# jinhojsk515/spmm

Measured on AMD Instinct MI355X. Metric: pretrain molecules/sec, higher is better.
Workload: dtype bf16; 1 GPU; SPMM pretrain step, text 12 layers (fusion at 6) + PV 6 layers, H=768, 12 heads, queue 36864, train mode (dropout 0.1), fwd+bwd+clip+AdamW+EMA; global_batch=128, seq_len=128, parallelism=dp1, schedule=eager launches on three HIP streams, packed text rows

## Files before the change

include/spmm_hip.h:

```cpp
#ifndef SPMM_HIP_H
#define SPMM_HIP_H

#include <stdint.h>

#ifdef __HIPCC__
#include <hip/hip_runtime.h>
typedef hipStream_t spmm_stream_t;
#else
typedef void* spmm_stream_t;
#endif

#ifdef __cplusplus
extern "C" {
#endif

int spmm_version(void);
const char* spmm_last_error(void);

#define SPMM_EPI_BF16 0
#define SPMM_EPI_GELU 1
#define SPMM_EPI_F32 2
#define SPMM_EPI_F32_ATOMIC 3
#define SPMM_EPI_GELU_GRAD 4
#define SPMM_EPI_F32_ACC 5
#define SPMM_EPI_GELU_DERIV 6
#define SPMM_EPI_MUL 7

#define SPMM_GEMM_AUTO 0
#define SPMM_GEMM_K128 1
#define SPMM_GEMM_K256x128 2
#define SPMM_GEMM_K256 3
#define SPMM_GEMM_K128PC 5
#define SPMM_GEMM_K256P8 8
#define SPMM_GEMM_K256P8_TILES 9
#define SPMM_GEMM_AUTO_TILES 16
int spmm_gemm_nt(const void* A, long lda, const void* W, long ldw, int M, int N, int K, int splits, const float* bias,
                 const float* div_ptr, float alpha, const void* R, long ldr, const void* G, long ldg, void* C, long ldc,
                 void* C2, long ldc2, int epi, float* colsum, int kernel, const int* M_dev, spmm_stream_t stream);
long spmm_gemm_tn_workspace_bytes(int M, int N, int K, int splits);
int spmm_gemm_tn_splits(int M, int N, int K, int kernel);
int spmm_gemm_tn(const void* A, long lda, const void* B, long ldb, int M, int N, int K, int splits, float alpha, float* C,
                 long ldc, float* workspace, int kernel, const int* M_dev, spmm_stream_t stream);
int spmm_gemm_tn_reduce(const float* ws, int ns, int N, int K, float* C, long ldc, spmm_stream_t stream);
int spmm_colsum_bf16(const void* x, long ld, int R, int C, float* out, const int* R_dev, spmm_stream_t stream);

int spmm_attn_fwd(const void* Q, long ldq, const void* K, long ldk, const void* V, long ldv, const int* kmask,
                  const int* kv_seq, const int* q_row0, const int* q_len, const int* kv_row0, const int* kv_len, void* O,
                  long ldo, float* LSE, int nseq, int nH, int Lq, int Lkv, int causal_from, int is_cross, float dropout_p,
                  const uint64_t* seed_ptr, uint64_t seed_salt, int q_off, int kv_off, spmm_stream_t stream);
int spmm_attn_bwd(const void* Q, long ldq, const void* K, long ldk, const void* V, long ldv, const int* kmask,
                  const int* kv_seq, const int* q_row0, const int* q_len, const int* kv_row0, const int* kv_len,
                  const void* O, long ldo, const float* LSE, const void* dO, long lddo, void* dQ,
                  long lddq, void* dK, long lddk, void* dV, long lddv, int nseq, int nH, int Lq, int Lkv, int causal_from,
                  int is_cross, float dropout_p, const uint64_t* seed_ptr, uint64_t seed_salt, int q_off, int kv_off, int d_mode,
                  float* Dbuf, spmm_stream_t stream);

int spmm_xattn_supported(int H, int nH, int Lq, int Lkv);
int spmm_xattn_pack_wo(const void* W, long ldw, void* out, int H, spmm_stream_t stream);
int spmm_xattn_fwd(const void* Q, long ldq, const void* K, long ldk, const void* V, long ldv, const int* kmask,
                   const int* kv_seq, const int* q_row0, const int* q_len, const int* kv_row0, const int* kv_len,
                   const void* WoF, const float* bo, const void* R, long ldr, const float* gamma, const float* beta, float eps,
                   void* Y, long ldy, void* Z, long ldz, float* mean, float* rstd, void* CTX, long ldc, float* LSE,
                   int nseq, int nH, int Lq, int Lkv, float attn_dropout_p, uint64_t salt_a, float hidden_dropout_p,
                   uint64_t salt_h, const uint64_t* seed_ptr, long row_base, spmm_stream_t stream);
int spmm_attn_probs(const void* Q, long ldq, const void* K, long ldk, const int* kmask, const int* kv_seq,
                    const int* q_row0, const int* q_len, const int* kv_row0, const int* kv_len,
                    float* P_mean, float* P_heads, long ldp, long head_stride,
                    int nseq, int nH, int Lq, int Lkv, spmm_stream_t stream);
int spmm_segment_sum_bf16(const void* src, const int* start, const int* list, void* out, int U, long W, spmm_stream_t stream);

int spmm_ln_fwd(const void* x, const void* res, const float* gamma, const float* beta, void* y, void* zout, float* mean,
                float* rstd, long rows, int H, float eps, float dropout_p, const uint64_t* seed_ptr, uint64_t salt,
                const int* rows_dev, spmm_stream_t stream);
int spmm_ln_fwd_r32(const void* x, const float* res32, const float* gamma, const float* beta, void* y, float* y32, void* zout,
                    float* mean, float* rstd, long rows, int H, float eps, float dropout_p, const uint64_t* seed_ptr,
                    uint64_t salt, spmm_stream_t stream);
int spmm_ln_bwd(const void* dy, const void* dy2, const void* z, const float* mean, const float* rstd, const float* gamma,
                void* dz, void* dx, float* dgamma, float* dbeta, long rows, int H, float dropout_p,
                const uint64_t* seed_ptr, uint64_t salt, int drop_on_dy, float* dxsum, const int* rows_dev,
                const float* beta_from_y, spmm_stream_t stream);

int spmm_embed_step_ln_fwd(const int* ids, int pos_index, const int* pos_ptr, const float* word, const float* pos, const float* type0,
                           const float* gamma, const float* beta, void* y, long rows, int H, float eps, spmm_stream_t stream);

int spmm_decode_attn(const void* q, long ldq, const void* K, const void* V, long seq_stride, long tok_stride, long head_stride, const int* anc,
                     int anc_ld, int kv_div, int group, void* out, long ldo, int R, int nH, int Lkv, float scale,
                     const int* t_ptr, const void* knew, const void* vnew, long ldn, const int* rowmap, spmm_stream_t stream);

int spmm_decode_xattn(const void* q, long ldq, const void* K, const void* V, long ldkv, const int* kv_seq, const int* kv_row0,
                      const int* kv_len, int group, void* out, long ldo, int R, int nH, int Lkv_max, float scale, spmm_stream_t stream);

int spmm_beam_step(const float* logits, long ldl, int N, int k, int V, int Lmax, int F, int t, const int* t_ptr, int t_off,
                   int* tokens, float* cur_p, float* fin_p, int* fin_len, int* fin_tok, int* fin_n, unsigned char* done,
                   int* anc, int anc_ld, int* ids_out, int* parent_out, int* n_done, const int* mol, const int* rowmap,
                   spmm_stream_t stream);

int spmm_beam_step_until(const float* logits, long ldl, int N, int k, int V, int Lmax, int F, int t, const int* t_ptr, int t_off,
                         int* tokens, float* cur_p, float* fin_p, int* fin_len, int* fin_tok, int* fin_n, unsigned char* done,
                         int* anc, int anc_ld, int* ids_out, int* parent_out, int* n_done, const int* mol, const int* rowmap,
                         int need, spmm_stream_t stream);

int spmm_beam_step_sampled(const float* logits, long ldl, int N, int k, int V, int Lmax, int F, int t, const int* t_ptr, int t_off,
                           int* tokens, float* cur_p, float* fin_p, int* fin_len, int* fin_tok, int* fin_n, unsigned char* done,
                           int* anc, int anc_ld, int* ids_out, int* parent_out, int* n_done, const int* mol, const int* rowmap,
                           const float* noise, long ldn, spmm_stream_t stream);

int spmm_gumbel_noise(const uint64_t* seed_ptr, uint64_t salt, int N, int k, int V, int Lmax, int t, const int* t_ptr, int t_off,
                      const int* mol, long mol_base, float* out, long ldo, spmm_stream_t stream);

int spmm_logit_warp(const float* lc, const float* lu, long ld, int R, int V, float w, float temperature, int top_k, float top_p,
                    int min_keep, float* out, long ldo, spmm_stream_t stream);

#define SPMM_SYNTAX_MASKED (-1e30f)
int spmm_smiles_mask(float* logits, float* logits2, long ld, int R, int V, const int* tokens, long tok_ld, int hist_rows, int k,
                     const int* mol, int Lmax, int t, const int* t_ptr, int t_off, int t_last, const int* table, int* state_out,
                     spmm_stream_t stream);

int spmm_wordpiece(const unsigned char* blob, const long* offsets, int N, int gap, const unsigned char* head, int head_len,
                   const int* table, int table_words, int max_chars, int max_pieces, int unk_id, int sep_id, int pad_id,
                   int* ids, long ld, int* lens, int* status, spmm_stream_t stream);

int spmm_sbs_step(const float* logits, long ldl, const float* noise, long ldn, int G, int W, int V, int Lmax, int t, const int* t_ptr,
                  int t_off, const float* phi_in, const float* gum_in, const unsigned char* fin_in, const int* len_in,
                  const int* tokens_in, const int* anc_in, float* phi_out, float* gum_out, unsigned char* fin_out, int* len_out,
                  int* tokens_out, int* anc_out, int anc_ld, int* ids_out, int* parent_out, int* open_out, unsigned int* ws,
                  spmm_stream_t stream);

int spmm_kv_prefill(const void* K, const void* V, long ld, long src_rows, const int* row0, const int* len, const int* dst_row, int E,
                    void* Kc, void* Vc, int R, int nH, int Lmax, spmm_stream_t stream);

int spmm_embed_ln_fwd(int mode, const int* ids, const float* word, const float* pos, const float* type0, const float* pv_x,
                      const float* pv_mask, const float* pv_w, const float* pv_b, const float* pv_cls,
                      const float* pv_masktok, int src_mod, const float* gamma, const float* beta, void* y, void* zout,
                      float* mean, float* rstd, long nseq, int L, int H, float eps, float dropout_p,
                      const uint64_t* seed_ptr, uint64_t salt, spmm_stream_t stream);
int spmm_embed_bwd(int mode, const void* dz, const int* ids, const float* pv_x, const float* pv_mask, int src_mod,
                   float* dword, float* dpos, float* dtype0, float* d_w, float* d_b, float* d_cls, float* d_masktok,
                   long nseq, int L, int H, spmm_stream_t stream);

int spmm_transpose_bf16(const void* in, long ldi, void* out, long ldo, int R, int C, int Rpad, float* colsum,
                        spmm_stream_t stream);
int spmm_cast_transpose(const float* in, void* out, void* outT, int R, int C, spmm_stream_t stream);
long spmm_cast_transpose_desc_bytes(void);
int spmm_cast_transpose_multi(const void* descs_dev, int ndesc, int total_tiles, spmm_stream_t stream);
int spmm_cast_f32_bf16(const float* in, void* out, long n, spmm_stream_t stream);
int spmm_cast_bf16_f32(const void* in, float* out, long n, spmm_stream_t stream);
int spmm_acc_rows(float* dst, long ldd, const void* src, long lds, const long* idx, long rows, int H, int atomic,
                  spmm_stream_t stream);
int spmm_gather_rows(void* dst, const void* src, const long* idx, long rows, int H, spmm_stream_t stream);

int spmm_gather_rows2(void* dst, const void* srcA, const void* srcB, const long* idx, long rows, int H, spmm_stream_t stream);
int spmm_add_rows_bf16(void* dst, const long* idx, const void* src, long rows, int H, spmm_stream_t stream);
int spmm_zero_bytes(void* p, long nbytes, spmm_stream_t stream);
int spmm_zero_rows(void* p, long rows, long row_bytes, long stride_bytes, spmm_stream_t stream);
int spmm_gelu_bwd(const void* dz, const void* pre, void* out, long n, spmm_stream_t stream);
int spmm_pack_plan(const int* mask, int B, int Lt, int M, int* lens32, int* row0_32, long* row0_64, long* rows, long* gidx2,
                   long* gidx4, long* inv, long* idx_m, int* bad, spmm_stream_t stream);
int spmm_fusion_plan(const long* neg, const int* lens32, const int* row0_32, int B, int Lt, int Lp, int M,
                     long* idx6, long* neg_rows, long* idx_top, int* small32, spmm_stream_t stream);

int spmm_l2norm_fwd(const float* x, long ldx, float* y, float* nrm, void* a3, void* w3, void* yT, long ldt, int rows, int E,
                    spmm_stream_t stream);
int spmm_l2norm_bwd(const float* dy, const float* y, const float* nrm, const float* gscale, void* dx, int rows, int E,
                    spmm_stream_t stream);
int spmm_ita_rows(const float* S, const float* SM, long ldj, int nrows, int B, int J, const float* alpha_ptr,
                  const float* temp_ptr, void* dS, long ldd, int Jpad, float* losses, int loss_slot, float* dtemp,
                  int* nan_flag, spmm_stream_t stream);
int spmm_sample_neg(const float* S, long ldj, int B, const long* forced, const uint64_t* seed_ptr, uint64_t salt, long* out,
                    long out_offset, spmm_stream_t stream);
int spmm_lm_loss(const float* logits, const float* logits_m, long ldl, const int* ids, long nseq, int L, int V,
                 const float* alpha_ptr, int* n_nonpad_ws, const float* gscale, void* dlogits, long ldd, int Vpad,
                 float* losses, int loss_slot, spmm_stream_t stream);
int spmm_s2s_loss(const float* logits, long ldl, const int* ids, const long* row_of, long rows, long nseq, int L, int V,
                  int* n_label_ws, const float* gscale, void* dlogits, long ldd, int Vpad, float* losses, int loss_slot,
                  spmm_stream_t stream);
int spmm_lm_score(const void* y, long ldy, const void* Wd, long ldw, const float* bias, const int* ids, const long* row_of, long rows,
                  long nseq, int L, int V, int H, const int* seq_row0, const int* seq_len, float* tok_lp, float* seq_lp, int* seq_n,
                  spmm_stream_t stream);
int spmm_itm_head(const void* xa, long stride_a, const void* xb, long stride_b, int H, const float* W, const float* bias,
                  int n, int B, const float* gscale, float* losses, int loss_slot, float* logits_out, void* dxa, void* dxb,
                  float* dW, float* db, int do_bwd, int x_is_f32, spmm_stream_t stream);
int spmm_task_head(const void* A, long lda, int B, int W, const float* W2, const float* b2, int C, int kind, const void* target,
                   const float* gscale, float* logits, float* loss, void* dA, long ldda, float* dW2, float* db2, int do_bwd,
                   spmm_stream_t stream);
int spmm_s2p_append(const void* y, long ldy, const float* w3, const float* b3, const float* pe_w, const float* pe_b, const float* pos,
                    const float* type0, const float* gamma, const float* beta, float eps, float* pred, long ldp, void* xcache,
                    long rows, int H, int n_props, int i, spmm_stream_t stream);
int spmm_mpm_head(const void* h, int Lp, int H, const float* w, const float* bias, const float* target, const float* mask,
                  int B, int* n_keep_ws, const float* gscale, float* losses, int loss_slot, float* pred_out, void* dh,
                  float* dw, float* db, int do_bwd, int x_is_f32, spmm_stream_t stream);
int spmm_rows_linear(const void* x, int x_is_bf16, long ldx, const float* W, const float* bias, float* out, long ldo, long rows,
                     int N, int K, int act, spmm_stream_t stream);
long spmm_sim_topk_workspace_bytes(int Q, long n, int k);
int spmm_sim_topk(const float* q, long ldq, const float* f, long ldf, long base, int Q, long n, int E, int k, float* scores, long* index,
                  int merge, const float* cut_scores, const long* cut_index, void* workspace, long workspace_bytes, spmm_stream_t stream);
int spmm_centroid_assign(const float* f, long ldf, const float* c, long ldc, long c0, long n, int Kc, int E, float* best, int* assign,
                         int merge, const int* prev, int* changed, spmm_stream_t stream);
long spmm_cluster_group_workspace_bytes(long n, int K);
int spmm_cluster_group(const int* assign, long n, int K, int* counts, long* offsets, int* members, int* outside, void* workspace,
                       long workspace_bytes, spmm_stream_t stream);
long spmm_cluster_centroids_workspace_bytes(long n, int K, int E);
int spmm_cluster_centroids(const float* f, long ldf, long n, int E, const float* best, const int* counts, const long* offsets,
                           const int* members, int K, float* centres, long ldc, float* norm, int* medoid, void* workspace,
                           long workspace_bytes, spmm_stream_t stream);
int spmm_enqueue(const float* feats, int n, int E, float* queue, int Q, void* w3, void* qT, long ldt, int Bloc, long* ptr,
                 int advance, const int* skip_flag, spmm_stream_t stream);
int spmm_queue_shadow(const float* queue, int E, int Q, void* w3, void* qT, long ldt, int Bloc, spmm_stream_t stream);
int spmm_clamp_scalar(float* p, float lo, float hi, spmm_stream_t stream);

long spmm_adam_scalars_bytes(void);
long spmm_grad_sqnorm_workspace_bytes(void);
int spmm_grad_sqnorm(const float* g, long n, float* out_zeroed, float* workspace, spmm_stream_t stream);
int spmm_adamw_step(float* p, const float* g, float* m, float* v, void* bf16_shadow, long n, const float* lr_ptr,
                    float beta1, float beta2, float eps, float weight_decay, const float* normsq, float max_norm, int* step,
                    const int* nan_flag, void* scalars_ws, spmm_stream_t stream);
int spmm_ema_update(float* pm, const float* p, void* bf16_shadow, long n, float momentum, spmm_stream_t stream);
int spmm_axpy_scalar(float* dst, const float* src, const float* scale_ptr, float scale, int n, spmm_stream_t stream);

#ifdef __cplusplus
}
#endif
#endif
```

spmm_amd/csrc/rowops.hip:

```cpp
#include "common.h"
#include <stdlib.h>
#include "../../include/spmm_hip.h"

namespace {

constexpr int MAXC = 4;

struct RowVec {
  float v[MAXC][4];
};

__device__ __forceinline__ void load_row_bf16(const bf16* __restrict__ p, int H, int lane, RowVec& r) {
#pragma unroll
  for (int i = 0; i < MAXC; ++i) {
    const int c = (lane + 64 * i) * 4;
    if (c < H) {
      const bf16x4 t = *(const bf16x4*)(p + c);
      r.v[i][0] = (float)t[0]; r.v[i][1] = (float)t[1]; r.v[i][2] = (float)t[2]; r.v[i][3] = (float)t[3];
    } else {
      r.v[i][0] = r.v[i][1] = r.v[i][2] = r.v[i][3] = 0.f;
    }
  }
}
__device__ __forceinline__ void store_row_bf16(bf16* __restrict__ p, int H, int lane, const RowVec& r) {
// ... 240 lines not shown
                                                     bf16* __restrict__ dz_o, bf16* __restrict__ dx_o,
                                                     float* __restrict__ dgamma, float* __restrict__ dbeta, long rows, int H,
                                                     uint32_t thresh16, float dscale, const uint64_t* seed_ptr, uint64_t salt,
                                                     int drop_on_dy, float* __restrict__ dxsum, const int* __restrict__ rows_ptr) {
  __shared__ float red[4][NC * 256];
  if (rows_ptr) { const long r_ = *rows_ptr; rows = r_ < rows ? r_ : rows; }
  const int lane = threadIdx.x & 63, wave = threadIdx.x >> 6;
  float gsum[NC][4], bsum[NC][4], xsum[NC][4];
#pragma unroll
  for (int i = 0; i < NC; ++i)
#pragma unroll
    for (int j = 0; j < 4; ++j) gsum[i][j] = bsum[i][j] = xsum[i][j] = 0.f;
  if (HOT) { dy2 = nullptr; drop_on_dy = 0; }
  const bool has2 = !HOT && dy2 != nullptr, has_dx = HOT || dx_o != nullptr, has_xs = HOT || dxsum != nullptr, drop = HOT || thresh16 != 0;
  const uint64_t seed = drop ? seed_mix(seed_ptr, salt) : 0;
  const long stride = (long)gridDim.x * 4;
  long row = (long)blockIdx.x * 4 + wave;
  RawRow<NC> ng, ng2, nz;
  float nmean = 0.f, nrstd = 0.f;
  if (row < rows) {
    load_raw<NC, EXACT>(dy + row * H, H, lane, ng);
    if (has2) load_raw<NC, EXACT>(dy2 + row * H, H, lane, ng2);
    load_raw<NC, EXACT>(z + row * H, H, lane, nz);
    nmean = FROMY ? 0.f : mean_i[row]; nrstd = rstd_i[row];
  }
  for (; row < rows; row += stride) {
    RawRow<NC> cg = ng, cg2 = ng2, cz = nz;
    const float mean = nmean, rstd = nrstd;
    const long nrow = row + stride;
    if (nrow < rows) {
      load_raw<NC, EXACT>(dy + nrow * H, H, lane, ng);
      if (has2) load_raw<NC, EXACT>(dy2 + nrow * H, H, lane, ng2);
      load_raw<NC, EXACT>(z + nrow * H, H, lane, nz);
      nmean = FROMY ? 0.f : mean_i[nrow]; nrstd = rstd_i[nrow];
    }
    float g[NC][4], xh[NC][4];
    const uint32_t rowkey = drop ? drop_rowkey(seed, (uint64_t)row) : 0u;
#pragma unroll
    for (int i = 0; i < NC; ++i)
#pragma unroll
      for (int j = 0; j < 4; ++j) g[i][j] = (float)cg.v[i][j] + (has2 ? (float)cg2.v[i][j] : 0.f);
    if (drop && drop_on_dy) {
#pragma unroll
      for (int i = 0; i < NC; ++i) {
        const int c = (lane + 64 * i) * 4;
        if (EXACT || c < H) {
          bool k[4];
          drop_keep4(rowkey, c, thresh16, k);
#pragma unroll
          for (int j = 0; j < 4; ++j) g[i][j] = k[j] ? g[i][j] * dscale : 0.f;
        }
      }
    }
    float s1 = 0.f, s2 = 0.f;
#pragma unroll
    for (int i = 0; i < NC; ++i) {
      const int c = (lane + 64 * i) * 4;
      if (EXACT || c < H) {
        const f32x4 gm = *(const f32x4*)(gamma + c);
        f32x4 bt = {0.f, 0.f, 0.f, 0.f}, ig = {0.f, 0.f, 0.f, 0.f};
        if constexpr (FROMY) {
          bt = *(const f32x4*)(beta + c);
#pragma unroll
          for (int j = 0; j < 4; ++j) ig[j] = gm[j] != 0.f ? __builtin_amdgcn_rcpf(gm[j]) : 0.f;
        }
#pragma unroll
        for (int j = 0; j < 4; ++j) {
          const float x = FROMY ? ((float)cz.v[i][j] - bt[j]) * ig[j] : ((float)cz.v[i][j] - mean) * rstd;
          const float dg = g[i][j] * gm[j];
          gsum[i][j] += g[i][j] * x;
          bsum[i][j] += g[i][j];
          if constexpr (!FROMY) xh[i][j] = x;
          g[i][j] = dg;
          s1 += dg;
          s2 += dg * x;
        }
      } else {
#pragma unroll
        for (int j = 0; j < 4; ++j) { if constexpr (!FROMY) xh[i][j] = 0.f; g[i][j] = 0.f; }
      }
    }
    s1 = wave_sum_dpp(s1) / H;
    s2 = wave_sum_dpp(s2) / H;
    const bool mask_dx = has_dx && drop && !drop_on_dy;
#pragma unroll
    for (int i = 0; i < NC; ++i) {
      const int c = (lane + 64 * i) * 4;
      if (EXACT || c < H) {
        float o[4];
        if constexpr (FROMY) {
          const f32x4 gm = *(const f32x4*)(gamma + c), bt = *(const f32x4*)(beta + c);
#pragma unroll
          for (int j = 0; j < 4; ++j) {
            const float x = ((float)cz.v[i][j] - bt[j]) * (gm[j] != 0.f ? __builtin_amdgcn_rcpf(gm[j]) : 0.f);
            o[j] = rstd * (g[i][j] - s1 - x * s2);
          }
        } else {
#pragma unroll
          for (int j = 0; j < 4; ++j) o[j] = rstd * (g[i][j] - s1 - xh[i][j] * s2);
        }
        const bf16x4 ob = to_bf16x4(o[0], o[1], o[2], o[3]);
        *(bf16x4*)(dz_o + row * H + c) = ob;
        if (has_dx) {
          bf16x4 xb = ob;
          if (mask_dx) {
            bool k[4];
            drop_keep4(rowkey, c, thresh16, k);
            xb = to_bf16x4(k[0] ? o[0] * dscale : 0.f, k[1] ? o[1] * dscale : 0.f, k[2] ? o[2] * dscale : 0.f, k[3] ? o[3] * dscale : 0.f);
          }
          *(bf16x4*)(dx_o + row * H + c) = xb;
          if (has_xs) {
#pragma unroll
            for (int j = 0; j < 4; ++j) xsum[i][j] += (float)xb[j];
          }
        } else if (has_xs) {
#pragma unroll
          for (int j = 0; j < 4; ++j) xsum[i][j] += (float)ob[j];
        }
      }
    }
  }
  if (!HOT && dgamma == nullptr && dxsum == nullptr) return;
#pragma unroll
  for (int which = 0; which < 3; ++which) {
    float* dst = which == 0 ? dgamma : which == 1 ? dbeta : dxsum;
    if (!HOT && dst == nullptr) continue;
    __syncthreads();
#pragma unroll
    for (int i = 0; i < NC; ++i)
#pragma unroll
      for (int j = 0; j < 4; ++j)
        red[wave][(lane + 64 * i) * 4 + j] = which == 0 ? gsum[i][j] : which == 1 ? bsum[i][j] : xsum[i][j];
    __syncthreads();
    for (int c = threadIdx.x; c < H; c += 256) atomicAdd(dst + c, red[0][c] + red[1][c] + red[2][c] + red[3][c]);
  }
}

struct EmbedP {
  const int* ids;
  const float* word;
  const float* pos;
  const float* type0;
  const float* pv_x;
  const float* pv_mask;
  const float* pv_w; const float* pv_b; const float* pv_cls; const float* pv_masktok;
  int src_mod;
  const float* gamma; const float* beta;
  bf16* y; bf16* zout; float* mean_o; float* rstd_o;
  long nseq; int L, H, mode; float eps;
  int pos0;
  const int* pos_ptr;
  uint32_t thresh16; float dscale; const uint64_t* seed_ptr; uint64_t salt;
};

__global__ __launch_bounds__(256) void embed_ln_fwd_kernel(EmbedP p) {
  const int lane = threadIdx.x & 63;
  const long row = (long)blockIdx.x * 4 + (threadIdx.x >> 6);
  if (row >= p.nseq * p.L) return;
  const long seq = row / p.L;
  const int l = (int)(row - seq * p.L);
  RowVec z, t, o;
  load_row_f32(p.pos + (long)(l + (p.pos_ptr ? *p.pos_ptr : p.pos0)) * p.H, p.H, lane, z);
  load_row_f32(p.type0, p.H, lane, t);
#pragma unroll
  for (int i = 0; i < MAXC; ++i)
#pragma unroll
    for (int j = 0; j < 4; ++j) z.v[i][j] += t.v[i][j];
  if (p.mode == 0) {
    const int id = p.ids[row];
    load_row_f32(p.word + (long)id * p.H, p.H, lane, t);
  } else if (p.mode == 2) {
    load_row_f32(p.pv_x + row * p.H, p.H, lane, t);
  } else if (l == 0) {
    load_row_f32(p.pv_cls, p.H, lane, t);
  } else {
    const long src = (seq % p.src_mod) * (p.L - 1) + (l - 1);
    const float m = p.pv_mask[src], xv = p.pv_x[src];
    RowVec w, b;
    load_row_f32(p.pv_w, p.H, lane, w);
    load_row_f32(p.pv_b, p.H, lane, b);
    load_row_f32(p.pv_masktok, p.H, lane, t);
#pragma unroll
    for (int i = 0; i < MAXC; ++i)
#pragma unroll
      for (int j = 0; j < 4; ++j) t.v[i][j] = (xv * w.v[i][j] + b.v[i][j]) * (1.f - m) + t.v[i][j] * m;
  }
#pragma unroll
  for (int i = 0; i < MAXC; ++i)
#pragma unroll
    for (int j = 0; j < 4; ++j) z.v[i][j] += t.v[i][j];
  float mean, rstd;
  ln_apply(z, p.H, lane, p.gamma, p.beta, p.eps, mean, rstd, o);
  if (p.thresh16) {
    const uint32_t rowkey = drop_rowkey(seed_mix(p.seed_ptr, p.salt), (uint64_t)row);
#pragma unroll
    for (int i = 0; i < MAXC; ++i) {
      const int c = (lane + 64 * i) * 4;
      if (c < p.H) {
        bool k[4];
        drop_keep4(rowkey, c, p.thresh16, k);
#pragma unroll
        for (int j = 0; j < 4; ++j) o.v[i][j] = k[j] ? o.v[i][j] * p.dscale : 0.f;
      }
    }
  }
  store_row_bf16(p.y + row * p.H, p.H, lane, o);
  if (p.zout) store_row_bf16(p.zout + row * p.H, p.H, lane, z);
  if (p.mean_o && lane == 0) { p.mean_o[row] = mean; p.rstd_o[row] = rstd; }
}

struct EmbedBwdP {
  const bf16* dz; const int* ids; const float* pv_x; const float* pv_mask; int src_mod;
  float* dword; float* dpos; float* dtype0; float* d_w; float* d_b; float* d_cls; float* d_masktok;
  long nseq; int L, H, mode;
};
__global__ __launch_bounds__(256) void embed_bwd_kernel(EmbedBwdP p) {
  const int l = blockIdx.x;
  const long s_per = (p.nseq + gridDim.y - 1) / gridDim.y;
  const long s_beg = blockIdx.y * s_per, s_end = min(p.nseq, s_beg + s_per);
  for (int c = threadIdx.x; c < p.H; c += 256) {
    float acc = 0.f, accw = 0.f, accb = 0.f, accm = 0.f;
    for (long s = s_beg; s < s_end; ++s) {
      const long row = s * p.L + l;
      const float g = (float)p.dz[row * p.H + c];
      acc += g;
      if (p.mode == 0) {
        const int id = p.ids[row];
        if (id != 0) atomicAdd(p.dword + (long)id * p.H + c, g);
      } else if (l > 0) {
        const long src = (s % p.src_mod) * (p.L - 1) + (l - 1);
        const float m = p.pv_mask[src];
        accw += g * (1.f - m) * p.pv_x[src];
        accb += g * (1.f - m);
        accm += g * m;
      }
    }
    atomicAdd(p.dpos + (long)l * p.H + c, acc);
    atomicAdd(p.dtype0 + c, acc);
    if (p.mode == 1) {
      if (l == 0) {
        atomicAdd(p.d_cls + c, acc);
      } else {
        atomicAdd(p.d_w + c, accw);
        atomicAdd(p.d_b + c, accb);
        atomicAdd(p.d_masktok + c, accm);
      }
    }
  }
}

__global__ __launch_bounds__(256) void transpose_bf16_kernel(const bf16* __restrict__ in, long ldi, bf16* __restrict__ out,
                                                             long ldo, int R, int C, int Rpad, float* __restrict__ colsum) {
  __shared__ bf16 tile[64][66];
  const int r0 = blockIdx.y * 64, c0 = blockIdx.x * 64;
  const int tx = threadIdx.x & 63, ty = threadIdx.x >> 6;
  float cs = 0.f;
#pragma unroll
  for (int i = 0; i < 16; ++i) {
    const int r = r0 + ty * 16 + i, c = c0 + tx;
    const bf16 v = (r < R && c < C) ? in[(long)r * ldi + c] : (bf16)0.f;
    tile[ty * 16 + i][tx] = v;
    cs += (float)v;
  }
  if (colsum) {
    __shared__ float part[4][64];
    part[ty][tx] = cs;
    __syncthreads();
    if (ty == 0 && c0 + tx < C) atomicAdd(colsum + c0 + tx, part[0][tx] + part[1][tx] + part[2][tx] + part[3][tx]);
  } else {
    __syncthreads();
  }
#pragma unroll
  for (int i = 0; i < 16; ++i) {
    const int c = c0 + ty * 16 + i, r = r0 + tx;
    if (c < C && r < Rpad) out[(long)c * ldo + r] = tile[tx][ty * 16 + i];
  }
}

__global__ __launch_bounds__(256) void cast_transpose_kernel(const float* __restrict__ in, bf16* __restrict__ out,
                                                             bf16* __restrict__ outT, int R, int C) {
  __shared__ bf16 tile[64][66];
  const int r0 = blockIdx.y * 64, c0 = blockIdx.x * 64;
  const int tx = threadIdx.x & 63, ty = threadIdx.x >> 6;
#pragma unroll
  for (int i = 0; i < 16; ++i) {
    const int r = r0 + ty * 16 + i, c = c0 + tx;
    bf16 v = (bf16)0.f;
    if (r < R && c < C) {
      v = (bf16)in[(long)r * C + c];
      if (out) out[(long)r * C + c] = v;
    }
    tile[ty * 16 + i][tx] = v;
  }
  __syncthreads();
  if (outT) {
#pragma unroll
    for (int i = 0; i < 16; ++i) {
      const int c = c0 + ty * 16 + i, r = r0 + tx;
      if (c < C && r < R) outT[(long)c * R + r] = tile[tx][ty * 16 + i];
    }
  }
}

struct CtDesc { const float* src; bf16* dstT; int R, C; int tile0, ntc; };
__global__ __launch_bounds__(256) void cast_transpose_multi_kernel(const CtDesc* __restrict__ descs, int ndesc) {
  __shared__ bf16 tile[64][66];
  int lo = 0, hi = ndesc - 1;
  while (lo < hi) {
    const int mid = (lo + hi + 1) >> 1;
    if (descs[mid].tile0 <= (int)blockIdx.x) lo = mid; else hi = mid - 1;
  }
  const CtDesc d = descs[lo];
  const int tt = blockIdx.x - d.tile0;
  const int r0 = (tt / d.ntc) * 64, c0 = (tt % d.ntc) * 64;
  const int tx = threadIdx.x & 63, ty = threadIdx.x >> 6;
#pragma unroll
  for (int i = 0; i < 16; ++i) {
    const int r = r0 + ty * 16 + i, c = c0 + tx;
    tile[ty * 16 + i][tx] = (r < d.R && c < d.C) ? (bf16)d.src[(long)r * d.C + c] : (bf16)0.f;
  }
  __syncthreads();
#pragma unroll
  for (int i = 0; i < 16; ++i) {
    const int c = c0 + ty * 16 + i, r = r0 + tx;
    if (c < d.C && r < d.R) d.dstT[(long)c * d.R + r] = tile[tx][ty * 16 + i];
  }
}

__global__ void cast_f32_bf16_kernel(const float* __restrict__ in, bf16* __restrict__ out, long n4) {
  for (long i = (long)blockIdx.x * blockDim.x + threadIdx.x; i < n4; i += (long)gridDim.x * blockDim.x) {
    const f32x4 v = *(const f32x4*)(in + i * 4);
    *(bf16x4*)(out + i * 4) = to_bf16x4(v[0], v[1], v[2], v[3]);
  }
}
__global__ void cast_bf16_f32_kernel(const bf16* __restrict__ in, float* __restrict__ out, long n4) {
  for (long i = (long)blockIdx.x * blockDim.x + threadIdx.x; i < n4; i += (long)gridDim.x * blockDim.x) {
    const bf16x4 v = *(const bf16x4*)(in + i * 4);
    f32x4 o = {(float)v[0], (float)v[1], (float)v[2], (float)v[3]};
    *(f32x4*)(out + i * 4) = o;
  }
}

__global__ void acc_rows_kernel(float* __restrict__ dst, long ldd, const bf16* __restrict__ src, long lds,
                                const long* __restrict__ idx, long rows, int H, int atomic) {
  const int h4 = H / 4;
  for (long i = (long)blockIdx.x * blockDim.x + threadIdx.x; i < rows * h4; i += (long)gridDim.x * blockDim.x) {
    const long r = i / h4;
    const int c = (int)(i - r * h4) * 4;
    const long dr = idx ? idx[r] : r;
    if (dr < 0) continue;
    const bf16x4 v = *(const bf16x4*)(src + r * lds + c);
    float* d = dst + dr * ldd + c;
    if (atomic) {
#pragma unroll
      for (int j = 0; j < 4; ++j) atomicAdd(d + j, (float)v[j]);
    } else {
      f32x4 o = *(f32x4*)d;
      o[0] += (float)v[0]; o[1] += (float)v[1]; o[2] += (float)v[2]; o[3] += (float)v[3];
      *(f32x4*)d = o;
    }
  }
}
__global__ void gather_rows_kernel(bf16* __restrict__ dst, const bf16* __restrict__ src, const long* __restrict__ idx,
                                   long rows, int H) {
  const int h8 = H / 8;
  for (long i = (long)blockIdx.x * blockDim.x + threadIdx.x; i < rows * h8; i += (long)gridDim.x * blockDim.x) {
    const long r = i / h8;
    const int c = (int)(i - r * h8) * 8;
    *(bf16x8*)(dst + r * H + c) = *(const bf16x8*)(src + idx[r] * H + c);
  }
}

int grid_for(long work, int block) {
  long g = (work + block - 1) / block;
  return (int)(g < 1 ? 1 : (g > 2048 ? 2048 : g));
}


}

extern "C" int spmm_ln_fwd(const void* x, const void* res, const float* gamma, const float* beta, void* y, void* zout,
                           float* mean, float* rstd, long rows, int H, float eps, float dropout_p,
                           const uint64_t* seed_ptr, uint64_t salt, const int* rows_dev, hipStream_t stream) {
  SPMM_CHECK_SHAPE(rows > 0 && H > 0 && H % 4 == 0 && H <= 1024, "spmm_ln_fwd: rows=%ld H=%d (need H%%4==0, H<=1024)", rows, H);
  SPMM_CHECK_SHAPE(dropout_p == 0.f || seed_ptr, "spmm_ln_fwd: dropout needs a device seed");
  SPMM_CHECK_SHAPE(x && gamma && beta && y, "spmm_ln_fwd: null x / gamma / beta / y");
  SPMM_CHECK_SHAPE((mean == nullptr) == (rstd == nullptr), "spmm_ln_fwd: mean and rstd come together");
  const uint32_t th = (uint32_t)(dropout_p * 65536.f + 0.5f);
  const float ds = 1.f / (1.f - dropout_p);
#define LN_FWD16(NC)                                                                                                          \
  hipLaunchKernelGGL(ln_fwd16_kernel<NC>, dim3((rows + 7) / 8), dim3(256), 0, stream, (const bf16*)x, (const bf16*)res, gamma, \
                     beta, (bf16*)y, (bf16*)zout, mean, rstd, rows, eps, th, ds, seed_ptr, salt, rows_dev)
  if (H == 768) LN_FWD16(3);
  else if (H == 1024) LN_FWD16(4);
  else if (H == 512) LN_FWD16(2);
  else if (H == 256) LN_FWD16(1);
  else
    hipLaunchKernelGGL(ln_fwd_kernel, dim3((rows + 3) / 4), dim3(256), 0, stream, (const bf16*)x, (const bf16*)res, gamma, beta,
                       (bf16*)y, (bf16*)zout, mean, rstd, rows, H, eps, th, ds, seed_ptr, salt, rows_dev);
#undef LN_FWD16
  SPMM_LAUNCH_CHECK("spmm_ln_fwd");
  return SPMM_OK;
}

extern "C" int spmm_ln_fwd_r32(const void* x, const float* res32, const float* gamma, const float* beta, void* y, float* y32, void* zout,
                               float* mean, float* rstd, long rows, int H, float eps, float dropout_p, const uint64_t* seed_ptr,
                               uint64_t salt, hipStream_t stream) {
  SPMM_CHECK_SHAPE(rows > 0 && H > 0 && H % 4 == 0 && H <= 1024, "spmm_ln_fwd_r32: rows=%ld H=%d (need H%%4==0, H<=1024)", rows, H);
  SPMM_CHECK_SHAPE(dropout_p == 0.f || seed_ptr, "spmm_ln_fwd_r32: dropout needs a device seed");
  SPMM_CHECK_SHAPE((mean == nullptr) == (rstd == nullptr), "spmm_ln_fwd_r32: mean and rstd come together");
  hipLaunchKernelGGL(ln_fwd_r32_kernel, dim3((rows + 3) / 4), dim3(256), 0, stream, (const bf16*)x, res32, gamma, beta, (bf16*)y, y32,
                     (bf16*)zout, mean, rstd, rows, H, eps, (uint32_t)(dropout_p * 65536.f + 0.5f), 1.f / (1.f - dropout_p), seed_ptr, salt);
  SPMM_LAUNCH_CHECK("spmm_ln_fwd_r32");
  return SPMM_OK;
}

extern "C" int spmm_ln_bwd(const void* dy, const void* dy2, const void* z, const float* mean, const float* rstd,
                           const float* gamma, void* dz, void* dx, float* dgamma, float* dbeta, long rows, int H,
                           float dropout_p, const uint64_t* seed_ptr, uint64_t salt, int drop_on_dy, float* dxsum, const int* rows_dev,
                           const float* beta_from_y, hipStream_t stream) {
  SPMM_CHECK_SHAPE(rows > 0 && H > 0 && H % 4 == 0 && H <= 1024, "spmm_ln_bwd: rows=%ld H=%d", rows, H);
  SPMM_CHECK_SHAPE(beta_from_y != nullptr || mean != nullptr, "spmm_ln_bwd: the row means are required unless `z` holds the LayerNorm output (beta_from_y)");
  SPMM_CHECK_SHAPE(beta_from_y == nullptr || !drop_on_dy, "spmm_ln_bwd: the output of a LayerNorm followed by dropout does not determine the normalised values");
  SPMM_CHECK_SHAPE(dropout_p == 0.f || seed_ptr, "spmm_ln_bwd: dropout needs a device seed");
  SPMM_CHECK_SHAPE(dy && z && rstd && gamma && dz, "spmm_ln_bwd: null dy / z / rstd / gamma / dz");
  long g = (rows + 3) / 4;
  static const long genv = getenv("SPMM_LN_BWD_GRID") ? atol(getenv("SPMM_LN_BWD_GRID")) : 0;
  long gmax = genv > 0 ? genv : rows / 64;
  if (genv <= 0) gmax = gmax < 256 ? 256 : (gmax > 512 ? 512 : gmax);
  if (g > gmax) g = gmax;
  const uint32_t th = (uint32_t)(dropout_p * 65536.f + 0.5f);
  const float ds = 1.f / (1.f - dropout_p);
  const bool hot = !dy2 && dx && dgamma && dbeta && dxsum && th && !drop_on_dy;
#define LN_BWD_LAUNCH(NC, EX, HOT, FY)                                                                                                \
  hipLaunchKernelGGL((ln_bwd_kernel<NC, EX, HOT, FY>), dim3(g), dim3(256), 0, stream, (const bf16*)dy, (const bf16*)dy2, (const bf16*)z, \
                     mean, rstd, gamma, beta_from_y, (bf16*)dz, (bf16*)dx, dgamma, dbeta, rows, H, th, ds, seed_ptr, salt, drop_on_dy, dxsum, rows_dev)
  if (beta_from_y != nullptr) {
    if (H == 768 && hot) LN_BWD_LAUNCH(3, true, true, true);
    else if (H <= 768) LN_BWD_LAUNCH(3, false, false, true);
    else LN_BWD_LAUNCH(4, false, false, true);
  } else {
    if (H == 768 && hot) LN_BWD_LAUNCH(3, true, true, false);
    else if (H <= 768) LN_BWD_LAUNCH(3, false, false, false);
    else LN_BWD_LAUNCH(4, false, false, false);
  }
#undef LN_BWD_LAUNCH
  SPMM_LAUNCH_CHECK("spmm_ln_bwd");
  return SPMM_OK;
}

extern "C" int spmm_embed_ln_fwd(int mode, const int* ids, const float* word, const float* pos, const float* type0,
                                 const float* pv_x, const float* pv_mask, const float* pv_w, const float* pv_b,
                                 const float* pv_cls, const float* pv_masktok, int src_mod, const float* gamma,
                                 const float* beta, void* y, void* zout, float* mean, float* rstd, long nseq, int L, int H,
                                 float eps, float dropout_p, const uint64_t* seed_ptr, uint64_t salt, hipStream_t stream) {
  SPMM_CHECK_SHAPE(nseq > 0 && L > 0 && H > 0 && H % 4 == 0 && H <= 1024, "spmm_embed_ln_fwd: nseq=%ld L=%d H=%d (need 0 < H <= 1024, H%%4==0)", nseq, L, H);
  SPMM_CHECK_SHAPE(mode >= 0 && mode <= 2, "spmm_embed_ln_fwd: unknown mode %d", mode);
  SPMM_CHECK_SHAPE(pos && type0 && gamma && beta && y, "spmm_embed_ln_fwd: null pos / type0 / gamma / beta / y");
  SPMM_CHECK_SHAPE((mean == nullptr) == (rstd == nullptr), "spmm_embed_ln_fwd: mean and rstd come together");
  SPMM_CHECK_SHAPE(mode == 0 ? (ids && word) : mode == 2 ? (pv_x != nullptr) : (pv_x && pv_mask && pv_w && pv_b && pv_cls && pv_masktok && src_mod > 0),
                   "spmm_embed_ln_fwd: missing inputs for mode %d", mode);
  SPMM_CHECK_SHAPE(dropout_p == 0.f || seed_ptr, "spmm_embed_ln_fwd: dropout needs a device seed");
  EmbedP p = {};
  p.ids = ids; p.word = word; p.pos = pos; p.type0 = type0; p.pv_x = pv_x; p.pv_mask = pv_mask; p.pv_w = pv_w; p.pv_b = pv_b;
  p.pv_cls = pv_cls; p.pv_masktok = pv_masktok; p.src_mod = src_mod; p.gamma = gamma; p.beta = beta; p.y = (bf16*)y;
  p.zout = (bf16*)zout; p.mean_o = mean; p.rstd_o = rstd; p.nseq = nseq; p.L = L; p.H = H; p.mode = mode; p.eps = eps;
  p.thresh16 = (uint32_t)(dropout_p * 65536.f + 0.5f); p.dscale = 1.f / (1.f - dropout_p); p.seed_ptr = seed_ptr; p.salt = salt;
  hipLaunchKernelGGL(embed_ln_fwd_kernel, dim3((nseq * L + 3) / 4), dim3(256), 0, stream, p);
  SPMM_LAUNCH_CHECK("spmm_embed_ln_fwd");
  return SPMM_OK;
}

extern "C" int spmm_embed_step_ln_fwd(const int* ids, int pos_index, const int* pos_ptr, const float* word, const float* pos, const float* type0,
                                      const float* gamma, const float* beta, void* y, long rows, int H, float eps,
                                      hipStream_t stream) {
  SPMM_CHECK_SHAPE(rows > 0 && pos_index >= 0 && H % 4 == 0 && H <= 1024, "spmm_embed_step_ln_fwd: rows=%ld pos=%d H=%d", rows, pos_index, H);
  SPMM_CHECK_SHAPE(ids && word && pos && type0 && gamma && beta && y, "spmm_embed_step_ln_fwd: null argument");
  EmbedP p = {};
  p.ids = ids; p.word = word; p.pos = pos; p.type0 = type0; p.gamma = gamma; p.beta = beta; p.y = (bf16*)y;
  p.nseq = rows; p.L = 1; p.H = H; p.mode = 0; p.eps = eps; p.pos0 = pos_index; p.pos_ptr = pos_ptr; p.dscale = 1.f;
  hipLaunchKernelGGL(embed_ln_fwd_kernel, dim3((rows + 3) / 4), dim3(256), 0, stream, p);
  SPMM_LAUNCH_CHECK("spmm_embed_step_ln_fwd");
  return SPMM_OK;
}

extern "C" int spmm_embed_bwd(int mode, const void* dz, const int* ids, const float* pv_x, const float* pv_mask, int src_mod,
                              float* dword, float* dpos, float* dtype0, float* d_w, float* d_b, float* d_cls,
                              float* d_masktok, long nseq, int L, int H, hipStream_t stream) {
  SPMM_CHECK_SHAPE(nseq > 0 && L > 0 && H > 0, "spmm_embed_bwd: nseq=%ld L=%d H=%d", nseq, L, H);
  SPMM_CHECK_SHAPE(mode == 0 || mode == 1, "spmm_embed_bwd: mode %d (0 = text, 1 = PV; inputs_embeds has no backward)", mode);
  SPMM_CHECK_SHAPE(dz && dpos && dtype0, "spmm_embed_bwd: null dz / dpos / dtype0");
  SPMM_CHECK_SHAPE(mode != 0 || (ids && dword), "spmm_embed_bwd: mode 0 needs ids and dword");
  SPMM_CHECK_SHAPE(mode != 1 || (pv_x && pv_mask && d_w && d_b && d_cls && d_masktok), "spmm_embed_bwd: mode 1 needs pv_x, pv_mask, d_w, d_b, d_cls and d_masktok");
  SPMM_CHECK_SHAPE(mode != 1 || src_mod > 0, "spmm_embed_bwd: mode 1 needs src_mod > 0, got src_mod=%d", src_mod);
  EmbedBwdP p = {(const bf16*)dz, ids, pv_x, pv_mask, src_mod, dword, dpos, dtype0, d_w, d_b, d_cls, d_masktok, nseq, L, H, mode};
  hipLaunchKernelGGL(embed_bwd_kernel, dim3(L, nseq >= 32 ? 16 : 1), dim3(256), 0, stream, p);
  SPMM_LAUNCH_CHECK("spmm_embed_bwd");
  return SPMM_OK;
}

namespace {
__global__ __launch_bounds__(256) void segment_sum_kernel(const bf16* __restrict__ src, const int* __restrict__ start,
                                                          const int* __restrict__ list, bf16* __restrict__ out, long W) {
  const int u = blockIdx.y;
  const long c = ((long)blockIdx.x * 256 + threadIdx.x) * 8;
  if (c >= W) return;
  const int k0 = start[u], k1 = start[u + 1];
  float acc[8] = {0.f, 0.f, 0.f, 0.f, 0.f, 0.f, 0.f, 0.f};
  for (int k = k0; k < k1; ++k) {
    const bf16x8 v = *(const bf16x8*)(src + (long)list[k] * W + c);
#pragma unroll
    for (int e = 0; e < 8; ++e) acc[e] += (float)v[e];
  }
  bf16x8 o;
#pragma unroll
  for (int e = 0; e < 8; ++e) o[e] = (bf16)acc[e];
  *(bf16x8*)(out + (long)u * W + c) = o;
}
}

extern "C" int spmm_segment_sum_bf16(const void* src, const int* start, const int* list, void* out, int U, long W, hipStream_t stream) {
  SPMM_CHECK_SHAPE(U > 0 && U <= 65535 && W > 0 && W % 8 == 0, "spmm_segment_sum_bf16: U=%d W=%ld (W %% 8 == 0)", U, W);
  SPMM_CHECK_SHAPE(src && start && list && out, "spmm_segment_sum_bf16: null src / start / list / out");
  hipLaunchKernelGGL(segment_sum_kernel, dim3((unsigned)((W / 8 + 255) / 256), U), dim3(256), 0, stream, (const bf16*)src, start, list,
                     (bf16*)out, W);
  SPMM_LAUNCH_CHECK("spmm_segment_sum_bf16");
  return SPMM_OK;
}

extern "C" int spmm_transpose_bf16(const void* in, long ldi, void* out, long ldo, int R, int C, int Rpad, float* colsum,
                                   hipStream_t stream) {
  SPMM_CHECK_SHAPE(R > 0 && C > 0 && Rpad >= R && ldo >= Rpad, "spmm_transpose_bf16: R=%d C=%d Rpad=%d ldo=%ld", R, C, Rpad, ldo);
  SPMM_CHECK_SHAPE(ldi >= C, "spmm_transpose_bf16: ldi=%ld is shorter than a row of C=%d", ldi, C);
  SPMM_CHECK_SHAPE(in && out, "spmm_transpose_bf16: null in / out");
  hipLaunchKernelGGL(transpose_bf16_kernel, dim3((C + 63) / 64, (Rpad + 63) / 64), dim3(256), 0, stream, (const bf16*)in, ldi,
                     (bf16*)out, ldo, R, C, Rpad, colsum);
  SPMM_LAUNCH_CHECK("spmm_transpose_bf16");
  return SPMM_OK;
}

extern "C" int spmm_cast_transpose(const float* in, void* out, void* outT, int R, int C, hipStream_t stream) {
  SPMM_CHECK_SHAPE(R > 0 && C > 0, "spmm_cast_transpose: R=%d C=%d", R, C);
  SPMM_CHECK_SHAPE(in && (out || outT), "spmm_cast_transpose: null in, or neither out nor outT");
  hipLaunchKernelGGL(cast_transpose_kernel, dim3((C + 63) / 64, (R + 63) / 64), dim3(256), 0, stream, in, (bf16*)out, (bf16*)outT, R, C);
  SPMM_LAUNCH_CHECK("spmm_cast_transpose");
  return SPMM_OK;
}

extern "C" long spmm_cast_transpose_desc_bytes(void) { return sizeof(CtDesc); }
extern "C" int spmm_cast_transpose_multi(const void* descs_dev, int ndesc, int total_tiles, hipStream_t stream) {
  SPMM_CHECK_SHAPE(ndesc > 0 && total_tiles > 0, "spmm_cast_transpose_multi: ndesc=%d tiles=%d", ndesc, total_tiles);
  hipLaunchKernelGGL(cast_transpose_multi_kernel, dim3(total_tiles), dim3(256), 0, stream, (const CtDesc*)descs_dev, ndesc);
  SPMM_LAUNCH_CHECK("spmm_cast_transpose_multi");
  return SPMM_OK;
}

extern "C" int spmm_cast_f32_bf16(const float* in, void* out, long n, hipStream_t stream) {
  SPMM_CHECK_SHAPE(n > 0 && n % 4 == 0, "spmm_cast_f32_bf16: n=%ld must be a positive multiple of 4", n);
  SPMM_CHECK_SHAPE(in && out, "spmm_cast_f32_bf16: null in / out");
  hipLaunchKernelGGL(cast_f32_bf16_kernel, dim3(grid_for(n / 4, 256)), dim3(256), 0, stream, in, (bf16*)out, n / 4);
  SPMM_LAUNCH_CHECK("spmm_cast_f32_bf16");
  return SPMM_OK;
}
extern "C" int spmm_cast_bf16_f32(const void* in, float* out, long n, hipStream_t stream) {
  SPMM_CHECK_SHAPE(n > 0 && n % 4 == 0, "spmm_cast_bf16_f32: n=%ld must be a positive multiple of 4", n);
  SPMM_CHECK_SHAPE(in && out, "spmm_cast_bf16_f32: null in / out");
  hipLaunchKernelGGL(cast_bf16_f32_kernel, dim3(grid_for(n / 4, 256)), dim3(256), 0, stream, (const bf16*)in, out, n / 4);
  SPMM_LAUNCH_CHECK("spmm_cast_bf16_f32");
  return SPMM_OK;
}

extern "C" int spmm_acc_rows(float* dst, long ldd, const void* src, long lds, const long* idx, long rows, int H, int atomic,
                             hipStream_t stream) {
  SPMM_CHECK_SHAPE(rows > 0 && H > 0 && H % 4 == 0, "spmm_acc_rows: rows=%ld H=%d", rows, H);
  SPMM_CHECK_SHAPE(dst && src, "spmm_acc_rows: null dst / src");
  SPMM_CHECK_SHAPE(rows == 1 || (ldd >= H && lds >= H), "spmm_acc_rows: ldd=%ld lds=%ld are shorter than a row of H=%d", ldd, lds, H);
  hipLaunchKernelGGL(acc_rows_kernel, dim3(grid_for(rows * (H / 4), 256)), dim3(256), 0, stream, dst, ldd, (const bf16*)src, lds,
                     idx, rows, H, atomic);
  SPMM_LAUNCH_CHECK("spmm_acc_rows");
  return SPMM_OK;
}
extern "C" int spmm_gather_rows(void* dst, const void* src, const long* idx, long rows, int H, hipStream_t stream) {
  SPMM_CHECK_SHAPE(rows > 0 && H > 0 && H % 8 == 0 && idx, "spmm_gather_rows: rows=%ld H=%d", rows, H);
  SPMM_CHECK_SHAPE(dst && src, "spmm_gather_rows: null dst / src");
  hipLaunchKernelGGL(gather_rows_kernel, dim3(grid_for(rows * (H / 8), 256)), dim3(256), 0, stream, (bf16*)dst, (const bf16*)src,
                     idx, rows, H);
  SPMM_LAUNCH_CHECK("spmm_gather_rows");
  return SPMM_OK;
}
```

spmm_amd/engine.py:

```python
from __future__ import annotations

import contextlib
import functools
from dataclasses import dataclass
from typing import List, NamedTuple, Optional

import numpy as np
import torch

from . import ops, streams
from .config import BertConfig, SPMMConfig
from .options import EngineOptions
from .params import ParamStore

BF = torch.bfloat16
LOSS_MLM, LOSS_MPM, LOSS_ITA, LOSS_ITM = 0, 1, 2, 3


def _ceil(x, m):
    return (x + m - 1) // m * m


class KVSource:

    def __init__(self, kv: torch.Tensor, U: int, Lkv: int, row0=None, length=None, pack_idx=None, proj=None):
        self.kv, self.U, self.Lkv, self.row0, self.len, self.pack_idx = kv, U, Lkv, row0, length, pack_idx
        self.proj = proj
        self._idx: List[torch.Tensor] = []
        self.nseq = 0
        self.start = self.list = None

    def add(self, idx: torch.Tensor) -> int:
        off = self.nseq
        self._idx.append(idx)
        self.nseq += idx.numel()
        return off

    def preset(self, nseq: int, start: torch.Tensor, lst: torch.Tensor):
        self.nseq, self.start, self.list = nseq, start, lst
        return self

    def finalize(self):
        idx = torch.cat(self._idx)
        order = torch.sort(idx, stable=True).indices
        start = torch.zeros(self.U + 1, dtype=torch.int32, device=idx.device)
        counts = torch.zeros(self.U, dtype=torch.int64, device=idx.device).index_add_(0, idx, torch.ones_like(idx))
        start[1:] = torch.cumsum(counts, 0)
        self.start, self.list = start, order.to(torch.int32)
        return self


@dataclass
class SelfKV:
    x: torch.Tensor
    dx: Optional[torch.Tensor] = None
    rows_dev: Optional[torch.Tensor] = None


@dataclass
class Group:
    row0: int
    nseq: int
    L: int
    kmask: Optional[torch.Tensor]
    causal_from: int
    kv: Optional[torch.Tensor] = None
    Lkv: int = 0
    kv_mask: Optional[torch.Tensor] = None
    q_row0: Optional[torch.Tensor] = None
    q_len: Optional[torch.Tensor] = None
    nrows: int = -1
    src: Optional[KVSource] = None
    kv_idx: Optional[torch.Tensor] = None
    kv_off: int = 0
    self_src: Optional[SelfKV] = None
    skv_row0: Optional[torch.Tensor] = None
    skv_len: Optional[torch.Tensor] = None
    skv_L: int = 0

    @property
    def rows(self):
        n = self.nrows if self.nrows >= 0 else self.nseq * self.L
        return slice(self.row0, self.row0 + n)

    def bind(self, src: KVSource, kv_idx: torch.Tensor, kv_off: int) -> "Group":
        self.src, self.Lkv, self.kv_idx, self.kv_off = src, src.Lkv, kv_idx, kv_off
        return self

    def attend(self, src: KVSource, idx: torch.Tensor) -> "Group":
        self.src, self.Lkv = src, src.Lkv
        self.kv_off = src.add(idx)
        self.kv_idx = idx.to(torch.int32)
        return self

    def cross_layout(self) -> dict:
        src = self.src
        return dict(kmask=self.kv_mask, kv_seq=self.kv_idx, q_row0=self.q_row0, q_len=self.q_len,
                    kv_row0=None if src is None else src.row0, kv_len=None if src is None else src.len)


@dataclass
class Batch:
    groups: List[Group]
    rows_dev: Optional[torch.Tensor] = None

    def __iter__(self):
        return iter(self.groups)

    def __len__(self):
        return len(self.groups)


@dataclass
class LnTape:
    z: Optional[torch.Tensor]
    y: Optional[torch.Tensor]
    mean: Optional[torch.Tensor]
    rstd: Optional[torch.Tensor]
    salt: int = 0


@dataclass
class HeadTape:
    dense: str
    norm: str
    X: torch.Tensor
    pre: Optional[torch.Tensor]
    ln: LnTape


def _prefix_lens(mask_h: torch.Tensor) -> Optional[torch.Tensor]:
    lens = mask_h.sum(1)
    prefix = bool((lens > 0).all()) and bool(((torch.arange(mask_h.shape[1])[None, :] < lens[:, None]) == (mask_h != 0)).all())
    return lens if prefix else None


def host_lens(mask_h: torch.Tensor, what: str) -> np.ndarray:
    if mask_h.dim() != 2 or mask_h.shape[0] == 0:
        raise ValueError(f"{what}: the attention mask must be [n, L] with n >= 1")
    lens = _prefix_lens(mask_h)
    if lens is None:
        raise ValueError(f"{what}: every attention mask must be a non-empty prefix (what padding a batch to its longest gives)")
    return lens.numpy().astype(np.int64)


def host_token_count(mask) -> Optional[int]:
    if not (torch.is_tensor(mask) and mask.device.type == "cpu" and mask.dim() == 2):
        return None
    lens = _prefix_lens(mask)
    return None if lens is None else int(lens.sum())


class PairLayout(NamedTuple):
    len_p: np.ndarray
    qrow0: np.ndarray
    Mt: int
    pos: np.ndarray
    seq: np.ndarray
    gather: np.ndarray


@dataclass
class TextRows:
    x: torch.Tensor
    groups: Batch
    pk: Optional[dict]
    cls_rows: torch.Tensor
    ids32: torch.Tensor
    mask32: torch.Tensor
    B: int
    L: int
    esv: LnTape
    y: Optional[torch.Tensor] = None
    tape: Optional[list] = None

    @property
    def kv_mask(self):
        return None if self.pk else self.mask32

    def tables(self):
        if self.pk:
            return self.pk["row0"], self.pk["len"]
        return torch.arange(self.B, dtype=torch.int32, device=self.mask32.device) * self.L, self.mask32.sum(1).to(torch.int32)

    def source(self, proj=None, tables: bool = False) -> KVSource:
        row0, length = self.tables() if (self.pk or tables) else (None, None)
        return KVSource(self.y, self.B, self.L, row0=row0, length=length, pack_idx=self.pk["rows"] if self.pk else None, proj=proj)

    def pair_layout(self, lens_u: np.ndarray, inv: np.ndarray) -> PairLayout:
        row0_u = np.concatenate([[0], np.cumsum(lens_u)[:-1]]) if self.pk else np.arange(self.B, dtype=np.int64) * self.L
        len_p = lens_u[inv]
        qrow0 = np.concatenate([[0], np.cumsum(len_p)[:-1]])
        pos = np.concatenate([np.arange(l) for l in len_p])
        seq = np.repeat(np.arange(len(inv)), len_p)
        return PairLayout(len_p, qrow0, int(len_p.sum()), pos, seq, row0_u[inv][seq] + pos)


STREAM_TOKENS_MAX = 49152


class Engine:
    def __init__(self, cfg: SPMMConfig, params: ParamStore, device, options: Optional[EngineOptions] = None):
        self.cfg, self.P, self.dev = cfg, params, device
        self.opt = options if options is not None else EngineOptions.from_env()
        if torch.device(device).type == "cuda":
            from ._lib import bind_device
            bind_device(torch.device(device).index if torch.device(device).index is not None else torch.cuda.current_device())
        f32 = dict(dtype=torch.float32, device=device)
        self.alpha = torch.zeros(1, **f32)
        self.lr = torch.zeros(1, **f32)
        self.gscale = torch.ones(4, **f32)
        self.step_zero = torch.zeros(16, dtype=torch.int32, device=device)
        self.losses = self.step_zero[0:8].view(torch.float32)
        self.loss_scratch = torch.zeros(8, **f32)
        rank = torch.distributed.get_rank() if (torch.distributed.is_available() and torch.distributed.is_initialized()) else 0
        self.seed_rank_offset = rank * 0x9E3779B97F4A7C15 % (1 << 62)
        self.seed = torch.full((1,), (0x5DEECE66D + self.seed_rank_offset) % (1 << 62), dtype=torch.int64, device=device)
        self.nan_flag = self.step_zero[9:10]
        self.icount = torch.zeros(8, dtype=torch.int32, device=device)
        self.dtemp_ita = self.step_zero[8:9].view(torch.float32)
        self.train_mode = True
        self.hint_bad = self.step_zero[10:11]
        self.pack_text = self.opt.pack_text
        self.layer_done_cb = None
        self.multi_stream = self.opt.multi_stream
        self.wgrad_async = self.opt.wgrad_stream and self.multi_stream
        self._one_stream = False
        dist_ = torch.distributed
        will_exchange = dist_.is_available() and dist_.is_initialized() and (dist_.get_world_size() > 1 or self.opt.force_dist)
        self._one_side = bool(will_exchange and self.opt.dp_four_streams)
        if self.multi_stream and torch.device(device).type == "cuda" and not ops._DRY_RUN and not will_exchange:
            streams.bind_in_order(device, ("side0", "side1", "wgrad"))
        self.force_one_stream = False
        self._wg_stream, self._wg_pending, self._wg_keep = None, False, []
        self._salt = 0
        self._off_path_ok, self._pre_bwd = False, None
        self._xattn_checked = self._xattn_off = False
        self.tape = None
        E, Q = cfg.embed_dim, cfg.queue_size
        self._bank = None

    def _fork(self, which: int = 0):
        if not self.multi_stream or self._one_stream or self.dev.type != "cuda" or ops._DRY_RUN:
            return None
        side = streams.get(self.dev, "side0" if self._one_side else f"side{which}")
        streams.after(side, torch.cuda.current_stream())
        return side

    def _join(self, side):
        if side is not None:
            streams.after(torch.cuda.current_stream(), side)

    @staticmethod
    def _on(side):
        return torch.cuda.stream(side) if side is not None else contextlib.nullcontext()

    def _new(self, *shape, dtype=BF):
        return torch.empty(*shape, dtype=dtype, device=self.dev)

    def _stats(self, M, save):
        return (self._new(M, dtype=torch.float32), self._new(M, dtype=torch.float32)) if save else (None, None)

    def _zeros(self, *shape, dtype=BF):
        return ops.zero_(torch.empty(*shape, dtype=dtype, device=self.dev))

    def _next_salt(self):
        self._salt += 1
        return self._salt * 0x9E3779B97F4A7C15 % (1 << 63)

    def _p_hidden(self, c: BertConfig):
        return c.hidden_dropout_prob if self.train_mode else 0.0

    def _p_attn(self, c: BertConfig):
        return c.attention_probs_dropout_prob if self.train_mode else 0.0

    def _wT(self, key, src_fp32):
        return self.P.wT(key, src_fp32)

    def _wgrad(self, dY, X, gW, gb=None, inline=False, md=None):
        ws = None if inline else self._wgrad_side()
        C = gW.view(dY.shape[1], X.shape[1])
        if ws is None:
            if gb is not None:
                ops.colsum_bf16(dY, gb, R_dev=md)
            ops.gemm_tn(dY, X, C, M_dev=md)
            return
        streams.after(ws, torch.cuda.current_stream())
        with torch.cuda.stream(ws):
            if gb is not None:
                ops.colsum_bf16(dY, gb, R_dev=md)
            ops.gemm_tn(dY, X, C, M_dev=md)
        self._wg_keep.append((dY, X))
        self._wg_pending = True

    def _wgrad_side(self):
        if not self.wgrad_async or self._one_stream or self.dev.type != "cuda" or ops._DRY_RUN:
            return None
        self._wg_stream = streams.get(self.dev, "wgrad")
        return self._wg_stream

    def off_path(self, fn):
        ws = self._wgrad_side() if self._off_path_ok else None
        if ws is None or torch.cuda.is_current_stream_capturing():
            fn()
            return
        streams.after(ws, torch.cuda.current_stream())
        with torch.cuda.stream(ws):
            fn()
            self._pre_bwd = streams.mark(ws)

    def pre_backward_wait(self):
        ev, self._pre_bwd = self._pre_bwd, None
        if ev is not None:
            torch.cuda.current_stream().wait_event(ev)

    def wgrad_join(self, release: bool = False):
        if self._wg_stream is not None and self._wg_pending:
            streams.after(torch.cuda.current_stream(), self._wg_stream)
            if release:
                self._wg_keep.clear()
                self._wg_pending = False

    def end_backward(self):
        self.wgrad_join(release=True)
        self.tape = None

    def _pack_plan(self, mask32: torch.Tensor, B: int, Lt: int, n_tokens: Optional[int] = None):
        if n_tokens is not None:
            M = int(n_tokens)
            if M >= B * Lt:
                return None
        else:
            lens = mask32.sum(1)
            prefix = (torch.arange(Lt, device=mask32.device)[None, :] < lens[:, None]) == (mask32 != 0)
            stats = torch.stack([lens.sum(), (lens > 0).sum(), prefix.all().to(lens.dtype)]).cpu()
            M, nonempty, is_prefix = int(stats[0]), int(stats[1]), int(stats[2])
            if nonempty != B or not is_prefix or M >= B * Lt:
                return None
        if M < 1:
            return None
        return ops.pack_plan(mask32, M, self.hint_bad)

    def text_rows(self, x: torch.Tensor, mask32: torch.Tensor, pk: Optional[dict]):
        B, L = mask32.shape
        if not pk:
            return x, Batch([Group(0, B, L, mask32, B)]), torch.arange(B, dtype=torch.int64, device=self.dev) * L
        x = ops.gather_rows2(self._new(pk["M"], x.shape[1]), x, pk["rows"])
        return x, Batch([Group(0, B, L, None, B, q_row0=pk["row0"], q_len=pk["len"], nrows=pk["M"])]), pk["row0_64"]

    def text_rows_of(self, pfx, c, ids32, mask32, *, n_tokens: Optional[int] = None, save=False, causal=False, what: str = "") -> TextRows:
        B, L = ids32.shape
        if L > c.max_position_embeddings:
            raise ValueError(f"{what}sequence length {L} exceeds the {c.max_position_embeddings} position embeddings")
        x, esv = self.embed_text(pfx, c, ids32, B, L, save)
        pk = self._pack_plan(mask32, B, L, n_tokens) if (self.pack_text and L <= ops.ATTN_MAXL) else None
        x, groups, cls_rows = self.text_rows(x, mask32, pk)
        if causal:
            groups.groups[0].causal_from = 0
        return TextRows(x, groups, pk, cls_rows, ids32, mask32, B, L, esv)

    def encode_text(self, pfx, c, ids32, mask32, *, n_tokens: Optional[int] = None, save=False, causal=False, what: str = "") -> TextRows:
        t = self.text_rows_of(pfx, c, ids32, mask32, n_tokens=n_tokens, save=save, causal=causal, what=what)
        t.y, t.tape, _ = self.stack_fwd(pfx, c, range(0, c.fusion_layer), False, t.x, t.groups, save)
        return t

    def _ln_res(self, x, X, X32, gamma, beta, y, md, **kw):
        if X32 is None:
            ops.ln_fwd(x, X, gamma, beta, y, rows_dev=md, **kw)
            return None
        assert md is None
        y32 = self._new(*y.shape, dtype=torch.float32)
        ops.ln_fwd_r32(x, X32, gamma, beta, y, y32=y32, **kw)
        return y32

    def _proj_ln(self, op, A, resid, X32, *, save, eps, ph, salt, md=None):
        P = self.P
        Wb = P.wb(op + "dense.weight")
        M, H = A.shape[0], Wb.shape[0]
        x, y = self._new(M, H), self._new(M, H)
        mean, rstd = self._stats(M, save)
        ops.gemm_nt(A, Wb, x, bias=P.w(op + "dense.bias"), M_dev=md)
        from_y = self.opt.ln_from_y and X32 is None
        y32 = self._ln_res(x, resid, X32, P.w(op + "LayerNorm.weight"), P.w(op + "LayerNorm.bias"), y, md,
                           zout=x if (save and not from_y) else None, mean=mean, rstd=rstd, eps=eps, dropout_p=ph, seed=self.seed, salt=salt)
        return y, LnTape(None if from_y else x, y, mean, rstd, salt), y32

    def _proj_ln_bwd(self, op, tape, dY, A, ph, md=None):
        P, (M, H) = self.P, dY.shape
        dz = self._new(M, H)
        dx = self._new(M, H) if ph > 0 else dz
        from_y = tape.z is None
        ops.ln_bwd(dY, tape.y if from_y else tape.z, tape.mean, tape.rstd, P.w(op + "LayerNorm.weight"), dz, dx=dx if ph > 0 else None,
                   dgamma=P.g(op + "LayerNorm.weight"), dbeta=P.g(op + "LayerNorm.bias"), dropout_p=ph, seed=self.seed, salt=tape.salt,
                   dxsum=P.g(op + "dense.bias"), rows_dev=md, beta_from_y=P.w(op + "LayerNorm.bias") if from_y else None)
        self._wgrad(dx, A, P.g(op + "dense.weight"), md=md)
        return dz, dx

    def _attn_block_fwd(self, pfx, c, X, groups, save, cross, X32=None, kv_tap=None, xattn_tap=None):
        P, H, nH = self.P, c.hidden_size, c.num_attention_heads
        salts_a = [self._next_salt() for _ in groups]
        salt_h = self._next_salt()
        sv = {"X": X, "salt_a": salts_a, "cross": cross}
        if not cross:
            ctx, core = self._self_attn_fwd(pfx, c, X, groups, save, salts_a, kv_tap)
        else:
            sv["Qc"] = Qc = ops.gemm_nt(X, P.wb(pfx + ".self.query.weight"), self._new(X.shape[0], H), bias=P.w(pfx + ".self.query.bias"),
                                        M_dev=groups.rows_dev)
            done = {id(g.src): g.src.proj[pfx] for g in groups if g.src is not None and g.src.proj and pfx in g.src.proj}
            kv_of = functools.partial(self._xattn_kv, P.fused(pfx + ".self.", ("key", "value"), "weight"),
                                      P.fused(pfx + ".self.", ("key", "value"), "bias", what="w"), done)
            if xattn_tap is not None:
                for gi, g in enumerate(groups):
                    xattn_tap(gi, g, Qc[g.rows], kv_of(g)[:, :H])
            fx = self.opt.fused_xattn
            fused = ((fx is True or fx == "all" or (fx == "nograd" and not save)) and not self._xattn_off and X32 is None
                     and groups.rows_dev is None and all(ops.xattn_supported(H, nH, g.L, g.Lkv) for g in groups))
            if fused:
                y, out = self._xattn_fused_fwd(pfx, c, X, Qc, kv_of, groups, save, salts_a, salt_h)
                g0 = groups.groups[0]
                if not self._xattn_checked and not ops._DRY_RUN and g0.row0 == 0:
                    self._xattn_checked = True
                    agrees, dmax, dmean = self._xattn_agrees(pfx, c, X, Qc, out["KV"][0], g0, y, salts_a[0], salt_h)
                    if not agrees:
                        import warnings
                        warnings.warn(f"spmm_amd: the fused cross-attention kernel disagrees with the composite launches (max |dy| {dmax:.3g}, "
                                      f"mean {dmean:.3g}); falling back to the composite for this process (SPMM_FUSED_XATTN=off)")
                        streams.note("fused cross-attention kernel failed its one-time self-check: composite launches used instead")
                        self._xattn_off = True
                        fused = False
                if fused:
                    sv.update(out)
                    return y, (sv if save else None), None
            ctx, core = self._xattn_core_fwd(c, Qc, kv_of, groups, save, salts_a)
        y, ln, y32 = self._proj_ln(pfx + ".output.", ctx, X, X32, save=save, eps=c.layer_norm_eps, ph=self._p_hidden(c), salt=salt_h,
                                   md=groups.rows_dev)
        sv.update(core, ctx=ctx, ln=ln)
        return y, (sv if save else None), y32

    def _self_attn_fwd(self, pfx, c, X, groups, save, salts, kv_tap=None):
        P, H, nH, M = self.P, c.hidden_size, c.num_attention_heads, X.shape[0]
        Wqkv = P.fused(pfx + ".self.", ("query", "key", "value"), "weight")
        bqkv = P.fused(pfx + ".self.", ("query", "key", "value"), "bias", what="w")
        QKV = ops.gemm_nt(X, Wqkv, self._new(M, 3 * H), bias=bqkv, M_dev=groups.rows_dev)
        if kv_tap is not None:
            kv_tap(QKV)
        ctx, lses = self._new(M, H), []
        skv = {}
        for g, salt in zip(groups, salts):
            lse = self._new(g.nseq, nH, g.L, dtype=torch.float32) if save else None
            r = g.rows
            kw = dict(nseq=g.nseq, nH=nH, Lq=g.L, dropout_p=self._p_attn(c), seed=self.seed, salt=salt, q_row0=g.q_row0, q_len=g.q_len)
            if g.self_src is not None:
                if id(g.self_src) not in skv:
                    skv[id(g.self_src)] = ops.gemm_nt(g.self_src.x, Wqkv[H:], self._new(g.self_src.x.shape[0], 2 * H), bias=bqkv[H:],
                                                      M_dev=g.self_src.rows_dev)
                KVs = skv[id(g.self_src)]
                ops.attn_fwd_long(QKV[r, :H], KVs[:, :H], KVs[:, H:], ctx[r], lse, Lkv=g.skv_L, kmask=None, causal_from=g.nseq,
                                  kv_row0=g.skv_row0, kv_len=g.skv_len, **kw)
            else:
                ops.attn_fwd_long(QKV[r, :H], QKV[r, H:2 * H], QKV[r, 2 * H:], ctx[r], lse, Lkv=g.L, kmask=g.kmask, causal_from=g.causal_from,
                                  kv_row0=g.q_row0, kv_len=g.q_len, **kw)
            lses.append(lse)
        return ctx, dict(QKV=QKV, SKV=skv, lse=lses)

    def _xattn_kv(self, Wkv, bkv, done, g):
        key, kv = (id(g), g.kv) if g.src is None else (id(g.src), g.src.kv)
        if key not in done:
            done[key] = ops.gemm_nt(kv, Wkv, self._new(kv.shape[0], Wkv.shape[0]), bias=bkv)
        return done[key]

    def _xattn_core_fwd(self, c, Qc, kv_of, groups, save, salts):
        H, nH = c.hidden_size, c.num_attention_heads
        ctx, KVs, lses = self._new(Qc.shape[0], H), [], []
        for g, salt in zip(groups, salts):
            KV = kv_of(g)
            lse = self._new(g.nseq, nH, g.L, dtype=torch.float32) if save else None
            ops.attn_fwd_long(Qc[g.rows], KV[:, :H], KV[:, H:], ctx[g.rows], lse, nseq=g.nseq, nH=nH, Lq=g.L, Lkv=g.Lkv, is_cross=True,
                              dropout_p=self._p_attn(c), seed=self.seed, salt=salt, **g.cross_layout())
            KVs.append(KV)
            lses.append(lse)
        return ctx, dict(KV=KVs, lse=lses)

    def _xattn_fused_fwd(self, pfx, c, X, Qc, kv_of, groups, save, salts, salt_h):
        P, H, nH, M = self.P, c.hidden_size, c.num_attention_heads, X.shape[0]
        y = self._new(M, H)
        z, ctx = (self._new(M, H), self._new(M, H)) if save else (None, None)
        mean, rstd = self._stats(M, save)
        WoF = P.wF(pfx + ".output.dense.weight")
        KVs, lses = [], []
        for g, salt in zip(groups, salts):
            KV = kv_of(g)
            lse = self._new(g.nseq, nH, g.L, dtype=torch.float32) if save else None
            r = g.rows
            ops.xattn_fwd(Qc[r], KV[:, :H], KV[:, H:], WoF, P.w(pfx + ".output.dense.bias"), X[r], P.w(pfx + ".output.LayerNorm.weight"),
                          P.w(pfx + ".output.LayerNorm.bias"), y[r], nseq=g.nseq, nH=nH, Lq=g.L, Lkv=g.Lkv, eps=c.layer_norm_eps,
                          Z=None if z is None else z[r], mean=None if mean is None else mean[r.start:r.stop],
                          rstd=None if rstd is None else rstd[r.start:r.stop], CTX=None if ctx is None else ctx[r], lse=lse,
                          attn_dropout_p=self._p_attn(c), salt_a=salt, hidden_dropout_p=self._p_hidden(c), salt_h=salt_h, seed=self.seed,
                          row_base=r.start, **g.cross_layout())
            KVs.append(KV)
            lses.append(lse)
        return y, dict(KV=KVs, lse=lses, ctx=ctx, ln=LnTape(z, y, mean, rstd, salt_h))

    def _xattn_agrees(self, pfx, c, X, Qc, KV, g, y, salt_a, salt_h):
        H, r = c.hidden_size, g.rows
        c2 = self._new(r.stop, H)
        ops.attn_fwd_long(Qc[r], KV[:, :H], KV[:, H:], c2, None, nseq=g.nseq, nH=c.num_attention_heads, Lq=g.L, Lkv=g.Lkv, is_cross=True,
                          dropout_p=self._p_attn(c), seed=self.seed, salt=salt_a, **g.cross_layout())
        y2, _, _ = self._proj_ln(pfx + ".output.", c2, X[r], None, save=False, eps=c.layer_norm_eps, ph=self._p_hidden(c), salt=salt_h)
        d = (y[r].float() - y2.float()).abs()
        dmax, dmean = float(d.max()), float(d.mean())
        scale = max(1.0, float(y2.float().abs().max()) / 8.0)
        return dmax < 0.25 * scale and dmean < 5e-3 * scale, dmax, dmean

    def _attn_block_bwd(self, pfx, c, sv, dY, groups, dkv_acc):
        P, H, nH = self.P, c.hidden_size, c.num_attention_heads
        X, M, md = sv["X"], sv["X"].shape[0], groups.rows_dev
        pa, ph = self._p_attn(c), self._p_hidden(c)
        dz, dx = self._proj_ln_bwd(pfx + ".output.", sv["ln"], dY, sv["ctx"], ph, md)
        dctx = self._new(M, H)
        ops.gemm_nt(dx, self._wT(pfx + ".output.dense", P.w(pfx + ".output.dense.weight")), dctx, M_dev=md)
        dX = self._new(M, H)
        if not sv["cross"]:
            QKV = sv["QKV"]
            dQKV = self._new(M, 3 * H)
            gWqkv = P.fused(pfx + ".self.", ("query", "key", "value"), "weight", what="g")
            gbqkv = P.fused(pfx + ".self.", ("query", "key", "value"), "bias", what="g")
            dskv = {}
            for i, g in enumerate(groups):
                r = g.rows
                kw = dict(nseq=g.nseq, nH=nH, Lq=g.L, dropout_p=pa, seed=self.seed, salt=sv["salt_a"][i], q_row0=g.q_row0, q_len=g.q_len)
                if g.self_src is not None:
                    if id(g.self_src) not in dskv:
                        dskv[id(g.self_src)] = (g.self_src, self._zeros(g.self_src.x.shape[0], 2 * H))
                    KVs, dKVs = sv["SKV"][id(g.self_src)], dskv[id(g.self_src)][1]
                    ops.attn_bwd_long(QKV[r, :H], KVs[:, :H], KVs[:, H:], sv["ctx"][r], sv["lse"][i], dctx[r], dQKV[r, :H], dKVs[:, :H], dKVs[:, H:],
                                      Lkv=g.skv_L, kmask=None, causal_from=g.nseq, kv_row0=g.skv_row0, kv_len=g.skv_len, **kw)
                    ops.zero_(dQKV[r, H:])
                    continue
                ops.attn_bwd_long(QKV[r, :H], QKV[r, H:2 * H], QKV[r, 2 * H:], sv["ctx"][r], sv["lse"][i], dctx[r], dQKV[r, :H],
                                  dQKV[r, H:2 * H], dQKV[r, 2 * H:], Lkv=g.L, kmask=g.kmask, causal_from=g.causal_from,
                                  kv_row0=g.q_row0, kv_len=g.q_len, **kw)
            self._wgrad(dQKV, X, gWqkv, gbqkv, md=md)
            WT = self._wT(pfx + ".self.qkv", P.fused(pfx + ".self.", ("query", "key", "value"), "weight", what="w"))
            for src, dKVs in dskv.values():
                self._wgrad(dKVs, src.x, gWqkv[H:], gbqkv[H:], md=src.rows_dev)
                ops.gemm_nt(dKVs, WT[:, H:], src.dx, M_dev=src.rows_dev)
            ops.gemm_nt(dQKV, WT, dX, R=dz, M_dev=md)
        else:
            Qc = sv["Qc"]
            dQc = self._new(M, H)
            gWkv = P.fused(pfx + ".self.", ("key", "value"), "weight", what="g")
            gbkv = P.fused(pfx + ".self.", ("key", "value"), "bias", what="g")
            WkvT = self._wT(pfx + ".self.kv", P.fused(pfx + ".self.", ("key", "value"), "weight", what="w"))
            pool = {}
            for i, g in enumerate(groups):
                r = g.rows
                KV = sv["KV"][i]
                src = g.src
                if src is not None:
                    if id(src) not in pool:
                        pool[id(src)] = (src, self._new(src.nseq * src.Lkv, 2 * H))
                    dKV = pool[id(src)][1][g.kv_off * g.Lkv:(g.kv_off + g.nseq) * g.Lkv]
                else:
                    dKV = self._new(g.nseq * g.Lkv, 2 * H)
                ops.attn_bwd_long(Qc[r], KV[:, :H], KV[:, H:], sv["ctx"][r], sv["lse"][i], dctx[r], dQc[r], dKV[:, :H], dKV[:, H:],
                                  nseq=g.nseq, nH=nH, Lq=g.L, Lkv=g.Lkv, is_cross=True, dropout_p=pa, seed=self.seed, salt=sv["salt_a"][i],
                                  **g.cross_layout())
                if src is None:
                    self._wgrad(dKV, g.kv, gWkv, gbkv)
                    ops.gemm_nt(dKV, WkvT, dkv_acc[i], epi=ops.EPI_F32_ACC)
            for src, dKV in pool.values():
                W = src.Lkv * 2 * H
                dKVu = ops.segment_sum_bf16(dKV.view(src.nseq, W), src.start, src.list, self._new(src.U, W)).view(-1, 2 * H)
                if src.pack_idx is not None:
                    dKVu = ops.gather_rows(self._new(src.pack_idx.numel(), 2 * H), dKVu, src.pack_idx)
                self._wgrad(dKVu, src.kv, gWkv, gbkv)
                ops.gemm_nt(dKVu, WkvT, dkv_acc[id(src)], epi=ops.EPI_F32_ACC)
            self._wgrad(dQc, X, P.g(pfx + ".self.query.weight"), P.g(pfx + ".self.query.bias"), md=md)
            ops.gemm_nt(dQc, self._wT(pfx + ".self.query", P.w(pfx + ".self.query.weight")), dX, R=dz, M_dev=md)
        return dX

    def _layer_fwd(self, lp, c, has_cross, X, groups, save, X32=None, kv_tap=None, xattn_tap=None):
        P, H, I, M = self.P, c.hidden_size, c.intermediate_size, X.shape[0]
        tap = {} if kv_tap is None else {"kv_tap": kv_tap}
        a, sv1, a32 = self._attn_block_fwd(lp + "attention", c, X, groups, save, cross=False, X32=X32, **tap)
        sv2 = None
        if has_cross:
            xtap = {} if xattn_tap is None else {"xattn_tap": xattn_tap}
            a, sv2, a32 = self._attn_block_fwd(lp + "crossattention", c, a, groups, save, cross=True, X32=a32, **xtap)
        h = self._new(M, I)
        dact = self._new(M, I) if save else None
        ops.gemm_nt(a, P.wb(lp + "intermediate.dense.weight"), h, bias=P.w(lp + "intermediate.dense.bias"),
                    epi=ops.EPI_GELU_DERIV if save else ops.EPI_GELU, C2=dact, M_dev=groups.rows_dev)
        salt = self._next_salt()
        y, ln, y32 = self._proj_ln(lp + "output.", h, a, a32, save=save, eps=c.layer_norm_eps, ph=self._p_hidden(c), salt=salt, md=groups.rows_dev)
        sv = dict(att=sv1, cross=sv2, a=a, h=h, dact=dact, ln=ln) if save else None
        return y, sv, y32

    def _layer_bwd(self, lp, c, sv, dY, groups, dkv_acc):
        P, H, I, M, md = self.P, c.hidden_size, c.intermediate_size, dY.shape[0], groups.rows_dev
        dz, dx = self._proj_ln_bwd(lp + "output.", sv["ln"], dY, sv["h"], self._p_hidden(c), md)
        dpre = self._new(M, I)
        ops.gemm_nt(dx, self._wT(lp + "output.dense", P.w(lp + "output.dense.weight")), dpre,
                    epi=ops.EPI_MUL, G=sv["dact"], colsum=P.g(lp + "intermediate.dense.bias"), M_dev=md)
        self._wgrad(dpre, sv["a"], P.g(lp + "intermediate.dense.weight"), md=md)
        da = self._new(M, H)
        ops.gemm_nt(dpre, self._wT(lp + "intermediate.dense", P.w(lp + "intermediate.dense.weight")), da, R=dz, M_dev=md)
        if sv["cross"] is not None:
            da = self._attn_block_bwd(lp + "crossattention", c, sv["cross"], da, groups, dkv_acc)
        return self._attn_block_bwd(lp + "attention", c, sv["att"], da, groups, None)

    def stack_fwd(self, pfx, c, layers, has_cross, X, groups, save, X32=None, kv_tap=None, xattn_tap=None):
        tape = []
        for i in layers:
            tap = None if kv_tap is None else functools.partial(kv_tap, i)
            xtap = {} if xattn_tap is None else {"xattn_tap": functools.partial(xattn_tap, i)}
            X, sv, X32 = self._layer_fwd(f"{pfx}encoder.layer.{i}.", c, has_cross and i >= c.fusion_layer, X, groups, save, X32=X32, kv_tap=tap,
                                         **xtap)
            tape.append(sv)
        return X, tape, X32

    def stack_bwd(self, pfx, c, layers, tape, dY, groups, dkv_acc=None):
        for i, sv in zip(reversed(list(layers)), reversed(tape)):
            dY = self._layer_bwd(f"{pfx}encoder.layer.{i}.", c, sv, dY, groups, dkv_acc)
            if self.layer_done_cb is not None:
                self._layer_done(f"{pfx}encoder.layer.{i}.")
        return dY

    def _layer_done(self, prefix):
        ws = self._wg_stream if (self._wg_pending and self.wgrad_async) else None
        if ws is None:
            self.wgrad_join()
            return self.layer_done_cb(prefix)
        streams.after(ws, torch.cuda.current_stream())
        with torch.cuda.stream(ws):
            return self.layer_done_cb(prefix)

    def _embed(self, mode, pfx, c, nseq, L, save, salt, **src):
        P, H = self.P, c.hidden_size
        y = self._new(nseq * L, H)
        z = self._new(nseq * L, H) if save else None
        mean, rstd = self._stats(nseq * L, save)
        ops.embed_ln_fwd(mode, y, nseq=nseq, L=L, H=H, pos=P.w(pfx + "embeddings.position_embeddings.weight"),
                         type0=P.w(pfx + "embeddings.token_type_embeddings.weight"), gamma=P.w(pfx + "embeddings.LayerNorm.weight"),
                         beta=P.w(pfx + "embeddings.LayerNorm.bias"), zout=z, mean=mean, rstd=rstd, eps=c.layer_norm_eps,
                         dropout_p=self._p_hidden(c), seed=self.seed, salt=salt, **src)
        return y, LnTape(z, None, mean, rstd, salt)

    def embed_text(self, pfx, c, ids32, nseq, L, save):
        return self._embed(0, pfx, c, nseq, L, save, self._next_salt(), ids=ids32, word=self.P.w(pfx + "embeddings.word_embeddings.weight"))

    def embed_pv(self, pfx, c, prop, mpm_mask, nseq, src_mod, save):
        P = self.P
        return self._embed(1, pfx, c, nseq, self.cfg.n_props + 1, save, self._next_salt(), pv_x=prop, pv_mask=mpm_mask,
                           pv_w=P.w("property_embed.weight"), pv_b=P.w("property_embed.bias"), pv_cls=P.w("property_cls"),
                           pv_masktok=P.w("property_mask"), src_mod=src_mod)

    def embed_generic(self, pfx, c, inputs_embeds_f32, nseq, L):
        return self._embed(2, pfx, c, nseq, L, False, self._next_salt(), pv_x=inputs_embeds_f32)[0]

    def _embed_ln_bwd(self, pfx, c, tape, dY):
        P = self.P
        dz = self._new(*dY.shape)
        ops.ln_bwd(dY, tape.z, tape.mean, tape.rstd, P.w(pfx + "embeddings.LayerNorm.weight"), dz,
                   dgamma=P.g(pfx + "embeddings.LayerNorm.weight"), dbeta=P.g(pfx + "embeddings.LayerNorm.bias"),
                   dropout_p=self._p_hidden(c), seed=self.seed, salt=tape.salt, drop_on_dy=True)
        return dz

    def _transform_fwd(self, dense, norm, X, save, *, eps, r32=False, pre=True):
        P, M, H = self.P, X.shape[0], X.shape[1]
        t = self._new(M, H)
        pre = self._new(M, H) if pre else None
        ops.gemm_nt(X, P.wb(dense + ".weight"), t, bias=P.w(dense + ".bias"), epi=ops.EPI_GELU, C2=pre)
        y = self._new(M, H)
        mean, rstd = self._stats(M, save)
        z = t if save else None
        kw = dict(zout=z, mean=mean, rstd=rstd, eps=eps)
        if r32:
            y32 = self._new(M, H, dtype=torch.float32)
            ops.ln_fwd_r32(t, None, P.w(norm + ".weight"), P.w(norm + ".bias"), y, y32=y32, **kw)
            y = y32
        else:
            ops.ln_fwd(t, None, P.w(norm + ".weight"), P.w(norm + ".bias"), y, **kw)
        return y, HeadTape(dense, norm, X, pre, LnTape(z, y, mean, rstd))

    def _transform_bwd(self, tape, dy):
        P, ln = self.P, tape.ln
        dz = self._new(*dy.shape)
        ops.ln_bwd(dy, ln.z, ln.mean, ln.rstd, P.w(tape.norm + ".weight"), dz, dgamma=P.g(tape.norm + ".weight"), dbeta=P.g(tape.norm + ".bias"))
        dpre = self._gelu_bwd(dz, tape.pre)
        self._wgrad(dpre, tape.X, P.g(tape.dense + ".weight"), P.g(tape.dense + ".bias"))
        return dpre

    def lm_head_fwd(self, pfx, c, X, save):
        P = self.P
        tf = pfx + "cls.predictions.transform."
        y, tape = self._transform_fwd(tf + "dense", tf + "LayerNorm", X, save, eps=c.layer_norm_eps)
        logits = self._new(X.shape[0], c.vocab_size, dtype=torch.float32)
        ops.gemm_nt(y, P.wb(pfx + "cls.predictions.decoder.weight"), logits, bias=P.w(pfx + "cls.predictions.bias"), epi=ops.EPI_F32)
        return logits, tape

    def lm_head_bwd(self, pfx, c, tape, dlogits, out=None):
        P, H, V, M = self.P, c.hidden_size, c.vocab_size, dlogits.shape[0]
        Vp = dlogits.shape[1]
        self._wgrad(dlogits[:, :V], tape.ln.y, P.g(pfx + "bert.embeddings.word_embeddings.weight"), P.g(pfx + "cls.predictions.bias"), inline=True)
        dy = self._new(M, H)
        ops.gemm_nt(dlogits, P.wT_padded(pfx + "cls.decoderT", pfx + "bert.embeddings.word_embeddings.weight", Vp), dy)
        dpre = self._transform_bwd(tape, dy)
        dX = self._new(M, H) if out is None else out
        ops.gemm_nt(dpre, self._wT(pfx + "cls.transform", P.w(pfx + "cls.predictions.transform.dense.weight")), dX)
        return dX

    def _gelu_bwd(self, dz, pre):
        return ops.gelu_bwd(dz, pre)

    def _feat_fwd(self, proj, X, L, B, save, cls_rows=None, X32=None):
        P, E, H = self.P, self.cfg.embed_dim, self.cfg.text.hidden_size
        if cls_rows is not None:
            cls = X.index_select(0, cls_rows)
        else:
            cls = X.view(-1, L * H)[:B, :H]
        raw = self._new(B, E, dtype=torch.float32)
        if X32 is not None:
            cls32 = X32.index_select(0, cls_rows) if cls_rows is not None else X32.view(-1, L * H)[:B, :H]
            ops.rows_linear(cls32, P.w(proj + ".weight"), P.w(proj + ".bias"), raw)
        else:
            ops.gemm_nt(cls, P.wb(proj + ".weight"), raw, bias=P.w(proj + ".bias"), epi=ops.EPI_F32)
        feat = self._new(B, E, dtype=torch.float32)
        nrm = self._new(B, dtype=torch.float32)
        return raw, feat, nrm, cls

    def _banks(self, B):
        if self._bank is not None and self._bank["B"] == B:
            return self._bank
        E, Q = self.cfg.embed_dim, self.cfg.queue_size
        J = B + Q
        Jp = _ceil(J, 64)
        bank = {"B": B, "J": J, "Jp": Jp}
        for nm in ("prop", "text"):
            w3 = torch.zeros(J, 3 * E, dtype=BF, device=self.dev)
            qT = torch.zeros(E, Jp, dtype=BF, device=self.dev)
            ops.queue_shadow(self.P.buffers[nm + "_queue"], w3, qT, Bloc=B)
            bank[nm] = (w3, qT)
        self._bank = bank
        return bank

    def invalidate_banks(self):
        self._bank = None
```

spmm_amd/ops.py:

```python
import ctypes
import os

import torch

from ._lib import lib

EPI_BF16, EPI_GELU, EPI_F32, EPI_F32_ATOMIC, EPI_GELU_GRAD, EPI_F32_ACC, EPI_GELU_DERIV, EPI_MUL = range(8)
BF16 = torch.bfloat16


_DRY_RUN = False
_dry_log = []


def _p(t):
    return None if t is None else ctypes.c_void_p(t.data_ptr())


def _st():
    if _DRY_RUN:
        return None
    return ctypes.c_void_p(torch.cuda.current_stream().cuda_stream)


_DEBUG_SYNC = os.environ.get("SPMM_DEBUG_SYNC") == "1"


def _call(name, *args):
    if not _DRY_RUN:
        if _DEBUG_SYNC:
            import sys
            r = lib().call(name, *args)
            print(f"[launch] {name} {[a for a in args if isinstance(a, int) and not isinstance(a, bool)][:8]}", file=sys.stderr, flush=True)
            torch.cuda.synchronize()
            return r
        return lib().call(name, *args)
    res, argtypes = lib().protos[name]
    if len(args) != len(argtypes):
        raise TypeError(f"{name}: {len(args)} arguments, header declares {len(argtypes)}")
    for i, (a, t) in enumerate(zip(args, argtypes)):
        try:
            t(a) if not isinstance(a, ctypes.c_void_p) else None
        except Exception as e:
            raise TypeError(f"{name}: argument {i} = {a!r} is not a {t.__name__}") from e
        if t is ctypes.c_void_p and not (a is None or isinstance(a, (ctypes.c_void_p, int))):
            raise TypeError(f"{name}: argument {i} must be a pointer, got {type(a)}")
    _dry_log.append(name)


def _row_stride(t):
    assert t.dim() == 2 and (t.stride(1) == 1 or t.shape[1] == 1), (t.shape, t.stride())
    return t.stride(0)


GEMM_AUTO, GEMM_AUTO_TILES = 0, 16
_nt_auto = GEMM_AUTO


class nt_tiles_per_workgroup:

    def __init__(self, on=True):
        self.on = on

    def __enter__(self):
        global _nt_auto
        self._prev = _nt_auto
        if self.on:
            _nt_auto = GEMM_AUTO_TILES
        return self

    def __exit__(self, *exc):
        global _nt_auto
        _nt_auto = self._prev
        return False


def gemm_nt(A, W, C, *, bias=None, epi=EPI_BF16, R=None, G=None, C2=None, alpha=1.0, div=None, splits=1, K=None, colsum=None, kernel=0,
            M_dev=None):
    if kernel == 0:
        kernel = _nt_auto
    M, Ka = A.shape
    N = W.shape[0]
    K = Ka if K is None else K
    assert A.dtype == BF16 and W.dtype == BF16 and W.shape[1] >= K and C.shape[0] >= M and C.shape[1] >= N
    if epi in (EPI_BF16, EPI_GELU, EPI_GELU_GRAD, EPI_GELU_DERIV, EPI_MUL):
        assert C.dtype == BF16
    else:
        assert C.dtype == torch.float32
    _call("spmm_gemm_nt", _p(A), _row_stride(A), _p(W), _row_stride(W), M, N, K, splits, _p(bias), _p(div),
               float(alpha), _p(R), 0 if R is None else _row_stride(R), _p(G), 0 if G is None else _row_stride(G),
               _p(C), _row_stride(C), _p(C2), 0 if C2 is None else _row_stride(C2), epi, _p(colsum), int(kernel), _p(M_dev), _st())
    return C


def gemm_tn(A, B, C, *, alpha=1.0, splits=None, kernel=0, M_dev=None):
    M, N = A.shape
    K = B.shape[1]
    assert A.dtype == BF16 and B.dtype == BF16 and C.dtype == torch.float32 and B.shape[0] == M and tuple(C.shape) == (N, K)
    if splits is None:
        splits = 1 if _DRY_RUN else lib().cdll.spmm_gemm_tn_splits(M, N, K, int(kernel))
    ws = torch.empty(splits * N * K, dtype=torch.float32, device=C.device) if splits > 1 else None
    _call("spmm_gemm_tn", _p(A), _row_stride(A), _p(B), _row_stride(B), M, N, K, splits, float(alpha), _p(C), _row_stride(C), _p(ws),
          int(kernel), _p(M_dev), _st())
    return C


def colsum_bf16(x, out, *, R_dev=None):
    R, C = x.shape
    _call("spmm_colsum_bf16", _p(x), _row_stride(x), R, C, _p(out), _p(R_dev), _st())
    return out


def attn_fwd(Q, K, V, O, lse, *, nseq, nH, Lq, Lkv, kmask=None, causal_from=None, is_cross=False, dropout_p=0.0,
             seed=None, salt=0, kv_seq=None, q_row0=None, q_len=None, kv_row0=None, kv_len=None, q_off=0, kv_off=0):
    cf = nseq if causal_from is None else causal_from
    _call("spmm_attn_fwd", _p(Q), _row_stride(Q), _p(K), _row_stride(K), _p(V), _row_stride(V), _p(kmask), _p(kv_seq), _p(q_row0),
               _p(q_len), _p(kv_row0), _p(kv_len), _p(O),
               _row_stride(O), _p(lse), nseq, nH, Lq, Lkv, cf, int(is_cross), float(dropout_p), _p(seed), salt, int(q_off), int(kv_off), _st())
    return O


def attn_bwd(Q, K, V, O, lse, dO, dQ, dK, dV, *, nseq, nH, Lq, Lkv, kmask=None, causal_from=None, is_cross=False,
             dropout_p=0.0, seed=None, salt=0, kv_seq=None, q_row0=None, q_len=None, kv_row0=None, kv_len=None, q_off=0, kv_off=0,
             d_mode=0, dbuf=None):
    cf = nseq if causal_from is None else causal_from
    _call("spmm_attn_bwd", _p(Q), _row_stride(Q), _p(K), _row_stride(K), _p(V), _row_stride(V), _p(kmask), _p(kv_seq), _p(q_row0),
               _p(q_len), _p(kv_row0), _p(kv_len), _p(O),
               _row_stride(O), _p(lse), _p(dO), _row_stride(dO), _p(dQ), _row_stride(dQ), _p(dK), _row_stride(dK), _p(dV),
               _row_stride(dV), nseq, nH, Lq, Lkv, cf, int(is_cross), float(dropout_p), _p(seed), salt, int(q_off), int(kv_off), int(d_mode),
               _p(dbuf), _st())


def attn_probs(Q, K, *, nseq, nH, Lq, Lkv, kmask=None, kv_seq=None, q_row0=None, q_len=None, kv_row0=None, kv_len=None, mean=True, heads=False,
               P_mean=None, P_heads=None):
    assert Q.dtype == BF16 and K.dtype == BF16 and Q.dim() == 2 and K.dim() == 2
    rows = Q.shape[0]
    if P_mean is None and mean:
        P_mean = torch.zeros(rows, Lkv, dtype=torch.float32, device=Q.device)
    if P_heads is None and heads:
        P_heads = torch.zeros(nH, rows, Lkv, dtype=torch.float32, device=Q.device)
    assert P_mean is not None or P_heads is not None, "attn_probs: nothing requested"
    ldp = None
    if P_mean is not None:
        assert P_mean.dtype == torch.float32 and P_mean.dim() == 2 and P_mean.shape[0] >= rows and P_mean.shape[1] >= Lkv
        ldp = _row_stride(P_mean)
    hs = 0
    if P_heads is not None:
        assert P_heads.dtype == torch.float32 and P_heads.dim() == 3 and tuple(P_heads.shape[:2]) == (nH, rows) and P_heads.shape[2] >= Lkv
        assert P_heads.stride(2) == 1 or P_heads.shape[2] == 1
        assert ldp is None or ldp == P_heads.stride(1), "attn_probs: P_mean and P_heads share one row stride"
        ldp, hs = P_heads.stride(1), P_heads.stride(0)
    _call("spmm_attn_probs", _p(Q), _row_stride(Q), _p(K), _row_stride(K), _p(kmask), _p(kv_seq), _p(q_row0), _p(q_len), _p(kv_row0),
          _p(kv_len), _p(P_mean), _p(P_heads), int(ldp), int(hs), int(nseq), int(nH), int(Lq), int(Lkv), _st())
    return P_mean, P_heads


def xattn_supported(H, nH, Lq, Lkv):
    return bool(_DRY_RUN or lib().cdll.spmm_xattn_supported(int(H), int(nH), int(Lq), int(Lkv)))


def xattn_pack_wo(W, out=None):
    H = W.shape[0]
    assert W.dtype == BF16 and W.shape[1] == H
    out = torch.empty(H * H, dtype=BF16, device=W.device) if out is None else out
    _call("spmm_xattn_pack_wo", _p(W), _row_stride(W), _p(out), H, _st())
    return out


def xattn_fwd(Q, K, V, WoF, bo, R, gamma, beta, Y, *, nseq, nH, Lq, Lkv, eps=1e-12, kmask=None, kv_seq=None, q_row0=None, q_len=None,
              kv_row0=None, kv_len=None, Z=None, mean=None, rstd=None, CTX=None, lse=None, attn_dropout_p=0.0, salt_a=0,
              hidden_dropout_p=0.0, salt_h=0, seed=None, row_base=0):
    _call("spmm_xattn_fwd", _p(Q), _row_stride(Q), _p(K), _row_stride(K), _p(V), _row_stride(V), _p(kmask), _p(kv_seq), _p(q_row0), _p(q_len),
          _p(kv_row0), _p(kv_len), _p(WoF), _p(bo), _p(R), _row_stride(R), _p(gamma), _p(beta), float(eps), _p(Y), _row_stride(Y), _p(Z),
          0 if Z is None else _row_stride(Z), _p(mean), _p(rstd), _p(CTX), 0 if CTX is None else _row_stride(CTX), _p(lse), nseq, nH, Lq, Lkv,
          float(attn_dropout_p), salt_a, float(hidden_dropout_p), salt_h, _p(seed), int(row_base), _st())
    return Y


def ln_fwd(x, res, gamma, beta, y, *, zout=None, mean=None, rstd=None, eps=1e-12, dropout_p=0.0, seed=None, salt=0, rows_dev=None):
    rows, H = x.shape
    _call("spmm_ln_fwd", _p(x), _p(res), _p(gamma), _p(beta), _p(y), _p(zout), _p(mean), _p(rstd), rows, H, float(eps),
               float(dropout_p), _p(seed), salt, _p(rows_dev), _st())
    return y


def ln_fwd_r32(x, res32, gamma, beta, y, *, y32=None, zout=None, mean=None, rstd=None, eps=1e-12, dropout_p=0.0, seed=None, salt=0):
    rows, H = x.shape
    assert res32 is None or res32.dtype == torch.float32
    assert y32 is None or y32.dtype == torch.float32
    _call("spmm_ln_fwd_r32", _p(x), _p(res32), _p(gamma), _p(beta), _p(y), _p(y32), _p(zout), _p(mean), _p(rstd), rows, H, float(eps),
          float(dropout_p), _p(seed), salt, _st())
    return y


def ln_bwd(dy, z, mean, rstd, gamma, dz, *, dy2=None, dx=None, dgamma=None, dbeta=None, dropout_p=0.0, seed=None, salt=0,
           drop_on_dy=False, dxsum=None, rows_dev=None, beta_from_y=None):
    rows, H = dy.shape
    _call("spmm_ln_bwd", _p(dy), _p(dy2), _p(z), _p(mean), _p(rstd), _p(gamma), _p(dz), _p(dx), _p(dgamma), _p(dbeta),
               rows, H, float(dropout_p), _p(seed), salt, int(drop_on_dy), _p(dxsum), _p(rows_dev), _p(beta_from_y), _st())
    return dz


def embed_ln_fwd(mode, y, *, nseq, L, H, pos, type0, gamma, beta, ids=None, word=None, pv_x=None, pv_mask=None, pv_w=None,
                 pv_b=None, pv_cls=None, pv_masktok=None, src_mod=1, zout=None, mean=None, rstd=None, eps=1e-12,
                 dropout_p=0.0, seed=None, salt=0):
    _call("spmm_embed_ln_fwd", mode, _p(ids), _p(word), _p(pos), _p(type0), _p(pv_x), _p(pv_mask), _p(pv_w), _p(pv_b),
               _p(pv_cls), _p(pv_masktok), src_mod, _p(gamma), _p(beta), _p(y), _p(zout), _p(mean), _p(rstd), nseq, L, H,
               float(eps), float(dropout_p), _p(seed), salt, _st())
    return y


def embed_bwd(mode, dz, *, nseq, L, H, dpos, dtype0, ids=None, dword=None, pv_x=None, pv_mask=None, src_mod=1, d_w=None,
              d_b=None, d_cls=None, d_masktok=None):
    _call("spmm_embed_bwd", mode, _p(dz), _p(ids), _p(pv_x), _p(pv_mask), src_mod, _p(dword), _p(dpos), _p(dtype0),
               _p(d_w), _p(d_b), _p(d_cls), _p(d_masktok), nseq, L, H, _st())


def transpose_bf16(x, out, *, Rpad=None, colsum=None):
    R, C = x.shape
    Rpad = out.shape[1] if Rpad is None else Rpad
    _call("spmm_transpose_bf16", _p(x), _row_stride(x), _p(out), _row_stride(out), R, C, Rpad, _p(colsum), _st())
    return out


def cast_transpose(w32, out, outT):
    R, C = w32.shape
    _call("spmm_cast_transpose", _p(w32), _p(out), _p(outT), R, C, _st())


def cast_transpose_multi(descs_dev, ndesc, total_tiles):
    _call("spmm_cast_transpose_multi", _p(descs_dev), ndesc, total_tiles, _st())


def cast_f32_bf16(x, out):
    _call("spmm_cast_f32_bf16", _p(x), _p(out), x.numel(), _st())
    return out


def cast_bf16_f32(x, out):
    _call("spmm_cast_bf16_f32", _p(x), _p(out), x.numel(), _st())
    return out


def acc_rows(dst, src, *, idx=None, atomic=False):
    rows, H = src.shape
    _call("spmm_acc_rows", _p(dst), _row_stride(dst), _p(src), _row_stride(src), _p(idx), rows, H, int(atomic), _st())


def gather_rows(dst, src, idx):
    rows, H = dst.shape
    _call("spmm_gather_rows", _p(dst), _p(src), _p(idx), rows, H, _st())
    return dst


SRC_B = 1 << 40


def gather_rows2(dst, srcA, idx, srcB=None):
    rows, H = dst.shape
    assert idx.dtype == torch.int64 and idx.numel() >= rows and dst.is_contiguous() and srcA.is_contiguous() and (srcB is None or srcB.is_contiguous())
    assert dst.dtype == BF16 and srcA.dtype == BF16 and srcA.shape[1] == H and (srcB is None or (srcB.dtype == BF16 and srcB.shape[1] == H))
    _call("spmm_gather_rows2", _p(dst), _p(srcA), _p(srcB), _p(idx), rows, H, _st())
    return dst


def add_rows_bf16(dst, idx, src):
    rows, H = src.shape
    assert dst.dtype == BF16 and src.dtype == BF16 and idx.dtype == torch.int64 and dst.is_contiguous() and src.is_contiguous() and dst.shape[1] == H
    _call("spmm_add_rows_bf16", _p(dst), _p(idx), _p(src), rows, H, _st())
    return dst


def zero_(t):
    n = t.numel() * t.element_size()
    if n == 0:
        return t
    if not t.is_contiguous():
        es = t.element_size()
        if t.dim() == 2 and t.stride(1) == 1 and (t.shape[1] * es) % 16 == 0 and (t.stride(0) * es) % 16 == 0 and t.data_ptr() % 16 == 0:
            _call("spmm_zero_rows", _p(t), t.shape[0], t.shape[1] * es, t.stride(0) * es, _st())
            return t
        return t.zero_()
    if n % 16 or t.data_ptr() % 16:
        return t.zero_()
    _call("spmm_zero_bytes", _p(t), n, _st())
    return t


def gelu_bwd(dz, pre, out=None):
    assert dz.dtype == BF16 and pre.dtype == BF16 and dz.is_contiguous() and pre.is_contiguous() and dz.shape == pre.shape
    out = torch.empty_like(dz) if out is None else out
    _call("spmm_gelu_bwd", _p(dz), _p(pre), _p(out), dz.numel(), _st())
    return out


def pack_plan(mask32, M, bad):
    B, Lt = mask32.shape
    dev = mask32.device
    alloc = torch.zeros if _DRY_RUN else torch.empty
    i32 = alloc(2 * B, dtype=torch.int32, device=dev)
    i64 = alloc(B + M + (M + B * Lt) + 2 * M + 2 * B * Lt + (B + M), dtype=torch.int64, device=dev)
    o = [0]

    def cut(n):
        o[0] += n
        return i64[o[0] - n:o[0]]
    row0_64, rows, gidx2, gidx4, inv, idx_m = cut(B), cut(M), cut(M + B * Lt), cut(2 * M), cut(2 * B * Lt), cut(B + M)
    _call("spmm_pack_plan", _p(mask32), B, Lt, M, _p(i32[:B]), _p(i32[B:]), _p(row0_64), _p(rows), _p(gidx2), _p(gidx4), _p(inv), _p(idx_m), _p(bad), _st())
    return dict(M=M, rows=rows, row0=i32[B:], row0_64=row0_64, len=i32[:B], gidx2=gidx2, gidx4=gidx4, inv=inv, idx_m=idx_m)


FUSION_SMALL = dict(ar=(0, 1), kvidx_pv=(1, 3), kvidx_tp=(4, 2), qrow0_tp=(6, 2), qlen_tp=(8, 2), row0_8=(10, 1), len_8=(11, 1),
                    skv_row0_pv=(12, 3), skv_len_pv=(15, 3), skv_row0_tx=(18, 2), skv_len_tx=(20, 2), start_t=(22, 2), list_t=(24, 4),
                    start_p=(28, 2), list_p=(30, 4))


def fusion_plan(neg, pk, Lp):
    B = pk["len"].numel()
    Lt = (pk["inv"].numel() // 2) // B
    M, dev = pk["M"], neg.device
    Rcap = 4 * B * Lp + 2 * M + 2 * B * Lt
    ntop = 6 * B + B * Lt + B * Lp
    alloc = torch.zeros if _DRY_RUN else torch.empty
    i64 = alloc(Rcap + B * Lt + ntop, dtype=torch.int64, device=dev)
    idx6, neg_rows, idx_top = i64[:Rcap], i64[Rcap:Rcap + B * Lt], i64[Rcap + B * Lt:]
    small = alloc(35 * B + 2, dtype=torch.int32, device=dev)
    _call("spmm_fusion_plan", _p(neg), _p(pk["len"]), _p(pk["row0"]), B, Lt, Lp, M, _p(idx6), _p(neg_rows), _p(idx_top), _p(small), _st())
    out = dict(idx6=idx6, neg_rows=neg_rows, idx_top=idx_top, Rcap=Rcap, rows_dev=small[34 * B:34 * B + 1], mn_dev=small[34 * B + 1:34 * B + 2])
    for k, (o, n) in FUSION_SMALL.items():
        out[k] = small[o * B:(o + n) * B]
    out["start_t"], out["start_p"] = out["start_t"][:B + 1], out["start_p"][:B + 1]
    return out


def l2norm_fwd(x, y, nrm, *, a3=None, w3=None, yT=None):
    rows, E = y.shape
    _call("spmm_l2norm_fwd", _p(x), _row_stride(x), _p(y), _p(nrm), _p(a3), _p(w3), _p(yT),
               0 if yT is None else _row_stride(yT), rows, E, _st())


def l2norm_bwd(dy, y, nrm, dx, *, gscale=None):
    rows, E = y.shape
    _call("spmm_l2norm_bwd", _p(dy), _p(y), _p(nrm), _p(gscale), _p(dx), rows, E, _st())


def ita_rows(S, SM, dS, *, B, J, alpha, temp, losses, slot, dtemp, nan_flag=None):
    nrows = S.shape[0]
    _call("spmm_ita_rows", _p(S), _p(SM), _row_stride(S), nrows, B, J, _p(alpha), _p(temp), _p(dS), _row_stride(dS),
               dS.shape[1], _p(losses), slot, _p(dtemp), _p(nan_flag), _st())


def sample_neg(S, B, out, *, forced=None, seed=None, salt=0, offset=0):
    _call("spmm_sample_neg", _p(S), _row_stride(S), B, _p(forced), _p(seed), salt, _p(out), offset, _st())


def lm_loss(logits, logits_m, ids, *, nseq, L, V, alpha, ws, losses, slot, dlogits=None, gscale=None):
    _call("spmm_lm_loss", _p(logits), _p(logits_m), _row_stride(logits), _p(ids), nseq, L, V, _p(alpha), _p(ws),
               _p(gscale), _p(dlogits), 0 if dlogits is None else _row_stride(dlogits),
               V if dlogits is None else dlogits.shape[1], _p(losses), slot, _st())


def s2s_loss(logits, ids, *, nseq, L, V, ws, losses, slot, row_of=None, dlogits=None, gscale=None):
    rows = logits.shape[0]
    assert logits.dtype == torch.float32 and logits.dim() == 2 and logits.shape[1] >= V and ids.dtype == torch.int32 and ids.numel() == nseq * L
    assert ids.is_contiguous() and ws.dtype == torch.int32 and ws.numel() >= 4 and losses.dtype == torch.float32
    assert row_of is None or (row_of.dtype == torch.int64 and row_of.numel() >= rows and row_of.is_contiguous())
    assert row_of is not None or rows == nseq * L
    assert dlogits is None or (dlogits.dtype == BF16 and dlogits.dim() == 2 and dlogits.shape[0] == rows)
    _call("spmm_s2s_loss", _p(logits), _row_stride(logits), _p(ids), _p(row_of), rows, nseq, L, V, _p(ws), _p(gscale), _p(dlogits),
          0 if dlogits is None else _row_stride(dlogits), V if dlogits is None else dlogits.shape[1], _p(losses), slot, _st())


LM_SCORE_MAXV = 512


def lm_score(y, Wd, bias, ids, *, nseq, L, row_of=None, seq_row0=None, seq_len=None, tok_lp=None, seq_lp=None, seq_n=None):
    rows, H = y.shape
    V = Wd.shape[0]
    dev = y.device
    assert y.dtype == BF16 and Wd.dtype == BF16 and Wd.shape[1] >= H and y.stride(1) == 1 and Wd.stride(1) == 1
    assert bias.dtype == torch.float32 and bias.numel() == V and bias.is_contiguous()
    assert ids.dtype == torch.int32 and ids.numel() == nseq * L and ids.is_contiguous()
    assert row_of is None or (row_of.dtype == torch.int64 and row_of.numel() >= rows and row_of.is_contiguous())
    assert (seq_row0 is None) == (seq_len is None)
    assert seq_row0 is None or all(t.dtype == torch.int32 and t.numel() == nseq and t.is_contiguous() for t in (seq_row0, seq_len))
    tok_lp = torch.empty(rows, dtype=torch.float32, device=dev) if tok_lp is None else tok_lp
    seq_lp = torch.empty(nseq, dtype=torch.float32, device=dev) if seq_lp is None else seq_lp
    seq_n = torch.empty(nseq, dtype=torch.int32, device=dev) if seq_n is None else seq_n
    assert tok_lp.dtype == torch.float32 and tok_lp.numel() == rows and tok_lp.is_contiguous()
    assert seq_lp.dtype == torch.float32 and seq_lp.numel() == nseq and seq_lp.is_contiguous()
    assert seq_n.dtype == torch.int32 and seq_n.numel() == nseq and seq_n.is_contiguous()
    _call("spmm_lm_score", _p(y), _row_stride(y), _p(Wd), _row_stride(Wd), _p(bias), _p(ids), _p(row_of), rows, nseq, L, V, H, _p(seq_row0),
          _p(seq_len), _p(tok_lp), _p(seq_lp), _p(seq_n), _st())
    return tok_lp, seq_lp, seq_n


def itm_head(xa, stride_a, xb, stride_b, H, W, bias, *, n, B, losses, slot, logits=None, dxa=None, dxb=None, dW=None,
             db=None, gscale=None):
    do_bwd = dxa is not None
    assert xa.dtype == xb.dtype and xa.dtype in (BF16, torch.float32)
    _call("spmm_itm_head", _p(xa), stride_a, _p(xb), stride_b, H, _p(W), _p(bias), n, B, _p(gscale), _p(losses), slot,
               _p(logits), _p(dxa), _p(dxb), _p(dW), _p(db), int(do_bwd), int(xa.dtype == torch.float32), _st())

# ... 36 lines not shown
    assert xcache is None or (xcache.dtype == BF16 and tuple(xcache.shape) == (rows, n_props + 1, H) and xcache.is_contiguous())
    assert pos is None or (pos.dtype == torch.float32 and pos.is_contiguous() and pos.shape[0] >= n_props + 1 and pos.shape[1] == H)
    _call("spmm_s2p_append", _p(y), _row_stride(y), _p(w3), _p(b3), _p(pe_w), _p(pe_b), _p(pos), _p(type0), _p(gamma), _p(beta), float(eps),
          _p(pred), _row_stride(pred), _p(xcache), rows, H, int(n_props), int(i), _st())
    return pred


def rows_linear(x, W, bias, out, *, act=0):
    rows, K = x.shape
    N = W.shape[0]
    assert W.dtype == torch.float32 and W.is_contiguous() and W.shape[1] == K and out.dtype == torch.float32 and tuple(out.shape) == (rows, N)
    assert x.dtype in (torch.float32, BF16) and x.stride(1) == 1
    _call("spmm_rows_linear", _p(x), int(x.dtype == BF16), _row_stride(x), _p(W), _p(bias), _p(out), _row_stride(out), rows, N, K, int(act), _st())
    return out


SIM_TOPK_MAXK = 64


def sim_topk_workspace(Q, n, k, device):
    nbytes = 16 if _DRY_RUN else lib().cdll.spmm_sim_topk_workspace_bytes(int(Q), int(n), int(k))
    return torch.empty(max(16, nbytes), dtype=torch.uint8, device=device)


def sim_topk(q, f, scores, index, *, base=0, merge=False, cut=None, ws=None):
    Q, E = q.shape
    n = f.shape[0]
    k = scores.shape[1]
    assert q.dtype == torch.float32 and f.dtype == torch.float32 and (n == 0 or f.shape[1] == E)
    assert scores.dtype == torch.float32 and index.dtype == torch.int64 and tuple(scores.shape) == tuple(index.shape) == (Q, k)
    assert scores.is_contiguous() and index.is_contiguous()
    cs, ci = (None, None) if cut is None else cut
    assert cut is None or (cs.dtype == torch.float32 and ci.dtype == torch.int64 and cs.numel() == ci.numel() == Q and cs.is_contiguous() and ci.is_contiguous())
    if ws is None and n > 0:
        ws = sim_topk_workspace(Q, n, k, q.device)
    _call("spmm_sim_topk", _p(q), _row_stride(q), _p(f) if n > 0 else None, _row_stride(f) if n > 0 else E, int(base), Q, n, E, k, _p(scores),
          _p(index), int(bool(merge)), _p(cs), _p(ci), _p(ws), 0 if ws is None else ws.numel(), _st())
    return scores, index


def centroid_assign(f, c, best, assign, *, c0=0, merge=False, prev=None, changed=None):
    n, E = f.shape
    Kc = c.shape[0]
    assert f.dtype == torch.float32 and c.dtype == torch.float32 and c.shape[1] == E
    assert best.dtype == torch.float32 and assign.dtype == torch.int32 and best.numel() == assign.numel() == n
    assert best.is_contiguous() and assign.is_contiguous()
    assert (prev is None) == (changed is None)
    assert prev is None or (prev.dtype == torch.int32 and prev.numel() == n and prev.is_contiguous() and changed.dtype == torch.int32
                            and prev.data_ptr() != assign.data_ptr())
    _call("spmm_centroid_assign", _p(f) if n > 0 else None, _row_stride(f) if n > 0 else E, _p(c), _row_stride(c), int(c0), n, Kc, E, _p(best),
          _p(assign), int(bool(merge)), _p(prev), _p(changed), _st())
    return best, assign


def cluster_group(assign, K, counts, offsets, members, outside, ws=None):
    n = assign.numel()
    assert assign.dtype == torch.int32 and assign.is_contiguous() and counts.dtype == torch.int32 and counts.numel() == K and counts.is_contiguous()
    assert offsets.dtype == torch.int64 and offsets.numel() == K + 1 and offsets.is_contiguous()
    assert members.dtype == torch.int32 and members.numel() == n and members.is_contiguous() and outside.dtype == torch.int32
    if ws is None:
        ws = cluster_group_workspace(n, K, counts.device)
    _call("spmm_cluster_group", _p(assign) if n > 0 else None, n, int(K), _p(counts), _p(offsets), _p(members) if n > 0 else None, _p(outside),
          _p(ws), ws.numel(), _st())
    return counts, offsets, members


def cluster_group_workspace(n, K, device):
    nbytes = 16 if _DRY_RUN else lib().cdll.spmm_cluster_group_workspace_bytes(int(n), int(K))
    return torch.empty(max(16, nbytes), dtype=torch.uint8, device=device)


def cluster_centroids_workspace(n, K, E, device):
    nbytes = 16 if _DRY_RUN else lib().cdll.spmm_cluster_centroids_workspace_bytes(int(n), int(K), int(E))
    return torch.empty(max(16, nbytes), dtype=torch.uint8, device=device)


def cluster_centroids(f, best, counts, offsets, members, centres, norm, medoid, ws=None):
    n, E = f.shape
    K = counts.numel()
    assert f.dtype == torch.float32 and best.dtype == torch.float32 and best.numel() == n and best.is_contiguous()
    assert counts.dtype == torch.int32 and offsets.dtype == torch.int64 and offsets.numel() == K + 1 and members.dtype == torch.int32
    assert members.numel() == n and counts.is_contiguous() and offsets.is_contiguous() and members.is_contiguous()
    assert centres.dtype == torch.float32 and tuple(centres.shape) == (K, E) and norm.dtype == torch.float32 and norm.numel() == K
    assert medoid.dtype == torch.int32 and medoid.numel() == K and norm.is_contiguous() and medoid.is_contiguous()
    if ws is None:
        ws = cluster_centroids_workspace(n, K, E, f.device)
    _call("spmm_cluster_centroids", _p(f) if n > 0 else None, _row_stride(f) if n > 0 else E, n, E, _p(best) if n > 0 else None, _p(counts),
          _p(offsets), _p(members) if n > 0 else None, K, _p(centres), _row_stride(centres), _p(norm), _p(medoid), _p(ws), ws.numel(), _st())
    return centres, norm, medoid


def enqueue(feats, queue, w3, qT, ptr, *, Bloc, advance=True, skip_flag=None):
    n, E = feats.shape
    _call("spmm_enqueue", _p(feats), n, E, _p(queue), queue.shape[1], _p(w3), _p(qT), _row_stride(qT), Bloc, _p(ptr),
               int(advance), _p(skip_flag), _st())


def queue_shadow(queue, w3, qT, *, Bloc):
    E, Q = queue.shape
    _call("spmm_queue_shadow", _p(queue), E, Q, _p(w3), _p(qT), _row_stride(qT), Bloc, _st())


def clamp_scalar(p, lo, hi):
    _call("spmm_clamp_scalar", _p(p), float(lo), float(hi), _st())


def adam_scalars_bytes():
    return lib().cdll.spmm_adam_scalars_bytes()


_sqn_ws = {}


def grad_sqnorm(g, out):
    ws = _sqn_ws.get(g.device)
    if ws is None:
        nbytes = 4096 if _DRY_RUN else lib().cdll.spmm_grad_sqnorm_workspace_bytes()
        ws = _sqn_ws[g.device] = torch.zeros(nbytes // 4, dtype=torch.float32, device=g.device)
    _call("spmm_grad_sqnorm", _p(g), g.numel(), _p(out), _p(ws), _st())


def adamw_step(p, g, m, v, shadow, *, lr, beta1=0.9, beta2=0.999, eps=1e-8, weight_decay=0.02, normsq, max_norm=5.0, step,
               nan_flag=None, scalars):
    _call("spmm_adamw_step", _p(p), _p(g), _p(m), _p(v), _p(shadow), p.numel(), _p(lr), beta1, beta2, eps, weight_decay,
               _p(normsq), max_norm, _p(step), _p(nan_flag), _p(scalars), _st())


def ema_update(pm, p, shadow, momentum):
    _call("spmm_ema_update", _p(pm), _p(p), _p(shadow), pm.numel(), float(momentum), _st())


def axpy_scalar(dst, src, *, scale_ptr=None, scale=1.0):
    _call("spmm_axpy_scalar", _p(dst), _p(src), _p(scale_ptr), float(scale), dst.numel(), _st())


def embed_step_ln_fwd(ids32, pos_index, y, *, word, pos, type0, gamma, beta, eps=1e-12, pos_ptr=None):
    rows, H = y.shape
    assert ids32.dtype == torch.int32 and ids32.numel() == rows and y.dtype == BF16
    _call("spmm_embed_step_ln_fwd", _p(ids32), int(pos_index), _p(pos_ptr), _p(word), _p(pos), _p(type0), _p(gamma), _p(beta), _p(y), rows, H,
          float(eps), _st())
    return y


def decode_attn(q, K, V, out, *, nH, Lkv, seq_stride, tok_stride, head_stride=64, anc=None, kv_div=1, group=1, scale=0.125, t_ptr=None, knew=None, vnew=None,
                rowmap=None):
    R = q.shape[0]
    assert q.dtype == BF16 and K.dtype == BF16 and V.dtype == BF16 and out.dtype == BF16
    assert anc is None or (anc.dtype == torch.int32 and anc.shape[0] == R)
    assert (knew is None) == (vnew is None) and (knew is None or (knew.dtype == BF16 and vnew.dtype == BF16 and _row_stride(knew) == _row_stride(vnew)))
    _call("spmm_decode_attn", _p(q), _row_stride(q), _p(K), _p(V), int(seq_stride), int(tok_stride), int(head_stride), _p(anc),
          0 if anc is None else _row_stride(anc), int(kv_div), int(group), _p(out), _row_stride(out), R, nH, Lkv, float(scale), _p(t_ptr),
          _p(knew), _p(vnew), 0 if knew is None else _row_stride(knew), _p(rowmap), _st())
    return out


def decode_xattn(q, K, V, out, *, nH, kv_row0, kv_len, Lkv_max, kv_seq=None, group=1, scale=0.125):
    R = q.shape[0]
    assert q.dtype == BF16 and K.dtype == BF16 and V.dtype == BF16 and out.dtype == BF16 and _row_stride(K) == _row_stride(V)
    assert kv_row0.dtype == torch.int32 and kv_len.dtype == torch.int32 and kv_row0.numel() == kv_len.numel()
    assert kv_row0.is_contiguous() and kv_len.is_contiguous()
    assert kv_seq is None or (kv_seq.dtype == torch.int32 and kv_seq.is_contiguous() and kv_seq.numel() * group == R)
    assert kv_seq is not None or kv_len.numel() * group >= R
    _call("spmm_decode_xattn", _p(q), _row_stride(q), _p(K), _p(V), _row_stride(K), _p(kv_seq), _p(kv_row0), _p(kv_len), int(group), _p(out),
          _row_stride(out), R, nH, int(Lkv_max), float(scale), _st())
    return out


def beam_step(logits, book, *, t=0, t_ptr=None, t_off=0, anc=None, ids_out=None, parent_out=None, rowmap=None, noise=None, need=None):
    _, k, L = book.tokens.shape
    mol = getattr(book, "mol", None)
    N = book.tokens.shape[0] if mol is None else mol.numel()
    assert logits.dtype == torch.float32 and logits.dim() == 2 and logits.shape[0] == N * k and logits.stride(1) == 1
    assert (mol is None or mol.dtype == torch.int32) and (rowmap is None or (rowmap.dtype == torch.int32 and rowmap.numel() == N * k))
    assert book.tokens.dtype == torch.int32 and book.fin_tok.dtype == torch.int32 and book.fin_len.dtype == torch.int32 and book.fin_n.dtype == torch.int32
    assert book.tokens.is_contiguous() and book.fin_tok.is_contiguous() and book.cur_p.is_contiguous() and book.fin_p.is_contiguous()
    assert anc is None or (anc.dtype == torch.int32 and anc.shape[0] == N * k and anc.stride(1) == 1)
    if ids_out is None:
        ids_out = torch.empty(N * k, dtype=torch.int32, device=logits.device)
    args = (_p(logits), logits.stride(0), N, k, logits.shape[1], L, book.F, int(t), _p(t_ptr), int(t_off), _p(book.tokens),
            _p(book.cur_p), _p(book.fin_p), _p(book.fin_len), _p(book.fin_tok), _p(book.fin_n), _p(book.done), _p(anc),
            0 if anc is None else anc.stride(0), _p(ids_out), _p(parent_out), _p(book.n_done), _p(mol), _p(rowmap))
    until = need is not None
    need = int(getattr(book, "need", k) if need is None else need)
    if until or need != k:
        assert noise is None, "the sampled search ends at k finals"
        _call("spmm_beam_step_until", *args, need, _st())
    elif noise is None:
        _call("spmm_beam_step", *args, _st())
    else:
        assert noise.dtype == torch.float32 and noise.dim() == 2 and noise.stride(1) == 1 and noise.device == logits.device
        assert noise.shape[0] == N * k and noise.shape[1] >= logits.shape[1], (noise.shape, logits.shape)
        _call("spmm_beam_step_sampled", *args, _p(noise), noise.stride(0), _st())
    return ids_out


def gumbel_noise(seed, N, k, V, Lmax, *, salt=0, t=0, t_ptr=None, t_off=0, mol=None, mol_base=0, out=None):
    assert seed.dtype == torch.int64 and seed.numel() == 1
    assert mol is None or (mol.dtype == torch.int32 and mol.numel() == N and mol.is_contiguous())
    if out is None:
        out = torch.empty(N * k, V, dtype=torch.float32, device=seed.device)
    assert out.dtype == torch.float32 and out.dim() == 2 and out.shape[0] == N * k and out.shape[1] >= V and out.stride(1) == 1
    _call("spmm_gumbel_noise", _p(seed), int(salt), N, k, V, Lmax, int(t), _p(t_ptr), int(t_off), _p(mol), int(mol_base), _p(out), out.stride(0), _st())
    return out


SBS_MAXW = 1024


def sbs_step(logits, noise, book, *, t=0, t_ptr=None, t_off=0, ids_out=None, parent_out=None):
    cur, nxt = book.cur, book.nxt
    G, W, L = cur["tokens"].shape
    assert logits.dtype == torch.float32 and logits.dim() == 2 and logits.shape[0] == G * W and logits.stride(1) == 1
    V = logits.shape[1]
    assert noise.dtype == torch.float32 and noise.dim() == 2 and noise.stride(1) == 1 and noise.device == logits.device
    assert noise.shape[0] == G * W and noise.shape[1] >= V, (noise.shape, logits.shape)
    for s in (cur, nxt):
        assert s["phi"].dtype == torch.float32 and s["gum"].dtype == torch.float32 and s["fin"].dtype == torch.uint8
        assert s["len"].dtype == torch.int32 and s["tokens"].dtype == torch.int32 and s["anc"].dtype == torch.int32
        assert all(s[f].is_contiguous() for f in ("phi", "gum", "fin", "len", "tokens")) and s["anc"].stride(1) == 1
        assert s["anc"].shape[0] == G * W and s["anc"].shape[1] >= L
    assert cur["anc"].stride(0) == nxt["anc"].stride(0)
    if ids_out is None:
        ids_out = torch.empty(G * W, dtype=torch.int32, device=logits.device)
    if book.ws is None or book.ws.numel() < 2 * G * W * V:
        book.ws = torch.empty(2 * G * W * V, dtype=torch.int32, device=logits.device)
    _call("spmm_sbs_step", _p(logits), logits.stride(0), _p(noise), noise.stride(0), G, W, V, L, int(t), _p(t_ptr), int(t_off),
          _p(cur["phi"]), _p(cur["gum"]), _p(cur["fin"]), _p(cur["len"]), _p(cur["tokens"]), _p(cur["anc"]),
          _p(nxt["phi"]), _p(nxt["gum"]), _p(nxt["fin"]), _p(nxt["len"]), _p(nxt["tokens"]), _p(nxt["anc"]), cur["anc"].stride(0),
          _p(ids_out), _p(parent_out), _p(book.open), _p(book.ws), _st())
    return ids_out


def logit_warp(lc, lu=None, *, w=1.0, temperature=1.0, top_k=0, top_p=1.0, min_keep=1, out=None):
    assert lc.dtype == torch.float32 and lc.dim() == 2 and (lc.stride(1) == 1 or lc.shape[1] == 1)
    R, V = lc.shape
    if lu is not None:
        assert lu.dtype == torch.float32 and lu.shape == lc.shape and lu.device == lc.device and (R <= 1 or lu.stride(0) == lc.stride(0))
        assert lu.stride(1) == 1 or V == 1
    if out is None:
        out = lc
    assert out.dtype == torch.float32 and out.shape == lc.shape and out.device == lc.device and (out.stride(1) == 1 or V == 1)
    _call("spmm_logit_warp", _p(lc), _p(lu), lc.stride(0), R, V, float(w), float(temperature), int(top_k), float(top_p), int(min_keep),
          _p(out), out.stride(0), _st())
    return out


SYNTAX_MASKED = -1e30


def smiles_mask(logits, tokens, table, *, t=0, t_last, k=1, mol=None, Lmax=None, logits2=None, t_ptr=None, t_off=0, state_out=None):
    assert logits.dtype == torch.float32 and logits.dim() == 2 and (logits.stride(1) == 1 or logits.shape[1] == 1)
    R, V = logits.shape
    if logits2 is not None:
        assert logits2.dtype == torch.float32 and logits2.shape == logits.shape and logits2.device == logits.device
        assert (R <= 1 or logits2.stride(0) == logits.stride(0)) and (logits2.stride(1) == 1 or V == 1)
    assert tokens.dtype == torch.int32 and tokens.dim() in (2, 3) and tokens.stride(-1) == 1
    if tokens.dim() == 3:
        assert tokens.is_contiguous() and tokens.shape[1] == k
        tokens = tokens.view(-1, tokens.shape[2])
    if Lmax is None:
        Lmax = tokens.shape[1]
    assert tokens.shape[1] >= (t if t_ptr is None else t_last), (tokens.shape, t, t_last)
    assert table.dtype == torch.int32 and tuple(table.shape) == (V, 4) and table.is_contiguous() and table.device == logits.device
    assert mol is None or (mol.dtype == torch.int32 and mol.is_contiguous() and mol.numel() * k == R)
    assert state_out is None or (state_out.dtype == torch.int32 and tuple(state_out.shape) == (R, 4) and state_out.is_contiguous())
    _call("spmm_smiles_mask", _p(logits), _p(logits2), logits.stride(0), R, V, _p(tokens), tokens.stride(0), tokens.shape[0], int(k), _p(mol),
          int(Lmax), int(t), _p(t_ptr), int(t_off), int(t_last), _p(table), _p(state_out), _st())
    return logits


WORDPIECE_TABLE_MAX, WORDPIECE_CHARS_MAX, WORDPIECE_HEAD_MAX = 8192, 256, 16


def wordpiece(blob, offsets, table, head, ids, lens, status, *, gap, max_chars, max_pieces, unk_id, sep_id, pad_id):
    assert blob.dtype == torch.uint8 and blob.dim() == 1 and blob.is_contiguous()
    assert offsets.dtype == torch.int64 and offsets.dim() == 1 and offsets.is_contiguous() and offsets.numel() >= 1
    N = offsets.numel() - 1
    assert head.dtype == torch.uint8 and head.dim() == 1 and head.is_contiguous() and head.numel() <= WORDPIECE_HEAD_MAX
    assert table.dtype == torch.int32 and table.dim() == 1 and table.is_contiguous() and table.numel() <= WORDPIECE_TABLE_MAX
    assert ids.dtype == torch.int32 and ids.dim() == 2 and ids.shape[0] == N and ids.shape[1] >= max_pieces + 1
    assert all(t.dtype == torch.int32 and tuple(t.shape) == (N,) and t.is_contiguous() for t in (lens, status))
    assert all(t.device == ids.device for t in (blob, offsets, table, head, lens, status))
    assert 1 <= max_chars <= WORDPIECE_CHARS_MAX and max_pieces >= 1 and gap in (0, 1)
    _call("spmm_wordpiece", _p(blob), _p(offsets), N, int(gap), _p(head), head.numel(), _p(table), table.numel(), int(max_chars),
          int(max_pieces), int(unk_id), int(sep_id), int(pad_id), _p(ids), _row_stride(ids), _p(lens), _p(status), _st())
    return ids


def kv_prefill(K, V, row0, length, dst_row, Kc, Vc):
    R, nH, Lmax, dh = Kc.shape
    assert K.dtype == BF16 and V.dtype == BF16 and Kc.dtype == BF16 and Vc.dtype == BF16 and dh == 64
    assert K.shape == V.shape and K.shape[1] == nH * 64 and _row_stride(K) == _row_stride(V)
    assert Kc.is_contiguous() and Vc.is_contiguous() and Vc.shape == Kc.shape
    E = row0.numel()
    assert all(t.dtype == torch.int32 and t.numel() == E and t.is_contiguous() and t.device == Kc.device for t in (row0, length, dst_row))
    _call("spmm_kv_prefill", _p(K), _p(V), _row_stride(K), K.shape[0], _p(row0), _p(length), _p(dst_row), E, _p(Kc), _p(Vc), R, nH, Lmax, _st())


def segment_sum_bf16(src, start, lst, out):
    U, W = out.shape
    assert src.dtype == BF16 and out.dtype == BF16 and src.shape[1] == W and src.is_contiguous() and out.is_contiguous()
    assert start.dtype == torch.int32 and lst.dtype == torch.int32 and start.numel() == U + 1
    _call("spmm_segment_sum_bf16", _p(src), _p(start), _p(lst), _p(out), U, W, _st())
    return out


ATTN_MAXL = 256


def _chunks(L, step=128):
    return [(o, min(step, L - o)) for o in range(0, L, step)]


def attn_fwd_long(Q, K, V, O, lse, *, nseq, nH, Lq, Lkv, kmask=None, causal_from=None, is_cross=False, dropout_p=0.0, seed=None,
                  salt=0, kv_seq=None, q_row0=None, q_len=None, kv_row0=None, kv_len=None):
    if Lq <= ATTN_MAXL and Lkv <= ATTN_MAXL:
        return attn_fwd(Q, K, V, O, lse, nseq=nseq, nH=nH, Lq=Lq, Lkv=Lkv, kmask=kmask, causal_from=causal_from, is_cross=is_cross,
                        dropout_p=dropout_p, seed=seed, salt=salt, kv_seq=kv_seq, q_row0=q_row0, q_len=q_len, kv_row0=kv_row0, kv_len=kv_len)
    if q_row0 is not None or kv_row0 is not None:
        raise ValueError("packed layouts are limited to %d-token sequences" % ATTN_MAXL)
    dev, H = Q.device, nH * 64
    nsrc = K.shape[0] // Lkv
    ar_q = torch.arange(nseq, dtype=torch.int32, device=dev)
    ar_k = torch.arange(nsrc, dtype=torch.int32, device=dev)
    Ov = O.view(nseq, Lq, nH, 64)
    for qi, (q0, ql) in enumerate(_chunks(Lq)):
        q_row0, q_len = ar_q * Lq + q0, torch.full((nseq,), ql, dtype=torch.int32, device=dev)
        outs, lses = [], []
        for ci, (k0, kl) in enumerate(_chunks(Lkv)):
            Oc = torch.empty(nseq * Lq, H, dtype=BF16, device=dev)
            lc = torch.empty(nseq, nH, ql, dtype=torch.float32, device=dev)
            attn_fwd(Q, K, V, Oc, lc, nseq=nseq, nH=nH, Lq=ql, Lkv=kl, kmask=None if kmask is None else kmask[:, k0:k0 + kl].contiguous(),
                     causal_from=causal_from, is_cross=is_cross, dropout_p=dropout_p, seed=seed, salt=salt + 7919 * (qi * 8 + ci + 1),
                     kv_seq=kv_seq, q_row0=q_row0, q_len=q_len, kv_row0=ar_k * Lkv + k0,
                     kv_len=torch.full((nsrc,), kl, dtype=torch.int32, device=dev), q_off=q0, kv_off=k0)
            outs.append(Oc.view(nseq, Lq, nH, 64)[:, q0:q0 + ql].float())
            lses.append(lc)
        L = torch.stack(lses)
        tot = torch.logsumexp(L, dim=0)
        acc = sum(o * torch.exp(l - tot).permute(0, 2, 1)[..., None] for o, l in zip(outs, lses))
        Ov[:, q0:q0 + ql] = acc.to(BF16)
        if lse is not None:
            lse[:, :, q0:q0 + ql] = tot
    return O


def attn_bwd_long(Q, K, V, O, lse, dO, dQ, dK, dV, *, nseq, nH, Lq, Lkv, kmask=None, causal_from=None, is_cross=False, dropout_p=0.0,
                  seed=None, salt=0, kv_seq=None, q_row0=None, q_len=None, kv_row0=None, kv_len=None):
    if Lq <= ATTN_MAXL and Lkv <= ATTN_MAXL:
        return attn_bwd(Q, K, V, O, lse, dO, dQ, dK, dV, nseq=nseq, nH=nH, Lq=Lq, Lkv=Lkv, kmask=kmask, causal_from=causal_from,
                        is_cross=is_cross, dropout_p=dropout_p, seed=seed, salt=salt, kv_seq=kv_seq, q_row0=q_row0, q_len=q_len,
                        kv_row0=kv_row0, kv_len=kv_len)
    if q_row0 is not None or kv_row0 is not None:
        raise ValueError("packed layouts are limited to %d-token sequences" % ATTN_MAXL)
    dev, H = Q.device, nH * 64
    nsrc = K.shape[0] // Lkv
    nkv_out = nseq if kv_seq is not None else nsrc
    ar_q = torch.arange(nseq, dtype=torch.int32, device=dev)
    ar_k = torch.arange(nsrc, dtype=torch.int32, device=dev)
    dQ32 = torch.zeros(nseq, Lq, H, dtype=torch.float32, device=dev)
    dK32 = torch.zeros(nkv_out, Lkv, H, dtype=torch.float32, device=dev)
    dV32 = torch.zeros(nkv_out, Lkv, H, dtype=torch.float32, device=dev)
    for qi, (q0, ql) in enumerate(_chunks(Lq)):
        q_row0, q_len = ar_q * Lq + q0, torch.full((nseq,), ql, dtype=torch.int32, device=dev)
        lse_i = lse[:, :, q0:q0 + ql].contiguous()
        calls = []
        for ci, (k0, kl) in enumerate(_chunks(Lkv)):
            calls.append(dict(nseq=nseq, nH=nH, Lq=ql, Lkv=kl, kmask=None if kmask is None else kmask[:, k0:k0 + kl].contiguous(),
                              causal_from=causal_from, is_cross=is_cross, dropout_p=dropout_p, seed=seed,
                              salt=salt + 7919 * (qi * 8 + ci + 1), kv_seq=kv_seq, q_row0=q_row0, q_len=q_len, kv_row0=ar_k * Lkv + k0,
                              kv_len=torch.full((nsrc,), kl, dtype=torch.int32, device=dev), q_off=q0, kv_off=k0))
        dQc = torch.empty(nseq * Lq, H, dtype=BF16, device=dev)
        D = torch.zeros(nseq, nH, ql, dtype=torch.float32, device=dev)
        for (k0, kl), kw in zip(_chunks(Lkv), calls):
            Dc = torch.empty_like(D)
            tmp = torch.empty((nseq if kv_seq is not None else nsrc) * (kl if kv_seq is not None else Lkv), H, dtype=BF16, device=dev)
            attn_bwd(Q, K, V, O, lse_i, dO, dQc, tmp, tmp, d_mode=1, dbuf=Dc, **kw)
            D += Dc
        for (k0, kl), kw in zip(_chunks(Lkv), calls):
            if kv_seq is not None:
                dKc = torch.zeros(nseq * kl, H, dtype=BF16, device=dev); dVc = torch.zeros_like(dKc)
            else:
                dKc = torch.zeros(nsrc * Lkv, H, dtype=BF16, device=dev); dVc = torch.zeros_like(dKc)
            attn_bwd(Q, K, V, O, lse_i, dO, dQc, dKc, dVc, d_mode=2, dbuf=D, **kw)
            dQ32[:, q0:q0 + ql] += dQc.view(nseq, Lq, H)[:, q0:q0 + ql].float()
            if kv_seq is not None:
                dK32[:, k0:k0 + kl] += dKc.view(nseq, kl, H).float(); dV32[:, k0:k0 + kl] += dVc.view(nseq, kl, H).float()
            else:
                dK32[:, k0:k0 + kl] += dKc.view(nsrc, Lkv, H)[:, k0:k0 + kl].float(); dV32[:, k0:k0 + kl] += dVc.view(nsrc, Lkv, H)[:, k0:k0 + kl].float()
    dQ.copy_(dQ32.view(nseq * Lq, H))
    dK.copy_(dK32.view(nkv_out * Lkv, H))
    dV.copy_(dV32.view(nkv_out * Lkv, H))
```

spmm_amd/options.py:

```python
from __future__ import annotations

import dataclasses
import os
from dataclasses import dataclass

_ENV = {
    "pack_text": ("SPMM_PACK_TEXT", lambda s: s != "0"),
    "cls_only_top": ("SPMM_CLS_ONLY_TOP", lambda s: s != "0"),
    "multi_stream": ("SPMM_STREAMS", lambda s: s != "1"),
    "wgrad_stream": ("SPMM_WGRAD_STREAM", lambda s: s != "0"),
    "pv_wgrad_inline": ("SPMM_PV_WGRAD_INLINE", int),
    "ln_from_y": ("SPMM_LN_FROM_Y", lambda s: s != "0"),
    "resid_fp32": ("SPMM_RESID_FP32", lambda s: s == "1"),
    "fused_xattn": ("SPMM_FUSED_XATTN", lambda s: {"0": "off", "1": "all"}.get(s, s)),
    "grad_overlap": ("SPMM_GRAD_OVERLAP", lambda s: s != "0"),
    "grad_wire": ("SPMM_GRAD_WIRE", str),
    "nt_under_comm": ("SPMM_NT_UNDER_COMM", str),
    "force_dist": ("SPMM_FORCE_DIST", lambda s: s == "1"),
    "dp_four_streams": ("SPMM_DP_FOUR_STREAMS", lambda s: s != "0"),
    "probe_streams": ("SPMM_PROBE_STREAMS", lambda s: s != "0"),
    "schedule_check": ("SPMM_SCHEDULE_CHECK", lambda s: s != "0"),
}


@dataclass
class EngineOptions:
    pack_text: bool = True
    cls_only_top: bool = True
    multi_stream: bool = True
    wgrad_stream: bool = True
    pv_wgrad_inline: int = 4
    ln_from_y: bool = True
    fused_xattn: str = "nograd"
    resid_fp32: bool = False
    grad_overlap: bool = True
    grad_wire: str = "fp32"
    nt_under_comm: str = "auto"
    force_dist: bool = False
    dp_four_streams: bool = True
    schedule_check: bool = True
    probe_streams: bool = False

    @classmethod
    def from_env(cls, **overrides) -> "EngineOptions":
        kw = {}
        for field, (var, parse) in _ENV.items():
            if var in os.environ:
                kw[field] = parse(os.environ[var])
        kw.update(overrides)
        o = cls(**kw)
        if isinstance(o.fused_xattn, bool):
            o.fused_xattn = "all" if o.fused_xattn else "off"
        if o.fused_xattn not in ("off", "nograd", "all"):
            raise ValueError(f"fused_xattn must be off, nograd or all, not {o.fused_xattn!r}")
        if o.grad_wire not in ("fp32", "bf16"):
            raise ValueError(f"grad_wire must be fp32 or bf16, not {o.grad_wire!r}")
        if o.nt_under_comm not in ("tiles", "persistent", "auto"):
            raise ValueError(f"nt_under_comm must be tiles, persistent or auto, not {o.nt_under_comm!r}")
        return o

    def replace(self, **kw) -> "EngineOptions":
        return dataclasses.replace(self, **kw)
```

spmm_amd/params.py:

```python
from __future__ import annotations

import math
import struct
from typing import Dict, List, Optional

import torch

from . import ops
from .config import SPMMConfig, is_buffer, momentum_twin, state_spec, student_of

ALIGN = 64


def ct_descriptor_table(pairs):
    blob, tile0 = b"", 0
    for src, dstT in pairs:
        R, C = src.shape
        ntr, ntc = (R + 63) // 64, (C + 63) // 64
        blob += struct.pack("<QQiiii", src.data_ptr(), dstT.data_ptr(), R, C, tile0, ntc)
        tile0 += ntr * ntc
    assert len(blob) == len(pairs) * 32
    return blob, tile0


def _layout_order(spec) -> List[str]:
    names = [n for n, _, k in spec if not is_buffer(n) and student_of(n) is None and k not in ("tied_w", "tied_b")]
    done, out = set(), []
    for n in names:
        if n in done:
            continue
        if n.endswith(".self.query.weight"):
            base = n[:-len("query.weight")]
            grp = [base + f"{x}.{y}" for y in ("weight", "bias") for x in ("query", "key", "value")]
            out += grp
            done.update(grp)
        else:
            out.append(n)
            done.add(n)
    assert sorted(out) == sorted(names)
    return out


class ParamStore:
    def __init__(self, cfg: SPMMConfig, device, train: bool = True, spec=None):
        self.cfg, self.device, self.train = cfg, device, train
        twins = spec is None
        self.spec = state_spec(cfg) if twins else list(spec)
        self.shape = {n: s for n, s, _ in self.spec}
        self.kind = {n: k for n, _, k in self.spec}
        self.order = _layout_order(self.spec)
        self.offset: Dict[str, int] = {}
        off = 0
        for n in self.order:
            self.offset[n] = off
            numel = int(math.prod(self.shape[n])) if self.shape[n] else 1
            off += (numel + ALIGN - 1) // ALIGN * ALIGN
        self.total = off
        f32 = dict(dtype=torch.float32, device=device)
        self.flat = torch.zeros(self.total, **f32)
        self.flat_m = torch.zeros(self.total if twins else 0, **f32)
        self.shadow = torch.zeros(self.total, dtype=torch.bfloat16, device=device)
        self.shadow_m = torch.zeros(self.total if twins else 0, dtype=torch.bfloat16, device=device)
        if train:
            self.grad = torch.zeros(self.total, **f32)
            self.adam_m = torch.zeros(self.total, **f32)
            self.adam_v = torch.zeros(self.total, **f32)
        H, E, Q = cfg.text.hidden_size, cfg.embed_dim, cfg.queue_size
        self.buffers: Dict[str, torch.Tensor] = {}
        for n, s, k in self.spec:
            if k == "posid":
                self.buffers[n] = torch.arange(s[1], device=device).expand(1, -1).clone()
            elif k == "queue":
                self.buffers[n] = torch.zeros(s, **f32)
            elif k == "ptr":
                self.buffers[n] = torch.zeros(1, dtype=torch.long, device=device)
        self._wT: Dict[str, torch.Tensor] = {}
        self._wT_pad: Dict[str, str] = {}
        self._wF: Dict[str, tuple] = {}

    def _resolve(self, name: str):
        st = student_of(name)
        mom = st is not None
        base = st if mom else name
        if self.kind.get(base) == "tied_w":
            base = base.replace("cls.predictions.decoder.weight", "bert.embeddings.word_embeddings.weight")
        elif self.kind.get(base) == "tied_b":
            base = base.replace("cls.predictions.decoder.bias", "cls.predictions.bias")
        return mom, base

    def _view(self, buf: torch.Tensor, base: str, shape=None):
        shape = self.shape[base] if shape is None else shape
        n = int(math.prod(shape)) if shape else 1
        return buf[self.offset[base]: self.offset[base] + n].view(shape)

    def w(self, name: str) -> torch.Tensor:
        mom, base = self._resolve(name)
        return self._view(self.flat_m if mom else self.flat, base)

    def wb(self, name: str) -> torch.Tensor:
        mom, base = self._resolve(name)
        return self._view(self.shadow_m if mom else self.shadow, base)

    def g(self, name: str) -> torch.Tensor:
        mom, base = self._resolve(name)
        assert not mom
        return self._view(self.grad, base)

    def fused(self, prefix: str, names, kind: str, what: str = "wb") -> torch.Tensor:
        first = f"{prefix}{names[0]}.{kind}"
        mom, base = self._resolve(first)
        shp = self.shape[base]
        rows = sum(self.shape[self._resolve(f"{prefix}{n}.{kind}")[1]][0] for n in names)
        o = self.offset[base]
        for n in names:
            b = self._resolve(f"{prefix}{n}.{kind}")[1]
            assert self.offset[b] == o, (b, self.offset[b], o)
            o += int(math.prod(self.shape[b]))
        buf = {"wb": self.shadow_m if mom else self.shadow, "w": self.flat_m if mom else self.flat,
               "g": None if mom else getattr(self, "grad", None)}[what]
        full = (rows,) + tuple(shp[1:])
        return buf[self.offset[base]: self.offset[base] + int(math.prod(full))].view(full)

    def wT(self, key: str, src: Optional[torch.Tensor] = None) -> torch.Tensor:
        if key not in self._wT:
            assert src is not None
            R, C = src.shape
            self._wT[key] = torch.empty(C, R, dtype=torch.bfloat16, device=self.device)
            self._wT_src = getattr(self, "_wT_src", {})
            self._wT_src[key] = src
            ops.cast_transpose(src, None, self._wT[key])
        return self._wT[key]

    def wT_padded(self, key: str, name: str, cols: int) -> torch.Tensor:
        if key not in self._wT:
            self._wT[key] = torch.zeros(self.w(name).shape[1], cols, dtype=torch.bfloat16, device=self.device)
            self._wT_pad[key] = name
            self.refresh_padded_shadows()
        return self._wT[key]

    def refresh_padded_shadows(self):
        for key, name in self._wT_pad.items():
            w = self.w(name)
            self._wT[key][:, :w.shape[0]].copy_(w.t())

    def wF(self, name: str) -> torch.Tensor:
        if name not in self._wF:
            src = self.wb(name)
            self._wF[name] = (src, torch.empty(src.numel(), dtype=torch.bfloat16, device=self.device), student_of(name) is not None)
            ops.xattn_pack_wo(src, self._wF[name][1])
        return self._wF[name][1]

    def refresh_frag(self, momentum: bool):
        for src, out, mom in self._wF.values():
            if mom == momentum:
                ops.xattn_pack_wo(src, out)

    def refresh_shadows(self, transposed_only: bool = False, part: str = "all"):
        if not transposed_only:
            ops.cast_f32_bf16(self.flat, self.shadow)
            if self.flat_m.numel():
                ops.cast_f32_bf16(self.flat_m, self.shadow_m)
        if part in ("all", "forward"):
            self.refresh_frag(False)
            if not transposed_only:
                self.refresh_frag(True)
        if part == "forward":
            return
        srcs = getattr(self, "_wT_src", {})
        if not srcs:
            return
        if getattr(self, "_ct_n", -1) != len(srcs):
            blob, tiles = ct_descriptor_table([(src, self._wT[key]) for key, src in srcs.items()])
            self._ct_desc = torch.frombuffer(bytearray(blob), dtype=torch.uint8).to(self.device)
            self._ct_n, self._ct_tiles = len(srcs), tiles
        ops.cast_transpose_multi(self._ct_desc, self._ct_n, self._ct_tiles)

    def copy_params(self):
        self.flat_m.copy_(self.flat)
        self.shadow_m.copy_(self.shadow)

    def named_tensors(self):
        for n, _, _ in self.spec:
            yield n, (self.buffers[n] if n in self.buffers else self.w(n))

    def load_state_dict(self, sd: Dict[str, torch.Tensor], strict: bool = True):
        missing = [n for n, _, _ in self.spec if n not in sd]
        unexpected = [k for k in sd if k not in self.shape]
        bad = [k for k in sd if k in self.shape and tuple(sd[k].shape) != tuple(self.shape[k]) and sd[k].numel() != int(math.prod(self.shape[k]) if self.shape[k] else 1)]
        if bad:
            raise RuntimeError(f"size mismatch for {bad[:5]}")
        if strict and (missing or unexpected):
            raise KeyError(f"state_dict mismatch: missing {missing[:5]} unexpected {unexpected[:5]}")
        with torch.no_grad():
            for n, t in self.named_tensors():
                if n in sd:
                    if self.kind[n] in ("tied_w", "tied_b"):
                        continue
                    t.copy_(sd[n].to(t.device).reshape(t.shape))
        self.refresh_shadows()
        return missing, unexpected
```

spmm_amd/step.py:

```python
from __future__ import annotations

from typing import Callable, Optional, Tuple

import torch

from . import ops, streams
from .engine import STREAM_TOKENS_MAX, BF, LOSS_ITA, LOSS_ITM, LOSS_MLM, LOSS_MPM, Batch, Engine, Group, KVSource, SelfKV, _ceil


class PretrainStep(Engine):
    def _s6_forward_cls(self, B, Lt, M, pk, mask32, neg, y1, y2, prop_embeds, text_embeds, save):
        cfg = self.cfg
        ct = cfg.text
        H, Lp, f, n = ct.hidden_size, cfg.n_props + 1, ct.fusion_layer, ct.num_hidden_layers
        fp = ops.fusion_plan(neg, pk, Lp)
        o_tp = 3 * B * Lp
        o_lm = o_tp + 2 * M
        o_12 = o_lm + B * Lt
        o_8 = o_12 + B * Lp
        Rcap = fp["Rcap"]
        X6 = ops.gather_rows2(self._new(Rcap, H), y1, fp["idx6"], y2)
        src_pv = KVSource(prop_embeds.view(B * Lp, H), B, Lp).preset(4 * B, fp["start_p"], fp["list_p"])
        src_text = KVSource(text_embeds, B, Lt, row0=pk["row0"], length=pk["len"], pack_idx=pk["rows"]).preset(4 * B, fp["start_t"], fp["list_t"])
        ar = fp["ar"]
        g_lo = Batch([Group(0, 3 * B, Lp, None, 3 * B).bind(src_text, fp["kvidx_pv"], 0),
                      Group(o_tp, 2 * B, Lt, None, 2 * B, q_row0=fp["qrow0_tp"], q_len=fp["qlen_tp"], nrows=2 * M).bind(src_pv, fp["kvidx_tp"], 0),
                      Group(o_lm, B, Lt, mask32, 0).bind(src_pv, ar, 2 * B),
                      Group(o_12, B, Lp, None, 0).bind(src_text, ar, 3 * B),
                      Group(o_8, B, Lt, None, B, q_row0=fp["row0_8"], q_len=fp["len_8"], nrows=B * Lt).bind(src_pv, ar, 3 * B)],
                     rows_dev=fp["rows_dev"])
        y, tape_lo, _ = self.stack_fwd("text_encoder.bert.", ct, range(f, n - 1), True, X6, g_lo, save)
        ntop = 6 * B + B * Lt + B * Lp
        Xtop = ops.gather_rows2(self._new(ntop, H), y, fp["idx_top"])
        skv_a = SelfKV(y[:o_lm])
        skv_b = SelfKV(y[o_8:], rows_dev=fp["mn_dev"])
        g_top = Batch([Group(0, 3 * B, 1, None, 3 * B, self_src=skv_a, skv_row0=fp["skv_row0_pv"], skv_len=fp["skv_len_pv"], skv_L=Lp).bind(src_text, fp["kvidx_pv"], 0),
                       Group(3 * B, 2 * B, 1, None, 2 * B, self_src=skv_a, skv_row0=fp["skv_row0_tx"], skv_len=fp["skv_len_tx"], skv_L=Lt).bind(src_pv, fp["kvidx_tp"], 0),
                       Group(5 * B, B, 1, None, B, self_src=skv_b, skv_row0=fp["row0_8"], skv_len=fp["len_8"], skv_L=Lt).bind(src_pv, ar, 3 * B),
                       Group(6 * B, B, Lt, mask32, 0).bind(src_pv, ar, 2 * B),
                       Group(6 * B + B * Lt, B, Lp, None, 0).bind(src_text, ar, 3 * B)])
        ytop, sv_top, _ = self._layer_fwd(f"text_encoder.bert.encoder.layer.{n - 1}.", ct, True, Xtop, g_top, save)
        return dict(fp=fp, ytop=ytop, sv_top=sv_top, g_top=g_top, skv=(skv_a, skv_b), g_lo=g_lo, tape_lo=tape_lo, src_text=src_text, src_pv=src_pv,
                    o_tp=o_tp, o_lm=o_lm, o_12=o_12, o_8=o_8, ntop=ntop, Rcap=Rcap)

    def _s6_backward_cls(self, T, dYtop, d_pe, d_te):
        S6, B, Lt, M = T["S6"], T["B"], T["Lt"], T["M"]
        cfg = self.cfg
        ct = cfg.text
        H, Lp, f, n = ct.hidden_size, cfg.n_props + 1, ct.fusion_layer, ct.num_hidden_layers
        fp, o_lm, o_8 = S6["fp"], S6["o_lm"], S6["o_8"]
        dkv_acc = {id(S6["src_text"]): d_te[:M], id(S6["src_pv"]): d_pe.view(B * Lp, H)}
        dX6 = self._new(S6["Rcap"], H)
        S6["skv"][0].dx = dX6[:o_lm]
        S6["skv"][1].dx = dX6[o_8:]
        dXtop = self._layer_bwd(f"text_encoder.bert.encoder.layer.{n - 1}.", ct, S6["sv_top"], dYtop, S6["g_top"], dkv_acc)
        if self.layer_done_cb is not None:
            self._layer_done(f"text_encoder.bert.encoder.layer.{n - 1}.")
        ops.add_rows_bf16(dX6, fp["idx_top"][:6 * B], dXtop[:6 * B])
        dX6[o_lm:o_8].copy_(dXtop[6 * B:])
        return self.stack_bwd("text_encoder.bert.", ct, range(f, n - 1), S6["tape_lo"], dX6, S6["g_lo"], dkv_acc=dkv_acc)

    def forward(self, prop: torch.Tensor, ids: torch.Tensor, mask: torch.Tensor, *, mpm_mask: Optional[torch.Tensor] = None,
                neg_idx: Optional[Tuple[torch.Tensor, torch.Tensor]] = None, gather: Optional[Callable] = None,
                save: bool = True, aux: Optional[dict] = None, n_tokens: Optional[int] = None) -> torch.Tensor:
        cfg, P = self.cfg, self.P
        ct, cp = cfg.text, cfg.prop
        H, E, Lp, f, n = ct.hidden_size, cfg.embed_dim, cfg.n_props + 1, ct.fusion_layer, ct.num_hidden_layers
        B, Lt = ids.shape
        if B % 4 or cfg.queue_size % 4:
            raise ValueError("batch size and queue size must be multiples of 4")
        self._salt = 0
        if self.train_mode:
            self.seed.add_(1)
        ops.zero_(self.step_zero)
        temp = P.w("temp").view(1)
        ops.clamp_scalar(temp, 0.01, 0.5)
        ids32 = ids.to(torch.int32).contiguous()
        mask32 = mask.to(torch.int32).contiguous()
        prop = prop.to(torch.float32).contiguous()
        if mpm_mask is None:
            mpm_mask = (torch.rand(B, cfg.n_props, device=self.dev) < 0.5).to(torch.float32)
        mpm_mask = mpm_mask.to(torch.float32).contiguous()

        self._one_stream = self.force_one_stream or B * Lt > STREAM_TOKENS_MAX
        pk = self._pack_plan(mask32, B, Lt, n_tokens) if (self.pack_text and aux is None and Lt <= ops.ATTN_MAXL) else None
        if n_tokens is not None:
            self.nan_flag.bitwise_or_(self.hint_bad)
        M = pk["M"] if pk else B * Lt
        ids2 = torch.cat([ids32, ids32])
        r32 = self.opt.resid_fp32 and aux is None
        f32 = (lambda t: t.float()) if r32 else (lambda t: None)
        side = self._fork()
        with self._on(side):
            x2, esv2 = self.embed_text("text_encoder.bert.", ct, ids2, 2 * B, Lt, save)
            x2_32 = f32(x2)
            if pk:
                x2d = x2
                x2 = ops.gather_rows2(self._new(M + B * Lt, H), x2d, pk["gidx2"])
                if r32:
                    x2_32 = torch.cat([x2_32[:B * Lt].index_select(0, pk["rows"]), x2_32[B * Lt:]])
                g2 = Batch([Group(0, B, Lt, None, B, q_row0=pk["row0"], q_len=pk["len"], nrows=M), Group(M, B, Lt, mask32, 0)])
            else:
                g2 = Batch([Group(0, 2 * B, Lt, torch.cat([mask32, mask32]), B)])
            y2, tape2, y2_32 = self.stack_fwd("text_encoder.bert.", ct, range(0, f), True, x2, g2, save, X32=x2_32)
            text_embeds, hidden10 = y2[:M], y2[M:]
            text_embeds_32, hidden10_32 = (y2_32[:M], y2_32[M:]) if r32 else (None, None)
        side_m = self._fork(1)
        ema_done = None
        with self._on(side_m):
            ops.ema_update(P.flat_m, P.flat, P.shadow_m, cfg.momentum)
            P.refresh_frag(True)
            if side_m is not None:
                ema_done = streams.mark(side_m)
            x4, _ = self.embed_text("text_encoder_m.bert.", ct, ids2, 2 * B, Lt, False)
            x4_32 = f32(x4)
            if pk:
                x4d = x4
                x4 = ops.gather_rows2(self._new(2 * M, H), x4d, pk["gidx4"])
                if r32:
                    x4_32 = torch.cat([x4_32[:B * Lt].index_select(0, pk["rows"]), x4_32[B * Lt:].index_select(0, pk["rows"])])
                g4 = Batch([g2.groups[0], Group(M, B, Lt, None, 0, q_row0=pk["row0"], q_len=pk["len"], nrows=M)])
            else:
                g4 = g2
            cls_m = bool(pk) and self.opt.cls_only_top and not r32 and f >= 1
            if cls_m:
                y4, _, _ = self.stack_fwd("text_encoder_m.bert.", ct, range(0, f - 1), True, x4, g4, False)
                x4t = ops.gather_rows2(self._new(B + M, H), y4, pk["idx_m"])
                g4t = Batch([Group(0, B, 1, None, B, self_src=SelfKV(y4[:M]), skv_row0=pk["row0"], skv_len=pk["len"], skv_L=Lt),
                             Group(B, B, Lt, None, 0, q_row0=pk["row0"], q_len=pk["len"], nrows=M)])
                y4t, _, _ = self._layer_fwd(f"text_encoder_m.bert.encoder.layer.{f - 1}.", ct, False, x4t, g4t, False)
                text_embeds_m, hidden9 = y4t[:B], y4t[B:]
            else:
                y4, _, y4_32 = self.stack_fwd("text_encoder_m.bert.", ct, range(0, f), True, x4, g4, False, X32=x4_32)
                text_embeds_m, hidden9 = y4[:M], y4[M:]
            text_embeds_m_32, hidden9_32 = (y4_32[:M], y4_32[M:]) if r32 else (None, None)
        x1, esv1 = self.embed_pv("property_encoder.", cp, prop, mpm_mask, 2 * B, B, save)
        g1 = Batch([Group(0, 2 * B, Lp, None, B)])
        y1, tape1, y1_32 = self.stack_fwd("property_encoder.", cp, range(cp.num_hidden_layers), False, x1, g1, save, X32=f32(x1))
        prop_embeds, prop_embeds_causal = y1[:B * Lp], y1[B * Lp:]
        prop_embeds_32, prop_embeds_causal_32 = (y1_32[:B * Lp], y1_32[B * Lp:]) if r32 else (None, None)
        if ema_done is not None:
            torch.cuda.current_stream().wait_event(ema_done)
        x3, _ = self.embed_pv("property_encoder_m.", cp, prop, mpm_mask, B, B, False)
        prop_embeds_m, _, prop_embeds_m_32 = self.stack_fwd("property_encoder_m.", cp, range(cp.num_hidden_layers), False, x3,
                                                            Batch([Group(0, B, Lp, None, B)]), False, X32=f32(x3))
        self._join(side)
        self._join(side_m)
        if pk:
            g5 = Batch([Group(0, B, Lt, None, 0, kv=prop_embeds_m, Lkv=Lp, kv_mask=None, q_row0=pk["row0"], q_len=pk["len"], nrows=M)])
        else:
            g5 = Batch([Group(0, B, Lt, mask32, 0, kv=prop_embeds_m, Lkv=Lp, kv_mask=None)])
        side5 = self._fork()
        with self._on(side5):
            y5, _, _ = self.stack_fwd("text_encoder_m.bert.", ct, range(f, n), True, hidden9, g5, False, X32=hidden9_32)
            logits_m, _ = self.lm_head_fwd("text_encoder_m.", ct, y5, False)
            if pk:
                V_ = logits_m.shape[1]
                if V_ % 4 == 0:
                    dense = torch.empty(B * Lt, V_, dtype=logits_m.dtype, device=self.dev)
                    ops.gather_rows2(dense.view(BF), logits_m.view(BF), pk["inv"])
                    logits_m = dense
                else:
                    logits_m = torch.zeros(B * Lt, V_, dtype=logits_m.dtype, device=self.dev).index_copy_(0, pk["rows"], logits_m)

        bank = self._banks(B)
        J, Jp = bank["J"], bank["Jp"]
        A3 = self._new(4 * B, 3 * E)
        feats = {}
        twins = {"property_proj": prop_embeds_32, "text_proj": text_embeds_32, "property_proj_m": prop_embeds_m_32, "text_proj_m": text_embeds_m_32}
        for k, (proj, X, L, w3, qT) in enumerate((("property_proj", prop_embeds, Lp, None, None),
                                                  ("text_proj", text_embeds, Lt, None, None),
                                                  ("property_proj_m", prop_embeds_m, Lp, *bank["prop"]),
                                                  ("text_proj_m", text_embeds_m, Lt, *bank["text"]))):
            if proj == "text_proj_m" and cls_m:
                raw, feat, nrm, cls = self._feat_fwd(proj, X, 1, B, save, X32=None)
            else:
                raw, feat, nrm, cls = self._feat_fwd(proj, X, L, B, save, cls_rows=pk["row0_64"] if (pk and proj.startswith("text_proj")) else None,
                                                     X32=twins[proj])
            ops.l2norm_fwd(raw, feat, nrm, a3=A3[k * B:(k + 1) * B], w3=None if w3 is None else w3[:B], yT=qT)
            feats[proj] = (feat, nrm, cls)
        S_text = self._new(4 * B, J, dtype=torch.float32)
        S_prop = self._new(4 * B, J, dtype=torch.float32)
        ops.gemm_nt(A3, bank["text"][0], S_text, epi=ops.EPI_F32, div=temp)
        ops.gemm_nt(A3, bank["prop"][0], S_prop, epi=ops.EPI_F32, div=temp)
        dS_text, dS_prop = self._new(2 * B, Jp), self._new(2 * B, Jp)
        for S, dS in ((S_text, dS_text), (S_prop, dS_prop)):
            ops.ita_rows(S[:2 * B], S[2 * B:], dS, B=B, J=J, alpha=self.alpha, temp=temp, losses=self.losses, slot=LOSS_ITA,
                         dtemp=self.dtemp_ita, nan_flag=self.nan_flag)
        dfeat = None
        if save:
            dfeat = self._zeros(2 * B, E, dtype=torch.float32)
            sp = max(1, min(Jp // 64, 16))
            ops.gemm_nt(dS_text, bank["text"][1], dfeat, epi=ops.EPI_F32_ATOMIC, splits=sp, div=temp)
            ops.gemm_nt(dS_prop, bank["prop"][1], dfeat, epi=ops.EPI_F32_ATOMIC, splits=sp, div=temp)

        neg = self._zeros(2 * B, dtype=torch.int64)
        fp, ft = (None, None) if neg_idx is None else (neg_idx[0].to(torch.int64).contiguous(), neg_idx[1].to(torch.int64).contiguous())
        ops.sample_neg(S_prop[B:2 * B], B, neg[:B], forced=fp, seed=self.seed, salt=self._next_salt())
        ops.sample_neg(S_text[:B], B, neg[B:], forced=ft, seed=self.seed, salt=self._next_salt())

        cls_top = bool(pk) and self.opt.cls_only_top and not r32 and aux is None
        if cls_top:
            S6 = self._s6_forward_cls(B, Lt, M, pk, mask32, neg, y1, y2, prop_embeds, text_embeds, save)
            ytop = S6["ytop"]
            ops.itm_head(ytop[:3 * B], H, ytop[3 * B:6 * B], H, H, P.w("itm_head.weight"), P.w("itm_head.bias"), n=3 * B, B=B, losses=self.losses,
                         slot=LOSS_ITM, logits=None)
            ytext = hid10_cls = ytop[6 * B:6 * B + B * Lt]
            ypv = ypv_h = ytop
            hp12_cls = ytop[6 * B + B * Lt:]
            src_text = src_pv = neg_rows = cls_text = itm_text = g6 = tape6 = None
            Mn = B * Lt
        else:
            pe = prop_embeds.view(B, Lp * H)
            pe_neg = ops.gather_rows(self._new(B, Lp * H), pe, neg[:B])
            ar = torch.arange(B, dtype=torch.int64, device=self.dev)
            mask_neg = mask32.index_select(0, neg[B:])
            qpv = torch.cat([pe, pe_neg, pe, prop_embeds_causal.view(B, Lp * H)]).view(4 * B * Lp, H)
            if r32:
                pe32 = prop_embeds_32.view(B, Lp * H)
                qpv_32 = torch.cat([pe32, pe32.index_select(0, neg[:B]), pe32, prop_embeds_causal_32.view(B, Lp * H)]).view(4 * B * Lp, H)
            src_pv = KVSource(prop_embeds.view(B * Lp, H), B, Lp)
            if pk:
                src_text = KVSource(text_embeds, B, Lt, row0=pk["row0"], length=pk["len"], pack_idx=pk["rows"])
                neg_rows = pk["row0_64"].index_select(0, neg[B:])[:, None] + torch.arange(Lt, device=self.dev)[None, :]
                neg_rows = torch.where(mask_neg.bool(), neg_rows, torch.full_like(neg_rows, M)).view(-1)
                r0 = 4 * B * Lp
                Mn = B * Lt
                te_neg = torch.cat([text_embeds, self._zeros(1, H)]).index_select(0, neg_rows)
                qtext = torch.cat([text_embeds, text_embeds, te_neg, hidden10])
                if r32:
                    te_neg_32 = torch.cat([text_embeds_32, self._zeros(1, H, dtype=torch.float32)]).index_select(0, neg_rows)
                    qtext_32 = torch.cat([text_embeds_32, text_embeds_32, te_neg_32, hidden10_32])
                gt = [Group(r0, 2 * B, Lt, None, 2 * B, q_row0=torch.cat([pk["row0"], pk["row0"] + M]), q_len=torch.cat([pk["len"], pk["len"]]),
                            nrows=2 * M).attend(src_pv, torch.cat([ar, neg[:B]])),
                      Group(r0 + 2 * M, 2 * B, Lt, torch.cat([mask_neg, mask32]), B).attend(src_pv, torch.cat([ar, ar]))]
                cls_text = torch.cat([pk["row0_64"], pk["row0_64"] + M, 2 * M + ar * Lt])
                kvmask_qpv = None
            else:
                src_text = KVSource(text_embeds, B, Lt)
                te = text_embeds.view(B, Lt * H)
                te_neg = ops.gather_rows(self._new(B, Lt * H), te, neg[B:])
                qtext = torch.cat([te, te, te_neg, hidden10.view(B, Lt * H)]).view(4 * B * Lt, H)
                if r32:
                    te32 = text_embeds_32.view(B, Lt * H)
                    qtext_32 = torch.cat([te32, te32, te32.index_select(0, neg[B:]), hidden10_32.view(B, Lt * H)]).view(4 * B * Lt, H)
                kvmask_qpv = torch.cat([mask32, mask32, mask_neg, mask32])
                gt = [Group(4 * B * Lp, 4 * B, Lt, kvmask_qpv, 3 * B).attend(src_pv, torch.cat([ar, neg[:B], ar, ar]))]
                neg_rows, cls_text, Mn = None, torch.arange(3 * B, dtype=torch.int64, device=self.dev) * Lt, B * Lt
            X6 = torch.cat([qpv, qtext])
            g6 = Batch([Group(0, 4 * B, Lp, None, 3 * B, kv_mask=kvmask_qpv).attend(src_text, torch.cat([ar, ar, neg[B:], ar]))] + gt)
            src_text.finalize()
            src_pv.finalize()
            y6, tape6, y6_32 = self.stack_fwd("text_encoder.bert.", ct, range(f, n), True, X6, g6, save, X32=torch.cat([qpv_32, qtext_32]) if r32 else None)
            ypv, ytext = y6[:4 * B * Lp], y6[4 * B * Lp:]
            ypv_h, ytext_h = (y6_32[:4 * B * Lp], y6_32[4 * B * Lp:]) if r32 else (ypv, ytext)

            vl_logits = self._new(3 * B, 2, dtype=torch.float32) if aux is not None else None
            itm_text = ytext_h.index_select(0, cls_text)
            ops.itm_head(ypv_h, Lp * H, itm_text, H, H, P.w("itm_head.weight"), P.w("itm_head.bias"), n=3 * B, B=B, losses=self.losses,
                         slot=LOSS_ITM, logits=vl_logits)

        feat_pm, feat_tm = feats["property_proj_m"][0], feats["text_proj_m"][0]
        if gather is not None:
            g = gather(torch.cat([feat_pm, feat_tm, self.nan_flag.to(torch.float32).expand(B, 1)], 1))
            feat_pm, feat_tm = g[:, :E].contiguous(), g[:, E:2 * E].contiguous()
            self.nan_flag.copy_((g[:, 2 * E].abs().sum() > 0).to(torch.int32).view(1))
        ptr = P.buffers["queue_ptr"]
        ops.enqueue(feat_pm, P.buffers["prop_queue"], *bank["prop"], ptr, Bloc=B, advance=False, skip_flag=self.nan_flag)
        ops.enqueue(feat_tm, P.buffers["text_queue"], *bank["text"], ptr, Bloc=B, advance=True, skip_flag=self.nan_flag)

        self._join(side5)
        hid10 = hid10_cls if cls_top else ytext[ytext.shape[0] - B * Lt:]
        logits, lmsv = self.lm_head_fwd("text_encoder.", ct, hid10, save)
        ops.lm_loss(logits, logits_m, ids32, nseq=B, L=Lt, V=ct.vocab_size, alpha=self.alpha, ws=self.icount[0:4], losses=self.losses,
                    slot=LOSS_MLM)

        hp12 = hp12_cls if cls_top else ypv[3 * B * Lp:]
        mln_h, mpmsv = self._transform_fwd("property_mtr_head.0", "property_mtr_head.2", hp12, True, eps=ct.layer_norm_eps, r32=r32)
        pred = self._new(B, cfg.n_props, dtype=torch.float32) if aux is not None else None
        ops.mpm_head(mln_h, Lp, H, P.w("property_mtr_head.3.weight"), P.w("property_mtr_head.3.bias"), prop, mpm_mask, B=B,
                     ws=self.icount[4:8], losses=self.losses, slot=LOSS_MPM, pred=pred)

        if aux is not None:
            aux.update(prop_embeds=prop_embeds, text_embeds=text_embeds, prop_embeds_m=prop_embeds_m, text_embeds_m=text_embeds_m,
                       prop_feat=feats["property_proj"][0], text_feat=feats["text_proj"][0], prop_feat_m=feats["property_proj_m"][0],
                       text_feat_m=feats["text_proj_m"][0], sim_i2t=S_text[:B], sim_t2i=S_prop[B:2 * B], sim_i2t_m=S_text[2 * B:3 * B],
                       vl_output=vl_logits, mlm_output=logits.view(B, Lt, -1)[:, :-1], logits_m=logits_m.view(B, Lt, -1)[:, :-1],
                       pred=pred, prop_neg_idx=neg[:B], text_neg_idx=neg[B:], mpm_mask=mpm_mask,
                       prop_embeds_causal=prop_embeds_causal)
        if save:
            self.tape = dict(B=B, Lt=Lt, pk=pk, M=M, Mn=Mn, src_text=src_text, src_pv=src_pv, neg_rows=neg_rows, cls_text=cls_text, itm_text=itm_text,
                             prop=prop, mpm_mask=mpm_mask, ids32=ids32, ids2=ids2, esv1=esv1, g1=g1, tape1=tape1,
                             esv2=esv2, g2=g2, tape2=tape2, feats=feats, dfeat=dfeat, neg=neg, g6=g6, tape6=tape6, ypv=ypv_h,
                             ytext=ytext, logits=logits, logits_m=logits_m, lmsv=lmsv, mpmsv=mpmsv, S6=S6 if cls_top else None)
        return self.losses[:4]

    def backward(self):
        T = self.tape
        if T is None:
            raise RuntimeError("backward() without a taped forward()")
        self.pre_backward_wait()
        cfg, P = self.cfg, self.P
        ct, cp = cfg.text, cfg.prop
        H, E, Lp, f, n = ct.hidden_size, cfg.embed_dim, cfg.n_props + 1, ct.fusion_layer, ct.num_hidden_layers
        B, Lt = T["B"], T["Lt"]
        gs = self.gscale
        scratch = self.loss_scratch
        pk, M = T["pk"], T["M"]
        S6 = T["S6"]
        if S6 is not None:
            dYtop = self._new(S6["ntop"], H)
            dY_mpm, dY_lm = dYtop[6 * B + B * Lt:], dYtop[6 * B:6 * B + B * Lt]
        else:
            nt6 = T["ytext"].shape[0]
            dY6 = self._zeros(4 * B * Lp + nt6, H)
            dYpv, dYtext = dY6[:4 * B * Lp], dY6[4 * B * Lp:]
            dY_mpm, dY_lm = dYpv[3 * B * Lp:], dYtext[nt6 - B * Lt:]

        dmln = self._new(B * Lp, H)
        ops.mpm_head(T["mpmsv"].ln.y, Lp, H, P.w("property_mtr_head.3.weight"), P.w("property_mtr_head.3.bias"), T["prop"], T["mpm_mask"], B=B,
                     ws=self.icount[4:8], losses=scratch, slot=LOSS_MPM, dh=dmln, dw=P.g("property_mtr_head.3.weight"),
                     db=P.g("property_mtr_head.3.bias"), gscale=gs[1:2])
        dmpre = self._transform_bwd(T["mpmsv"], dmln)
        ops.gemm_nt(dmpre, self._wT("property_mtr_head.0", P.w("property_mtr_head.0.weight")), dY_mpm)

        V = ct.vocab_size
        dlogits = self._new(B * Lt, _ceil(V, 64))
        ops.lm_loss(T["logits"], T["logits_m"], T["ids32"], nseq=B, L=Lt, V=V, alpha=self.alpha, ws=self.icount[0:4], losses=scratch,
                    slot=LOSS_MLM, dlogits=dlogits, gscale=gs[0:1])
        self.lm_head_bwd("text_encoder.", ct, T["lmsv"], dlogits, out=dY_lm)

        neg_p, neg_t = T["neg"][:B], T["neg"][B:]
        d_pe = self._zeros(B, Lp * H, dtype=torch.float32)
        d_te = self._zeros(M + 1, H, dtype=torch.float32)
        if S6 is not None:
            ytop = S6["ytop"]
            ops.itm_head(ytop[:3 * B], H, ytop[3 * B:6 * B], H, H, P.w("itm_head.weight"), P.w("itm_head.bias"), n=3 * B, B=B, losses=scratch,
                         slot=LOSS_ITM, dxa=dYtop[:3 * B], dxb=dYtop[3 * B:6 * B], dW=P.g("itm_head.weight"), db=P.g("itm_head.bias"), gscale=gs[3:4])
            dX6 = self._s6_backward_cls(T, dYtop, d_pe, d_te)
            dXpv = dX6[:3 * B * Lp].view(3 * B, Lp * H)
            dXt = dX6[S6["o_tp"]:S6["o_lm"]]
            ops.acc_rows(d_pe, dXpv[0:B])
            ops.acc_rows(d_pe, dXpv[B:2 * B], idx=neg_p, atomic=True)
            ops.acc_rows(d_pe, dXpv[2 * B:3 * B])
            ops.acc_rows(d_te[:M], dXt[:M])
            ops.acc_rows(d_te[:M], dXt[M:2 * M])
            ops.acc_rows(d_te, dX6[S6["o_8"]:], idx=S6["fp"]["neg_rows"], atomic=True)
            dXt_lm, dX12 = dX6[S6["o_lm"]:S6["o_12"]], dX6[S6["o_12"]:S6["o_8"]]
        else:
            ditm = self._new(3 * B, H)
            ops.itm_head(T["ypv"], Lp * H, T["itm_text"], H, H, P.w("itm_head.weight"), P.w("itm_head.bias"), n=3 * B, B=B, losses=scratch,
                         slot=LOSS_ITM, dxa=dYpv, dxb=ditm, dW=P.g("itm_head.weight"), db=P.g("itm_head.bias"), gscale=gs[3:4])
            dYtext.index_copy_(0, T["cls_text"], ditm)
            dX6 = self.stack_bwd("text_encoder.bert.", ct, range(f, n), T["tape6"], dY6, T["g6"],
                                 dkv_acc={id(T["src_text"]): d_te[:M], id(T["src_pv"]): d_pe.view(B * Lp, H)})
            dXpv, dXt = dX6[:4 * B * Lp].view(4 * B, Lp * H), dX6[4 * B * Lp:]
            ops.acc_rows(d_pe, dXpv[0:B])
            ops.acc_rows(d_pe, dXpv[B:2 * B], idx=neg_p, atomic=True)
            ops.acc_rows(d_pe, dXpv[2 * B:3 * B])
            if pk:
                ops.acc_rows(d_te[:M], dXt[:M])
                ops.acc_rows(d_te[:M], dXt[M:2 * M])
                nr = T["neg_rows"]
                ops.acc_rows(d_te, dXt[2 * M:2 * M + T["Mn"]], idx=torch.where(nr < M, nr, torch.full_like(nr, -1)), atomic=True)
            else:
                dte, dxt = d_te[:M].view(B, Lt * H), dXt.view(4 * B, Lt * H)
                ops.acc_rows(dte, dxt[0:B])
                ops.acc_rows(dte, dxt[B:2 * B])
                ops.acc_rows(dte, dxt[2 * B:3 * B], idx=neg_t, atomic=True)
            dXt_lm, dX12 = dXt[nt6 - B * Lt:], dXpv[3 * B:].reshape(B * Lp, H)

        for k, proj in enumerate(("property_proj", "text_proj")):
            feat, nrm, cls = T["feats"][proj]
            dproj = self._new(B, E)
            ops.l2norm_bwd(T["dfeat"][k * B:(k + 1) * B], feat, nrm, dproj, gscale=gs[2:3])
            self._wgrad(dproj, cls, P.g(proj + ".weight"), P.g(proj + ".bias"))
            dcls = self._new(B, H)
            ops.gemm_nt(dproj, self._wT(proj, P.w(proj + ".weight")), dcls)
            if k == 0:
                ops.acc_rows(d_pe[:, :H], dcls)
            elif pk:
                ops.acc_rows(d_te, dcls, idx=pk["row0_64"])
            else:
                ops.acc_rows(d_te[:M].view(B, Lt * H)[:, :H], dcls)
        ops.axpy_scalar(P.g("temp").view(1), self.dtemp_ita, scale_ptr=gs[2:3])

        side = self._fork()
        with self._on(side):
            dY2 = self._new(M + B * Lt, H)
            ops.cast_f32_bf16(d_te[:M].view(-1), dY2[:M].view(-1))
            dY2[M:].copy_(dXt_lm)
            dX2 = self.stack_bwd("text_encoder.bert.", ct, range(0, f), T["tape2"], dY2, T["g2"])
            if pk:
                dX2 = ops.gather_rows2(self._new(2 * B * Lt, H), dX2, pk["inv"])
            dz2 = self._embed_ln_bwd("text_encoder.bert.", ct, T["esv2"], dX2)
            tp = "text_encoder.bert.embeddings."
            ops.embed_bwd(0, dz2, nseq=2 * B, L=Lt, H=H, dpos=P.g(tp + "position_embeddings.weight"),
                          dtype0=P.g(tp + "token_type_embeddings.weight"), ids=T["ids2"], dword=P.g(tp + "word_embeddings.weight"))

        dY1 = self._new(2 * B * Lp, H)
        ops.cast_f32_bf16(d_pe.view(-1), dY1[:B * Lp].view(-1))
        dY1[B * Lp:].copy_(dX12)
        nl1 = cp.num_hidden_layers
        k1 = min(max(int(self.opt.pv_wgrad_inline), 0), nl1) if side is not None else 0
        dX1 = self.stack_bwd("property_encoder.", cp, range(k1, nl1), T["tape1"][k1:], dY1, T["g1"])
        wa, self.wgrad_async = self.wgrad_async, False
        dX1 = self.stack_bwd("property_encoder.", cp, range(0, k1), T["tape1"][:k1], dX1, T["g1"])
        self.wgrad_async = wa
        dz1 = self._embed_ln_bwd("property_encoder.", cp, T["esv1"], dX1)
        pp = "property_encoder.embeddings."
        ops.embed_bwd(1, dz1, nseq=2 * B, L=Lp, H=H, dpos=P.g(pp + "position_embeddings.weight"),
                      dtype0=P.g(pp + "token_type_embeddings.weight"), pv_x=T["prop"], pv_mask=T["mpm_mask"], src_mod=B,
                      d_w=P.g("property_embed.weight"), d_b=P.g("property_embed.bias"), d_cls=P.g("property_cls"),
                      d_masktok=P.g("property_mask"))
        self._join(side)
        self.end_backward()
```

Before: 2493 molecules/s.

## Hoist cross-attention K/V projections of all fusion layers into one batched GEMM

Concatenates the key/value weights of every fusion-layer cross-attention into a bank and computes K/V for the text and property sources with a single GEMM before the fusion stack, instead of one projection per layer. In backward, a new fold_pack kernel scatters each layer's segment-summed dKV straight into a shared buffer. One GEMM then produces the input gradient and per-layer weight GEMMs produce the weight gradients, possibly on the side stream. The banked weights are refreshed through the existing cast-transpose pass, which now also writes a non-transposed copy. This trades many small GEMMs and segment-sum/gather steps for larger batched ones, at the cost of extra memory, an extra weight copy and zero-fill of unused blocks.

```diff
diff --git a/include/spmm_hip.h b/include/spmm_hip.h
--- a/include/spmm_hip.h
+++ b/include/spmm_hip.h
@@ -68,6 +68,8 @@
                     float* P_mean, float* P_heads, long ldp, long head_stride,
                     int nseq, int nH, int Lq, int Lkv, spmm_stream_t stream);
 int spmm_segment_sum_bf16(const void* src, const int* start, const int* list, void* out, int U, long W, spmm_stream_t stream);
+int spmm_fold_pack_bf16(const void* src, const int* start, const int* list, const long* pack_idx, void* out, long ldo, long rows, int L,
+                        int W, const int* rows_dev, spmm_stream_t stream);
 
 int spmm_ln_fwd(const void* x, const void* res, const float* gamma, const float* beta, void* y, void* zout, float* mean,
                 float* rstd, long rows, int H, float eps, float dropout_p, const uint64_t* seed_ptr, uint64_t salt,
diff --git a/spmm_amd/csrc/rowops.hip b/spmm_amd/csrc/rowops.hip
--- a/spmm_amd/csrc/rowops.hip
+++ b/spmm_amd/csrc/rowops.hip
@@ -566,7 +566,7 @@
   }
 }
 
-struct CtDesc { const float* src; bf16* dstT; int R, C; int tile0, ntc; };
+struct CtDesc { const float* src; bf16* dstT; bf16* dst; int R, C; int tile0, ntc; int ldT, ldd; };
 __global__ __launch_bounds__(256) void cast_transpose_multi_kernel(const CtDesc* __restrict__ descs, int ndesc) {
   __shared__ bf16 tile[64][66];
   int lo = 0, hi = ndesc - 1;
@@ -581,13 +581,18 @@
 #pragma unroll
   for (int i = 0; i < 16; ++i) {
     const int r = r0 + ty * 16 + i, c = c0 + tx;
-    tile[ty * 16 + i][tx] = (r < d.R && c < d.C) ? (bf16)d.src[(long)r * d.C + c] : (bf16)0.f;
+    bf16 v = (bf16)0.f;
+    if (r < d.R && c < d.C) {
+      v = (bf16)d.src[(long)r * d.C + c];
+      if (d.dst) d.dst[(long)r * d.ldd + c] = v;
+    }
+    tile[ty * 16 + i][tx] = v;
   }
   __syncthreads();
 #pragma unroll
   for (int i = 0; i < 16; ++i) {
     const int c = c0 + ty * 16 + i, r = r0 + tx;
-    if (c < d.C && r < d.R) d.dstT[(long)c * d.R + r] = tile[tx][ty * 16 + i];
+    if (c < d.C && r < d.R) d.dstT[(long)c * d.ldT + r] = tile[tx][ty * 16 + i];
   }
 }
 
@@ -781,6 +786,44 @@
   for (int e = 0; e < 8; ++e) o[e] = (bf16)acc[e];
   *(bf16x8*)(out + (long)u * W + c) = o;
 }
+
+__global__ __launch_bounds__(256) void fold_pack_kernel(const bf16* __restrict__ src, const int* __restrict__ start,
+                                                        const int* __restrict__ list, const long* __restrict__ pack_idx,
+                                                        bf16* __restrict__ out, long ldo, long rows, int L, int W,
+                                                        const int* __restrict__ rows_dev) {
+  if (rows_dev) rows = rows < (long)*rows_dev ? rows : (long)*rows_dev;
+  const int w8 = W / 8;
+  for (long i = (long)blockIdx.x * blockDim.x + threadIdx.x; i < rows * w8; i += (long)gridDim.x * blockDim.x) {
+    const long r = i / w8;
+    const int c = (int)(i - r * w8) * 8;
+    const long d = pack_idx ? pack_idx[r] : r;
+    const long u = d / L;
+    const int pos = (int)(d - u * L);
+    const int k0 = start[u], k1 = start[u + 1];
+    float acc[8] = {0.f, 0.f, 0.f, 0.f, 0.f, 0.f, 0.f, 0.f};
+    for (int k = k0; k < k1; ++k) {
+      const bf16x8 v = *(const bf16x8*)(src + ((long)list[k] * L + pos) * W + c);
+#pragma unroll
+      for (int e = 0; e < 8; ++e) acc[e] += (float)v[e];
+    }
+    bf16x8 o;
+#pragma unroll
+    for (int e = 0; e < 8; ++e) o[e] = (bf16)acc[e];
+    *(bf16x8*)(out + r * ldo + c) = o;
+  }
+}
+}
+
+extern "C" int spmm_fold_pack_bf16(const void* src, const int* start, const int* list, const long* pack_idx, void* out, long ldo,
+                                   long rows, int L, int W, const int* rows_dev, hipStream_t stream) {
+  SPMM_CHECK_SHAPE(rows > 0 && L > 0 && W > 0 && W % 8 == 0, "spmm_fold_pack_bf16: rows=%ld L=%d W=%d (W %% 8 == 0)", rows, L, W);
+  SPMM_CHECK_SHAPE(src && start && list && out, "spmm_fold_pack_bf16: null src / start / list / out");
+  SPMM_CHECK_SHAPE(ldo >= W && ldo % 8 == 0 && ((uintptr_t)out % 16 == 0) && ((uintptr_t)src % 16 == 0),
+                   "spmm_fold_pack_bf16: ldo=%ld (>= W=%d, ldo %% 8 == 0, src and out 16-byte aligned)", ldo, W);
+  hipLaunchKernelGGL(fold_pack_kernel, dim3(grid_for(rows * (W / 8), 256)), dim3(256), 0, stream, (const bf16*)src, start, list,
+                     pack_idx, (bf16*)out, ldo, rows, L, W, rows_dev);
+  SPMM_LAUNCH_CHECK("spmm_fold_pack_bf16");
+  return SPMM_OK;
 }
 
 extern "C" int spmm_segment_sum_bf16(const void* src, const int* start, const int* list, void* out, int U, long W, hipStream_t stream) {
diff --git a/spmm_amd/engine.py b/spmm_amd/engine.py
--- a/spmm_amd/engine.py
+++ b/spmm_amd/engine.py
@@ -11,7 +11,7 @@
 from . import ops, streams
 from .config import BertConfig, SPMMConfig
 from .options import EngineOptions
-from .params import ParamStore
+from .params import ParamStore, XkvBank
 
 BF = torch.bfloat16
 LOSS_MLM, LOSS_MPM, LOSS_ITA, LOSS_ITM = 0, 1, 2, 3
@@ -26,6 +26,7 @@
     def __init__(self, kv: torch.Tensor, U: int, Lkv: int, row0=None, length=None, pack_idx=None, proj=None):
         self.kv, self.U, self.Lkv, self.row0, self.len, self.pack_idx = kv, U, Lkv, row0, length, pack_idx
         self.proj = proj
+        self.hoist: Optional["XkvHoist"] = None
         self._idx: List[torch.Tensor] = []
         self.nseq = 0
         self.start = self.list = None
@@ -48,6 +49,16 @@
         start[1:] = torch.cumsum(counts, 0)
         self.start, self.list = start, order.to(torch.int32)
         return self
+
+
+@dataclass
+class XkvHoist:
+    bank: "XkvBank"
+    X: torch.Tensor
+    KV: torch.Tensor
+    rows: dict
+    dKV: Optional[torch.Tensor] = None
+    wrote: Optional[set] = None
 
 
 @dataclass
@@ -469,6 +480,56 @@
             done[key] = ops.gemm_nt(kv, Wkv, self._new(kv.shape[0], Wkv.shape[0]), bias=bkv)
         return done[key]
 
+    def xkv_hoist_fwd(self, pfx, c, layers, srcs) -> Optional[XkvHoist]:
+        layers = list(layers)
+        if self.opt.xkv_hoist == "off" or len(layers) < 2 or not srcs:
+            return None
+        bank = self.P.xkv_bank([f"{pfx}encoder.layer.{i}.crossattention" for i in layers])
+        if self._pre_bwd is not None:
+            torch.cuda.current_stream().wait_event(self._pre_bwd)
+        X = torch.cat([s.kv for s in srcs])
+        KV = ops.gemm_nt(X, bank.W, self._new(X.shape[0], bank.W.shape[0]), bias=bank.b)
+        hz, r0 = XkvHoist(bank, X, KV, {}), 0
+        for s in srcs:
+            r = hz.rows[id(s)] = slice(r0, r0 + s.kv.shape[0])
+            r0 = r.stop
+            s.proj = {p: KV[r, bank.cols(l)] for p, l in bank.col.items()}
+            s.hoist = hz
+        return hz
+
+    def xkv_bwd_begin(self, hz: Optional[XkvHoist]) -> bool:
+        if hz is None or self.opt.xkv_hoist != "all" or self.layer_done_cb is not None:
+            return False
+        hz.dKV, hz.wrote = self._new(*hz.KV.shape), set()
+        return True
+
+    def xkv_bwd_finish(self, hz: XkvHoist, hub: torch.Tensor):
+        P, bank, dKV = self.P, hz.bank, hz.dKV
+        hz.dKV = None
+        for l in range(len(bank.pfxs)):
+            for sid, r in hz.rows.items():
+                if (sid, l) not in hz.wrote:
+                    ops.zero_(dKV[r, bank.cols(l)])
+        ops.gemm_nt(dKV, bank.WT, hub, epi=ops.EPI_F32_ACC)
+        gW = [P.fused(p + ".self.", ("key", "value"), "weight", what="g") for p in bank.pfxs]
+        gb = [P.fused(p + ".self.", ("key", "value"), "bias", what="g") for p in bank.pfxs]
+
+        def grads():
+            sums = self._zeros(dKV.shape[1], dtype=torch.float32)
+            for r in hz.rows.values():
+                ops.colsum_bf16(dKV[r], sums)
+            torch._foreach_add_(gb, list(sums.split(bank.W2)))
+            for l, g in enumerate(gW):
+                ops.gemm_tn(dKV[:, bank.cols(l)], hz.X, g, min_splits=len(hz.rows))
+        ws = self._wgrad_side()
+        if ws is None:
+            return grads()
+        streams.after(ws, torch.cuda.current_stream())
+        with torch.cuda.stream(ws):
+            grads()
+        self._wg_keep.append((dKV, hz.X))
+        self._wg_pending = True
+
     def _xattn_core_fwd(self, c, Qc, kv_of, groups, save, salts):
         H, nH = c.hidden_size, c.num_attention_heads
         ctx, KVs, lses = self._new(Qc.shape[0], H), [], []
@@ -552,7 +613,7 @@
             dQc = self._new(M, H)
             gWkv = P.fused(pfx + ".self.", ("key", "value"), "weight", what="g")
             gbkv = P.fused(pfx + ".self.", ("key", "value"), "bias", what="g")
-            WkvT = self._wT(pfx + ".self.kv", P.fused(pfx + ".self.", ("key", "value"), "weight", what="w"))
+            WkvT = functools.partial(self._wT, pfx + ".self.kv", P.fused(pfx + ".self.", ("key", "value"), "weight", what="w"))
             pool = {}
             for i, g in enumerate(groups):
                 r = g.rows
@@ -569,14 +630,20 @@
                                   **g.cross_layout())
                 if src is None:
                     self._wgrad(dKV, g.kv, gWkv, gbkv)
-                    ops.gemm_nt(dKV, WkvT, dkv_acc[i], epi=ops.EPI_F32_ACC)
+                    ops.gemm_nt(dKV, WkvT(), dkv_acc[i], epi=ops.EPI_F32_ACC)
             for src, dKV in pool.values():
+                hz = src.hoist
+                if hz is not None and hz.dKV is not None and pfx in hz.bank.col:
+                    l = hz.bank.col[pfx]
+                    ops.fold_pack_bf16(dKV, src.start, src.list, hz.dKV[hz.rows[id(src)], hz.bank.cols(l)], L=src.Lkv, pack_idx=src.pack_idx)
+                    hz.wrote.add((id(src), l))
+                    continue
                 W = src.Lkv * 2 * H
                 dKVu = ops.segment_sum_bf16(dKV.view(src.nseq, W), src.start, src.list, self._new(src.U, W)).view(-1, 2 * H)
                 if src.pack_idx is not None:
                     dKVu = ops.gather_rows(self._new(src.pack_idx.numel(), 2 * H), dKVu, src.pack_idx)
                 self._wgrad(dKVu, src.kv, gWkv, gbkv)
-                ops.gemm_nt(dKVu, WkvT, dkv_acc[id(src)], epi=ops.EPI_F32_ACC)
+                ops.gemm_nt(dKVu, WkvT(), dkv_acc[id(src)], epi=ops.EPI_F32_ACC)
             self._wgrad(dQc, X, P.g(pfx + ".self.query.weight"), P.g(pfx + ".self.query.bias"), md=md)
             ops.gemm_nt(dQc, self._wT(pfx + ".self.query", P.w(pfx + ".self.query.weight")), dX, R=dz, M_dev=md)
         return dX
diff --git a/spmm_amd/ops.py b/spmm_amd/ops.py
--- a/spmm_amd/ops.py
+++ b/spmm_amd/ops.py
@@ -93,12 +93,12 @@
     return C
 
 
-def gemm_tn(A, B, C, *, alpha=1.0, splits=None, kernel=0, M_dev=None):
+def gemm_tn(A, B, C, *, alpha=1.0, splits=None, kernel=0, M_dev=None, min_splits=1):
     M, N = A.shape
     K = B.shape[1]
     assert A.dtype == BF16 and B.dtype == BF16 and C.dtype == torch.float32 and B.shape[0] == M and tuple(C.shape) == (N, K)
     if splits is None:
-        splits = 1 if _DRY_RUN else lib().cdll.spmm_gemm_tn_splits(M, N, K, int(kernel))
+        splits = max(int(min_splits), 1 if _DRY_RUN else lib().cdll.spmm_gemm_tn_splits(M, N, K, int(kernel)))
     ws = torch.empty(splits * N * K, dtype=torch.float32, device=C.device) if splits > 1 else None
     _call("spmm_gemm_tn", _p(A), _row_stride(A), _p(B), _row_stride(B), M, N, K, splits, float(alpha), _p(C), _row_stride(C), _p(ws),
           int(kernel), _p(M_dev), _st())
@@ -741,6 +741,15 @@
     assert src.dtype == BF16 and out.dtype == BF16 and src.shape[1] == W and src.is_contiguous() and out.is_contiguous()
     assert start.dtype == torch.int32 and lst.dtype == torch.int32 and start.numel() == U + 1
     _call("spmm_segment_sum_bf16", _p(src), _p(start), _p(lst), _p(out), U, W, _st())
+    return out
+
+
+def fold_pack_bf16(src, start, lst, out, *, L, pack_idx=None, rows_dev=None):
+    rows, W = out.shape
+    assert src.dtype == BF16 and out.dtype == BF16 and src.shape[1] == W and src.is_contiguous() and src.shape[0] % L == 0
+    assert start.dtype == torch.int32 and lst.dtype == torch.int32
+    assert pack_idx is None or (pack_idx.dtype == torch.int64 and pack_idx.numel() >= rows)
+    _call("spmm_fold_pack_bf16", _p(src), _p(start), _p(lst), _p(pack_idx), _p(out), _row_stride(out), rows, int(L), W, _p(rows_dev), _st())
     return out
 
 
diff --git a/spmm_amd/options.py b/spmm_amd/options.py
--- a/spmm_amd/options.py
+++ b/spmm_amd/options.py
@@ -13,6 +13,7 @@
     "ln_from_y": ("SPMM_LN_FROM_Y", lambda s: s != "0"),
     "resid_fp32": ("SPMM_RESID_FP32", lambda s: s == "1"),
     "fused_xattn": ("SPMM_FUSED_XATTN", lambda s: {"0": "off", "1": "all"}.get(s, s)),
+    "xkv_hoist": ("SPMM_XKV_HOIST", lambda s: {"0": "off", "1": "all"}.get(s, s)),
     "grad_overlap": ("SPMM_GRAD_OVERLAP", lambda s: s != "0"),
     "grad_wire": ("SPMM_GRAD_WIRE", str),
     "nt_under_comm": ("SPMM_NT_UNDER_COMM", str),
@@ -32,6 +33,7 @@
     pv_wgrad_inline: int = 4
     ln_from_y: bool = True
     fused_xattn: str = "nograd"
+    xkv_hoist: str = "all"
     resid_fp32: bool = False
     grad_overlap: bool = True
     grad_wire: str = "fp32"
@@ -53,6 +55,10 @@
             o.fused_xattn = "all" if o.fused_xattn else "off"
         if o.fused_xattn not in ("off", "nograd", "all"):
             raise ValueError(f"fused_xattn must be off, nograd or all, not {o.fused_xattn!r}")
+        if isinstance(o.xkv_hoist, bool):
+            o.xkv_hoist = "all" if o.xkv_hoist else "off"
+        if o.xkv_hoist not in ("off", "fwd", "all"):
+            raise ValueError(f"xkv_hoist must be off, fwd or all, not {o.xkv_hoist!r}")
         if o.grad_wire not in ("fp32", "bf16"):
             raise ValueError(f"grad_wire must be fp32 or bf16, not {o.grad_wire!r}")
         if o.nt_under_comm not in ("tiles", "persistent", "auto"):
diff --git a/spmm_amd/params.py b/spmm_amd/params.py
--- a/spmm_amd/params.py
+++ b/spmm_amd/params.py
@@ -14,13 +14,39 @@
 
 def ct_descriptor_table(pairs):
     blob, tile0 = b"", 0
-    for src, dstT in pairs:
+    for src, dstT, *rest in pairs:
         R, C = src.shape
+        dst = rest[0] if rest else None
+        assert src.is_contiguous() and tuple(dstT.shape) == (C, R) and (dstT.stride(1) == 1 or R == 1)
+        assert dst is None or (tuple(dst.shape) == (R, C) and (dst.stride(1) == 1 or C == 1))
         ntr, ntc = (R + 63) // 64, (C + 63) // 64
-        blob += struct.pack("<QQiiii", src.data_ptr(), dstT.data_ptr(), R, C, tile0, ntc)
+        blob += struct.pack("<QQQiiiiii", src.data_ptr(), dstT.data_ptr(), 0 if dst is None else dst.data_ptr(), R, C, tile0, ntc,
+                            dstT.stride(0) if C > 1 else R, C if dst is None or R == 1 else dst.stride(0))
         tile0 += ntr * ntc
-    assert len(blob) == len(pairs) * 32
+    assert len(blob) == len(pairs) * 48
     return blob, tile0
+
+
+class XkvBank:
+
+    def __init__(self, P: "ParamStore", pfxs):
+        self.pfxs, self.col = list(pfxs), {p: i for i, p in enumerate(pfxs)}
+        self.srcW = [P.fused(p + ".self.", ("key", "value"), "weight", what="w") for p in pfxs]
+        self.srcb = [P.fused(p + ".self.", ("key", "value"), "bias", what="w") for p in pfxs]
+        self.W2, H = self.srcW[0].shape
+        n = len(pfxs) * self.W2
+        self.W = torch.empty(n, H, dtype=torch.bfloat16, device=P.device)
+        self.WT = torch.empty(H, n, dtype=torch.bfloat16, device=P.device)
+        self.b = torch.empty(n, dtype=torch.float32, device=P.device)
+
+    def cols(self, i: int) -> slice:
+        return slice(i * self.W2, (i + 1) * self.W2)
+
+    def descriptors(self):
+        return [(w, self.WT[:, self.cols(i)], self.W[self.cols(i)]) for i, w in enumerate(self.srcW)]
+
+    def refresh_bias(self):
+        torch.cat(self.srcb, out=self.b)
 
 
 def _layout_order(spec) -> List[str]:
@@ -77,6 +103,7 @@
         self._wT: Dict[str, torch.Tensor] = {}
         self._wT_pad: Dict[str, str] = {}
         self._wF: Dict[str, tuple] = {}
+        self._xkv: Dict[tuple, XkvBank] = {}
 
     def _resolve(self, name: str):
         st = student_of(name)
@@ -143,6 +170,15 @@
             w = self.w(name)
             self._wT[key][:, :w.shape[0]].copy_(w.t())
 
+    def xkv_bank(self, pfxs) -> XkvBank:
+        key = tuple(pfxs)
+        if key not in self._xkv:
+            bank = self._xkv[key] = XkvBank(self, pfxs)
+            blob, tiles = ct_descriptor_table(bank.descriptors())
+            ops.cast_transpose_multi(torch.frombuffer(bytearray(blob), dtype=torch.uint8).to(self.device), len(bank.pfxs), tiles)
+            bank.refresh_bias()
+        return self._xkv[key]
+
     def wF(self, name: str) -> torch.Tensor:
         if name not in self._wF:
             src = self.wb(name)
@@ -167,13 +203,16 @@
         if part == "forward":
             return
         srcs = getattr(self, "_wT_src", {})
-        if not srcs:
+        banked = [d for bank in self._xkv.values() for d in bank.descriptors()]
+        if not srcs and not banked:
             return
-        if getattr(self, "_ct_n", -1) != len(srcs):
-            blob, tiles = ct_descriptor_table([(src, self._wT[key]) for key, src in srcs.items()])
+        if getattr(self, "_ct_n", -1) != len(srcs) + len(banked):
+            blob, tiles = ct_descriptor_table([(src, self._wT[key]) for key, src in srcs.items()] + banked)
             self._ct_desc = torch.frombuffer(bytearray(blob), dtype=torch.uint8).to(self.device)
-            self._ct_n, self._ct_tiles = len(srcs), tiles
+            self._ct_n, self._ct_tiles = len(srcs) + len(banked), tiles
         ops.cast_transpose_multi(self._ct_desc, self._ct_n, self._ct_tiles)
+        for bank in self._xkv.values():
+            bank.refresh_bias()
 
     def copy_params(self):
         self.flat_m.copy_(self.flat)
diff --git a/spmm_amd/step.py b/spmm_amd/step.py
--- a/spmm_amd/step.py
+++ b/spmm_amd/step.py
@@ -22,6 +22,7 @@
         X6 = ops.gather_rows2(self._new(Rcap, H), y1, fp["idx6"], y2)
         src_pv = KVSource(prop_embeds.view(B * Lp, H), B, Lp).preset(4 * B, fp["start_p"], fp["list_p"])
         src_text = KVSource(text_embeds, B, Lt, row0=pk["row0"], length=pk["len"], pack_idx=pk["rows"]).preset(4 * B, fp["start_t"], fp["list_t"])
+        xkv = self.xkv_hoist_fwd("text_encoder.bert.", ct, range(f, n), [src_text, src_pv])
         ar = fp["ar"]
         g_lo = Batch([Group(0, 3 * B, Lp, None, 3 * B).bind(src_text, fp["kvidx_pv"], 0),
                       Group(o_tp, 2 * B, Lt, None, 2 * B, q_row0=fp["qrow0_tp"], q_len=fp["qlen_tp"], nrows=2 * M).bind(src_pv, fp["kvidx_tp"], 0),
@@ -41,7 +42,7 @@
                        Group(6 * B + B * Lt, B, Lp, None, 0).bind(src_text, ar, 3 * B)])
         ytop, sv_top, _ = self._layer_fwd(f"text_encoder.bert.encoder.layer.{n - 1}.", ct, True, Xtop, g_top, save)
         return dict(fp=fp, ytop=ytop, sv_top=sv_top, g_top=g_top, skv=(skv_a, skv_b), g_lo=g_lo, tape_lo=tape_lo, src_text=src_text, src_pv=src_pv,
-                    o_tp=o_tp, o_lm=o_lm, o_12=o_12, o_8=o_8, ntop=ntop, Rcap=Rcap)
+                    xkv=xkv, o_tp=o_tp, o_lm=o_lm, o_12=o_12, o_8=o_8, ntop=ntop, Rcap=Rcap)
 
     def _s6_backward_cls(self, T, dYtop, d_pe, d_te):
         S6, B, Lt, M = T["S6"], T["B"], T["Lt"], T["M"]
@@ -209,6 +210,7 @@
             ypv = ypv_h = ytop
             hp12_cls = ytop[6 * B + B * Lt:]
             src_text = src_pv = neg_rows = cls_text = itm_text = g6 = tape6 = None
+            xkv = S6["xkv"]
             Mn = B * Lt
         else:
             pe = prop_embeds.view(B, Lp * H)
@@ -251,6 +253,7 @@
             g6 = Batch([Group(0, 4 * B, Lp, None, 3 * B, kv_mask=kvmask_qpv).attend(src_text, torch.cat([ar, ar, neg[B:], ar]))] + gt)
             src_text.finalize()
             src_pv.finalize()
+            xkv = self.xkv_hoist_fwd("text_encoder.bert.", ct, range(f, n), [src_text, src_pv])
             y6, tape6, y6_32 = self.stack_fwd("text_encoder.bert.", ct, range(f, n), True, X6, g6, save, X32=torch.cat([qpv_32, qtext_32]) if r32 else None)
             ypv, ytext = y6[:4 * B * Lp], y6[4 * B * Lp:]
             ypv_h, ytext_h = (y6_32[:4 * B * Lp], y6_32[4 * B * Lp:]) if r32 else (ypv, ytext)
@@ -292,7 +295,8 @@
             self.tape = dict(B=B, Lt=Lt, pk=pk, M=M, Mn=Mn, src_text=src_text, src_pv=src_pv, neg_rows=neg_rows, cls_text=cls_text, itm_text=itm_text,
                              prop=prop, mpm_mask=mpm_mask, ids32=ids32, ids2=ids2, esv1=esv1, g1=g1, tape1=tape1,
                              esv2=esv2, g2=g2, tape2=tape2, feats=feats, dfeat=dfeat, neg=neg, g6=g6, tape6=tape6, ypv=ypv_h,
-                             ytext=ytext, logits=logits, logits_m=logits_m, lmsv=lmsv, mpmsv=mpmsv, S6=S6 if cls_top else None)
+                             ytext=ytext, logits=logits, logits_m=logits_m, lmsv=lmsv, mpmsv=mpmsv, S6=S6 if cls_top else None,
+                             xkv=xkv)
         return self.losses[:4]
 
     def backward(self):
@@ -331,13 +335,21 @@
         self.lm_head_bwd("text_encoder.", ct, T["lmsv"], dlogits, out=dY_lm)
 
         neg_p, neg_t = T["neg"][:B], T["neg"][B:]
-        d_pe = self._zeros(B, Lp * H, dtype=torch.float32)
-        d_te = self._zeros(M + 1, H, dtype=torch.float32)
+        xkv = T["xkv"]
+        batched = self.xkv_bwd_begin(xkv)
+        if batched:
+            d_te = self._zeros(M + B * Lp, H, dtype=torch.float32)
+            d_pe = d_te[M:].view(B, Lp * H)
+        else:
+            d_pe = self._zeros(B, Lp * H, dtype=torch.float32)
+            d_te = self._zeros(M + 1, H, dtype=torch.float32)
         if S6 is not None:
             ytop = S6["ytop"]
             ops.itm_head(ytop[:3 * B], H, ytop[3 * B:6 * B], H, H, P.w("itm_head.weight"), P.w("itm_head.bias"), n=3 * B, B=B, losses=scratch,
                          slot=LOSS_ITM, dxa=dYtop[:3 * B], dxb=dYtop[3 * B:6 * B], dW=P.g("itm_head.weight"), db=P.g("itm_head.bias"), gscale=gs[3:4])
             dX6 = self._s6_backward_cls(T, dYtop, d_pe, d_te)
+            if batched:
+                self.xkv_bwd_finish(xkv, d_te)
             dXpv = dX6[:3 * B * Lp].view(3 * B, Lp * H)
             dXt = dX6[S6["o_tp"]:S6["o_lm"]]
             ops.acc_rows(d_pe, dXpv[0:B])
@@ -354,6 +366,8 @@
             dYtext.index_copy_(0, T["cls_text"], ditm)
             dX6 = self.stack_bwd("text_encoder.bert.", ct, range(f, n), T["tape6"], dY6, T["g6"],
                                  dkv_acc={id(T["src_text"]): d_te[:M], id(T["src_pv"]): d_pe.view(B * Lp, H)})
+            if batched:
+                self.xkv_bwd_finish(xkv, d_te)
             dXpv, dXt = dX6[:4 * B * Lp].view(4 * B, Lp * H), dX6[4 * B * Lp:]
             ops.acc_rows(d_pe, dXpv[0:B])
             ops.acc_rows(d_pe, dXpv[B:2 * B], idx=neg_p, atomic=True)
```

Measured after the change: 2505 molecules/s (median of 6 runs). Within noise of the previous version (+0.5%).
